# jameschapman19/cca_zoo

Hardware: NVIDIA H100
Metric: rcca_fit_per_s (higher is better)
Workload: dtype tf32x3b+f32

## Files before the change

cca_zoo_b200/_base.py:

```python
from __future__ import annotations

from abc import ABC, abstractmethod
from numbers import Integral
from typing import Any, ClassVar

import numpy as np
import torch
from sklearn.base import BaseEstimator
from sklearn.utils._param_validation import Interval, StrOptions
from sklearn.utils.validation import check_is_fitted

from . import ops, parallel
from ._validation import validate_views


_COPY_STREAMS: dict = {}


def _copy_stream(device):
    key = (device.type, device.index)
    if key not in _COPY_STREAMS:
        _COPY_STREAMS[key] = torch.cuda.Stream(device)
    return _COPY_STREAMS[key]

# ... 24 lines not shown
    _wants_second_moment: ClassVar[bool] = False
    _wants_column_means: ClassVar[bool] = False

    def __init__(self, latent_dimensions: int = 1, center: bool = True, precision: str = "tf32x3b",
                 device=None) -> None:
        self.latent_dimensions = latent_dimensions
        self.center = center
        self.precision = precision
        self.device = device

    _param_names_by_class: ClassVar[dict] = {}

    def _validate_params(self):
        cls = type(self)
        names = BaseModel._param_names_by_class.get(cls)
        if names is None:
            names = BaseModel._param_names_by_class[cls] = tuple(cls._get_param_names())
        snap = tuple(_freeze(getattr(self, n, None)) for n in names)
        if self.__dict__.get("_validated_params_") == snap:
            return
        super()._validate_params()
        self._validated_params_ = snap

    @abstractmethod
    def fit(self, views, y=None):
        """Fit the model to multiview data (list of ``(n_samples, n_features_i)`` arrays)."""

    @abstractmethod
    def _solve(self, C: torch.Tensor, dims: list[int], n_total: int) -> list[torch.Tensor]:
        """Weights from the block covariance (device tensors)."""

    def _device(self) -> torch.device:
        if not torch.cuda.is_available():
            raise RuntimeError(
                "cca_zoo_b200 needs a CUDA device (sm_90a); there is no CPU fallback.  "
                "Use the reference cca_zoo package on CPU-only machines."
            )
        if self.device is None:
            return torch.device("cuda", torch.cuda.current_device())
        return torch.device(self.device)

    def _to_device(self, v, device):
        if isinstance(v, torch.Tensor):
            t = v
        else:
            arr = np.asarray(v)
            if arr.dtype not in (np.float32, np.float64):
                arr = arr.astype(np.float64)
            t = torch.from_numpy(np.ascontiguousarray(arr))
        if t.dtype not in (torch.float32, torch.float64):
            t = t.to(torch.float64)
        return t.to(device, non_blocking=True)

    _stream_threshold_bytes: ClassVar[int] = 64 << 20
    _stream_chunk_rows: ClassVar[int] = 16384

    def _local_moments(self, validated, device):
        host = all(not (isinstance(v, torch.Tensor) and v.is_cuda) for v in validated)
        n_rows = int(validated[0].shape[0])
        nbytes = sum(int(np.prod(v.shape)) * (v.element_size() if isinstance(v, torch.Tensor) else v.dtype.itemsize)
                     for v in validated)
        if not (host and nbytes >= self._stream_threshold_bytes and n_rows >= 4 * self._stream_chunk_rows):
            dev_views = [self._to_device(v, device) for v in validated]
            if len({v.dtype for v in dev_views}) > 1:
                dev_views = [v.to(torch.float64) for v in dev_views]
            dims = [int(v.shape[1]) for v in dev_views]
            mom, _ = ops.moments_safe(dev_views, precision=self.precision)
            return mom, n_rows, dims, dev_views[0].dtype
        cpu_views = []
        for v in validated:
            t = v if isinstance(v, torch.Tensor) else torch.from_numpy(np.ascontiguousarray(v))
            if t.dtype not in (torch.float32, torch.float64):
                t = t.to(torch.float64)
            cpu_views.append(t)
        if len({t.dtype for t in cpu_views}) > 1:
            cpu_views = [t.to(torch.float64) for t in cpu_views]
        dims = [int(t.shape[1]) for t in cpu_views]
        main = torch.cuda.current_stream(device)
        copy = _copy_stream(device)
        mom = None
        step = self._stream_chunk_rows
        pending = None
        self._stream_x0 = "undecided"
        for lo in range(0, n_rows, step):
            hi = min(lo + step, n_rows)
            with torch.cuda.stream(copy):
                chunk = [t[lo:hi].to(device, non_blocking=True) for t in cpu_views]
                ready = torch.cuda.Event()
                ready.record(copy)
            if pending is not None:
                mom = self._accumulate(mom, pending, main)
            pending = (chunk, ready)
        mom = self._accumulate(mom, pending, main)
        return mom, n_rows, dims, cpu_views[0].dtype

    def _accumulate(self, mom, pending, main):
        chunk, ready = pending
        main.wait_event(ready)
        for c in chunk:
            c.record_stream(main)
        if isinstance(self._stream_x0, str):
            cand, ratio = ops.column_pilot(chunk)
            self._stream_x0 = cand if ratio > ops.SHIFT_RATIO[chunk[0].dtype] else None
        if self._stream_x0 is None:
            part = ops.moments(chunk, precision=self.precision)
        else:
            part, _ = ops.moments_safe(chunk, precision=self.precision, x0=self._stream_x0)
        if mom is None:
            return part
        mom.add_(part)
        return mom

    def _solve_dtype(self, in_dtype):
        return torch.float64 if (self._solve_in_float64 or in_dtype == torch.float64) else torch.float32

    def _covariance_stage(self, mom, n_local, dims, in_dtype, check_finite, reduced=False):
        if reduced:
            n_total = int(n_local)
        else:
            mom, n_total = parallel.allreduce_moments(mom, n_local, dims=dims)
        if check_finite and not bool(torch.isfinite(mom).all()):
            raise ValueError("Input contains NaN or infinity.")
        solve_dtype = self._solve_dtype(in_dtype)
        centred = bool(self.center) or self._covariance_always_centred
        C, mean = ops.covariance(mom, dims, n_total, center=centred, dtype=solve_dtype)
        self._second_moment = None
        if self._wants_second_moment and not self.center:
            self._second_moment, _ = ops.covariance(mom, dims, n_total, center=False, dtype=solve_dtype)
        self.n_views_ = len(dims)
        self.n_features_in_ = dims
        self.n_samples_ = n_total
        off = np.concatenate([[0], np.cumsum(dims)]).astype(int)
        mean_np = mean.to(torch.float64).cpu().numpy()
        if self._wants_column_means:
            self._column_means = mean_np if centred else ops.column_means(mom, dims, n_total)
        np_dtype = np.float32 if in_dtype == torch.float32 else np.float64
        if self.center:
            self.means_ = [mean_np[off[i]:off[i + 1]].astype(np_dtype) for i in range(len(dims))]
        else:
            self.means_ = [np.zeros(p) for p in dims]
        return C, dims, n_total

    def _fit_device(self, views, min_views: int = 2):
        self._validate_params()
        validated = validate_views(views, min_views)
        device = self._device()
        mom, n_local, dims, in_dtype = self._local_moments(validated, device)
        self._partial = None
        return self._covariance_stage(mom, n_local, dims, in_dtype, True)

    def _device_fit_plan(self, dims, n_local, in_dtype):
        return None

    def _fit_moments(self, mom, n_local, dims, in_dtype):
        plan = self._device_fit_plan(dims, n_local, in_dtype)
        if plan is None:
            C, dims, n_total = self._covariance_stage(mom, n_local, dims, in_dtype, True)
            return self._finish(self._solve(C, dims, n_total))
        mom, n_host, n_dev = parallel.allreduce_moments_lazy(mom, n_local, dims=dims)
        solve_dtype = self._solve_dtype(in_dtype)
        attempts = plan.pop("iters")
        hdr = None
        for iters in attempts:
            block, offsets = plan["call"](mom, dims, n_host, n_dev, solve_dtype, iters)
            host = block.cpu()
            hdr, mean, sig, ws = ops.decode_fit_block(host, offsets, dims, plan["k"], solve_dtype)
            status = int(hdr[0])
            if status & ops.FIT_NON_FINITE:
                raise ValueError("Input contains NaN or infinity.")
            if status == 0:
                n_total = int(round(float(hdr[1])))
                self.n_views_ = len(dims)
                self.n_features_in_ = dims
                self.n_samples_ = n_total
                np_dtype = np.float32 if in_dtype == torch.float32 else np.float64
                off = np.concatenate([[0], np.cumsum(dims)]).astype(int)
                if self.center:
                    self.means_ = [mean[off[i]:off[i + 1]].astype(np_dtype) for i in range(len(dims))]
                else:
                    self.means_ = [np.zeros(p) for p in dims]
                self._second_moment = None
                self.weights_ = [np.array(w) for w in ws]
                self._fit_info = {"route": "device", "iters": iters, "residual": float(hdr[2]), "sigma_1": float(hdr[3]),
                                  "ritz_sweeps": int(hdr[5])}
                return self
            if status != ops.FIT_NOT_CONVERGED:
                break
        n_total = int(round(float(hdr[1])))
        C, dims, n_total = self._covariance_stage(mom, n_total, dims, in_dtype, False, reduced=True)
        self._fit_info = {"route": "host", "device_status": int(hdr[0])}
        return self._finish(self._solve(C, dims, n_total))

    def partial_fit(self, views, y=None, solve: bool = True):
        self._validate_params()
        validated = validate_views(views)
        device = self._device()
        mom, n_local, dims, in_dtype = self._local_moments(validated, device)
        state = getattr(self, "_partial", None)
        if state is not None:
            if state["dims"] != dims or state["dtype"] != in_dtype:
                raise ValueError(f"partial_fit batches must keep the view widths/dtype: {state['dims']} vs {dims}")
            mom = state["mom"].to(device).add_(mom)
            n_local += state["n"]
        self._partial = {"mom": mom, "n": n_local, "dims": dims, "dtype": in_dtype}
        if solve:
            if type(self)._requires_two_views and len(dims) != 2:
                raise ValueError(f"rCCA requires exactly 2 views, got {len(dims)}. Use MCCA for more than 2 views.")
            self._fit_moments(mom.clone(), n_local, dims, in_dtype)
        return self

    _requires_two_views: ClassVar[bool] = False

    def __getstate__(self):
        state = super().__getstate__()
        part = state.get("_partial")
        if part is not None:
            state = dict(state)
            state["_partial"] = {**part, "mom": part["mom"].detach().cpu()}
        return state

    def _finish(self, weights: list[torch.Tensor]):
        self.weights_ = [w.cpu().numpy() for w in weights]
        return self

    @staticmethod
    def _as_numpy_views(views):
        out = []
        for v in views:
            out.append(v.detach().cpu().numpy() if isinstance(v, torch.Tensor) else v)
        return out

    def transform(self, views):
        check_is_fitted(self)
        on_gpu = any(isinstance(v, torch.Tensor) and v.is_cuda for v in views)
        big = sum(int(np.prod(getattr(v, "shape", (0,)))) for v in views) >= self._device_score_threshold
        if on_gpu or (big and torch.cuda.is_available()):
            return self._transform_device(validate_views(views))
        validated = validate_views(self._as_numpy_views(views))
        return [(v - m) @ w for v, m, w in zip(validated, self.means_, self.weights_)]

    def _transform_device(self, validated, weights=None):
        device = self._device()
        out = []
        for v, m, w in zip(validated, self.means_, self.weights_ if weights is None else weights):
            X = self._to_device(v, device)
            np_dt = np.result_type(X.cpu().numpy().dtype if False else (np.float32 if X.dtype == torch.float32
                                                                         else np.float64), w.dtype)
            dt = torch.float32 if np_dt == np.float32 else torch.float64
            X = X.to(dt)
            W = torch.from_numpy(np.ascontiguousarray(w, dtype=np_dt)).to(device)
            mw = -(np.asarray(m, dtype=np.float64) @ np.asarray(w, dtype=np.float64))
            Z = torch.from_numpy(mw.astype(np_dt)).to(device).expand(X.shape[0], -1).contiguous()
            ops.gemm(X, W, beta=1.0, out=Z)
            out.append(Z.cpu().numpy())
        return out

    def fit_transform(self, views, y=None):
        return self.fit(views, y).transform(views)

    def score(self, views, y=None):
        return self.average_pairwise_correlations(views)

    _device_score_threshold: ClassVar[int] = 1 << 24

    def _pairwise_correlations_device(self, validated):
        device = self._device()
        dev_views = [self._to_device(v, device) for v in validated]
        if len({v.dtype for v in dev_views}) > 1:
            dev_views = [v.to(torch.float64) for v in dev_views]
        dims = [int(v.shape[1]) for v in dev_views]
        if dims != list(self.n_features_in_):
            raise ValueError(f"views have {dims} features, the model was fitted on {self.n_features_in_}")
        mom, _ = ops.moments_safe(dev_views, precision=self.precision)
        mom, n_total = parallel.allreduce_moments(mom, int(dev_views[0].shape[0]), dims=dims)
        C, _ = ops.covariance(mom, dims, n_total, center=True, dtype=torch.float64)
        off = np.concatenate([[0], np.cumsum(dims)]).astype(int)
        sl = [slice(int(off[i]), int(off[i + 1])) for i in range(len(dims))]
        W = [torch.from_numpy(np.ascontiguousarray(w, dtype=np.float64)).to(device) for w in self.weights_]
        m, k = len(dims), W[0].shape[1]
        S = torch.empty((m, m, k), dtype=torch.float64, device=device)
        for i in range(m):
            Ti = ops.gemm(C[:, sl[i]], W[i])
            for j in range(m):
                S[j, i] = ops.gemm(W[j], Ti[sl[j]], transa=True).diagonal()
        S = S.cpu().numpy()
        norms = np.sqrt(np.stack([S[i, i] for i in range(m)]) * (n_total - 1))
        denom = np.where(norms > 1e-12, norms, 1.0) / np.sqrt(n_total - 1)
        return S / (denom[:, None, :] * denom[None, :, :])

    def pairwise_correlations(self, views):
        check_is_fitted(self)
        on_gpu = any(isinstance(v, torch.Tensor) and v.is_cuda for v in views)
        big = sum(int(np.prod(getattr(v, "shape", (0,)))) for v in views) >= self._device_score_threshold
        if on_gpu or (big and torch.cuda.is_available()):
            return self._pairwise_correlations_device(validate_views(views))
        transformed = self.transform(views)
        T = np.stack(transformed, axis=0)
        T = T - T.mean(axis=1, keepdims=True)
        norms = np.sqrt((T**2).sum(axis=1, keepdims=True))
        T_norm = T / np.where(norms > 1e-12, norms, 1.0)
        return np.einsum("isd,jsd->ijd", T_norm, T_norm)

    def average_pairwise_correlations(self, views):
        corrs = self.pairwise_correlations(views)
        n_views = corrs.shape[0]
        off_diag_sum = corrs.sum(axis=(0, 1)) - sum(corrs[i, i, :] for i in range(n_views))
        return off_diag_sum / (n_views * (n_views - 1))

    @property
    def weights(self):
        check_is_fitted(self)
        return self.weights_

    def get_factor_loadings(self, views):
        validated = validate_views(self._as_numpy_views(views))
        transformed = self.transform(views)
        loadings = []
# ... 16 lines not shown
```

cca_zoo_b200/_lib.py:

```python
from __future__ import annotations

import ctypes as C
import os

_HERE = os.path.dirname(os.path.abspath(__file__))
LIB_PATH = os.path.join(_HERE, "libccab200.so")

F32, F64 = 0, 1
PREC_TF32, PREC_TF32X3, PREC_EXACT, PREC_TF32X3B = 0, 1, 2, 3
MAX_VIEWS = 8

_i64p = C.POINTER(C.c_int64)
_vp = C.c_void_p

SIGNATURES = {
    "ccab_version": (C.c_int, []),
    "ccab_last_error": (C.c_char_p, []),
    "ccab_launch_count": (C.c_int64, []),
    "ccab_moments_size": (C.c_int64, [C.c_int, _i64p]),
    "ccab_moments_padded_dim": (C.c_int64, [C.c_int, _i64p]),
    "ccab_moments_workspace_bytes": (C.c_size_t, [C.c_int, C.c_int, C.c_int, _i64p, C.c_int64]),
    "ccab_moments": (C.c_int, [C.c_int, C.c_int, C.c_int, C.POINTER(_vp), _i64p, _i64p, C.c_int64, _vp, _vp,
                               C.c_size_t, _vp]),
    "ccab_moments_packed_size": (C.c_int64, [C.c_int, _i64p]),
    "ccab_moments_pack": (C.c_int, [C.c_int, _i64p, _vp, C.c_double, _vp, _vp]),
    "ccab_moments_unpack": (C.c_int, [C.c_int, _i64p, _vp, _vp, _vp]),
    "ccab_moments_exchange_nvls": (C.c_int, [C.c_int, _i64p, _vp, C.c_double, _vp, _vp, _vp, C.c_int, C.c_int, C.c_int,
                                             C.c_int64, C.c_uint, _vp, _vp]),
    "ccab_column_pilot": (C.c_int, [C.c_int, _vp, C.c_int64, C.c_int, C.c_int64, _vp, _vp, _vp]),
    "ccab_shift_rows": (C.c_int, [C.c_int, _vp, C.c_int64, C.c_int, C.c_int64, _vp, _vp, C.c_int64, _vp]),
    "ccab_moments_unshift": (C.c_int, [C.c_int, C.c_int, _i64p, _vp, C.POINTER(_vp), C.c_double, _vp]),
    "ccab_covariance": (C.c_int, [C.c_int, C.c_int, _i64p, _vp, C.c_double, C.c_int, _vp, C.c_int64, _vp, _vp]),
    "ccab_syevj_workspace_bytes": (C.c_size_t, [C.c_int, C.c_int, C.c_int]),
    "ccab_syevj": (C.c_int, [C.c_int, C.c_int, C.c_int, _vp, C.c_int64, C.c_int64, C.c_double, _vp, _vp, C.c_int64,
                             C.POINTER(C.c_int), C.POINTER(C.c_float), _vp, C.c_size_t, _vp]),
    "ccab_syevj_small": (C.c_int, [C.c_int, C.c_int, C.c_int, _vp, C.c_int64, C.c_int64, _vp, _vp, C.c_int64, _vp, _vp]),
    "ccab_gesvj_workspace_bytes": (C.c_size_t, [C.c_int, C.c_int, C.c_int]),
    "ccab_gesvj": (C.c_int, [C.c_int, C.c_int, C.c_int, _vp, C.c_int64, _vp, _vp, C.c_int64, _vp, C.c_int64,
                             C.POINTER(C.c_int), C.POINTER(C.c_float), _vp, C.c_size_t, _vp]),
    "ccab_gemm": (C.c_int, [C.c_int, C.c_int, C.c_int, C.c_int, C.c_int, C.c_int, C.c_double, _vp, C.c_int64, _vp,
                            C.c_int64, C.c_double, _vp, C.c_int64, _vp]),
    "ccab_gemm_tc": (C.c_int, [C.c_int, C.c_int, C.c_int, C.c_int, C.c_int, C.c_double, _vp, C.c_int64, C.c_int64, _vp,
                               C.c_int64, C.c_int64, C.c_double, _vp, C.c_int64, C.c_int64, _vp, C.c_int64, C.c_int64,
                               C.c_int, C.c_int, _vp]),
    "ccab_whiten_rows": (C.c_int, [C.c_int, C.c_int, _vp, _vp, C.c_int64, C.c_double, C.c_double, _vp, C.c_double,
                                   C.c_double, C.c_int, C.c_double, _vp, C.c_int64, _vp, _vp, _vp]),
    "ccab_ccaloss_small": (C.c_int, [C.c_int, C.c_int, C.c_int, _vp, C.c_int64, C.c_double, _vp, _vp, _vp, _vp, _vp,
                                     _vp]),
    "ccab_potrf_inv_workspace_bytes": (C.c_size_t, [C.c_int, C.c_int, C.c_int]),
    "ccab_potrf_inv": (C.c_int, [C.c_int, C.c_int, C.c_int, _vp, C.c_int64, C.c_int64, _vp, C.c_int64, C.c_int64,
                                 C.c_double, _vp, _vp, C.c_size_t, _vp]),
    "ccab_rcca_fit_workspace_bytes": (C.c_size_t, [C.c_int, _i64p, C.c_int, C.c_int]),
    "ccab_rcca_fit_result_layout": (C.c_int, [C.c_int, _i64p, C.c_int, C.c_int, _i64p]),
    "ccab_rcca_fit": (C.c_int, [C.c_int, _i64p, _vp, _vp, C.c_double, C.c_int, C.POINTER(C.c_double), C.c_int, C.c_int,
                                C.c_int, _vp, C.c_size_t, _vp, C.c_size_t, _vp]),
    "ccab_ccaloss_workspace_bytes": (C.c_size_t, [C.c_int, C.c_int, C.c_int, C.c_int, C.c_int64]),
    "ccab_ccaloss_fwd": (C.c_int, [C.c_int, C.c_int, _vp, C.c_int64, _vp, C.c_int64, C.c_int64, C.c_int, C.c_int,
                                   C.c_double, _vp, _vp, _vp, _vp, C.c_size_t, _vp]),
    "ccab_ccaloss_bwd": (C.c_int, [C.c_int, _vp, C.c_int64, _vp, C.c_int64, C.c_int64, C.c_int, C.c_int, _vp, _vp, _vp,
                                   C.c_int64, _vp, C.c_int64, _vp]),
    "ccab_mcca_fit_workspace_bytes": (C.c_size_t, [C.c_int, C.c_int, _i64p, C.c_int, C.c_int]),
    "ccab_mcca_fit_result_layout": (C.c_int, [C.c_int, C.c_int, _i64p, C.c_int, C.c_int, _i64p]),
    "ccab_mcca_fit": (C.c_int, [C.c_int, C.c_int, _i64p, _vp, _vp, C.c_double, C.c_int, C.POINTER(C.c_double),
                                C.c_double, C.c_int, C.c_int, C.c_int, _vp, C.c_size_t, _vp, C.c_size_t, _vp]),
    "ccab_als_fit_workspace_bytes": (C.c_size_t, [C.c_int, _i64p]),
    "ccab_als_regression_workspace_bytes": (C.c_size_t, [C.c_int, _i64p]),
    "ccab_als_fit": (C.c_int, [C.c_int, C.c_int, _i64p, _vp, C.c_double, C.c_double, C.POINTER(C.c_double), C.c_double,
                               _vp, C.c_int, C.c_int, C.c_double, _vp, _vp, _vp, C.c_size_t, _vp]),
    "ccab_ey_fit_workspace_bytes": (C.c_size_t, [C.c_int, _i64p, C.c_int, C.c_int]),
    "ccab_ey_fit": (C.c_int, [C.c_int, _i64p, C.c_int, C.c_double, C.c_double, C.c_double, C.c_double, C.c_int, _vp,
                              C.c_int, C.POINTER(_vp), _i64p, C.c_int, _vp, _vp, _vp, C.c_size_t, _vp]),
    "ccab_gfa_fit_workspace_bytes": (C.c_size_t, [C.c_int, _i64p, C.c_int]),
    "ccab_gfa_fit": (C.c_int, [C.c_int, _i64p, C.c_int, _vp, C.c_double, _vp, C.c_double, C.c_int, C.c_int, _vp, _vp,
                               C.c_size_t, _vp]),
    "ccab_scale": (C.c_int, [C.c_int, C.c_int, C.c_int, _vp, C.c_int64, _vp, C.c_int, _vp, C.c_int, _vp, C.c_int64,
                             _vp]),
    "ccab_center_columns": (C.c_int, [C.c_int, C.c_int, C.c_int, _vp, C.c_int64, _vp]),
    "ccab_frobenius_norm": (C.c_int, [C.c_int, C.c_int, C.c_int, _vp, C.c_int64, _vp, _vp]),
    "ccab_profile_moments": (C.c_int, [C.c_int]),
    "ccab_profile_moments_last_ms": (C.c_double, []),
}

_lib = None


def load():
    global _lib
    if _lib is None:
        if not os.path.exists(LIB_PATH):
            raise RuntimeError(
                f"{LIB_PATH} not found: build it with `python -c 'import __graft_entry__ as g; g.build()'` "
                "(or `make -C cca_zoo_b200/csrc`).  cca_zoo_b200 has no CPU fallback."
            )
        lib = C.CDLL(LIB_PATH)
        for name, (res, args) in SIGNATURES.items():
            fn = getattr(lib, name)
            fn.restype = res
            fn.argtypes = args
        _lib = lib
    return _lib


def last_error() -> str:
    return load().ccab_last_error().decode("utf-8", "replace")


def check(rc: int, what: str) -> None:
    if rc == 0:
        return
    msg = f"{what} failed (code {rc}): {last_error()}"
    if rc < 0:
        raise ValueError(msg)
    raise RuntimeError(msg)


def i64_array(values):
    return (C.c_int64 * len(values))(*[int(v) for v in values])
```

cca_zoo_b200/_solvers.py:

```python
from __future__ import annotations

import os

import numpy as np
import torch

from . import ops


def _slices(dims):
    off = np.concatenate([[0], np.cumsum(dims)]).astype(int)
    return [slice(int(off[i]), int(off[i + 1])) for i in range(len(dims))]


def _eps(dtype):
    return float(torch.finfo(dtype).eps)


class _two_streams:

    _pool = {}

    def __init__(self, device):
        self.device = device

    def __enter__(self):
        key = (self.device.index, torch.cuda.current_stream(self.device).cuda_stream)
        if key not in self._pool:
            self._pool[key] = [torch.cuda.Stream(self.device), torch.cuda.Stream(self.device)]
        self.streams = self._pool[key]
        self.main = torch.cuda.current_stream(self.device)
        ev = torch.cuda.Event()
        ev.record(self.main)
        for st in self.streams:
            st.wait_event(ev)
        return self.streams

    def __exit__(self, *exc):
        for st in self.streams:
            ev = torch.cuda.Event()
            ev.record(st)
            self.main.wait_event(ev)
        return False


def _rank_tol(d, dtype):
    return d * _eps(dtype)


def _regularised_rank_tol(lam, c, d):
    tol = _rank_tol(d, lam.dtype)
    if c == 0.0:
        return tol
    if c >= 1.0:
        return -1.0
    lam_max = max(float(lam[0].item()), 0.0)
    thr = (tol * ((1.0 - c) * lam_max + c) - c) / (1.0 - c)
    if thr < 0.0 or lam_max == 0.0:
        return -1.0
    return thr / lam_max


def _block_eigh(C, dims):
    sl = _slices(dims)
    lams, vts = [None] * len(dims), [None] * len(dims)
    by_size = {}
    for i, d in enumerate(dims):
        by_size.setdefault(d, []).append(i)
    for d, idx in by_size.items():
        A = torch.stack([C[sl[i], sl[i]] for i in idx]).contiguous()
        ev, evt = ops.syevj(A)
        for b, i in enumerate(idx):
            lams[i], vts[i] = ev[b], evt[b]
    return lams, vts


def _cholqr(Y, flags, passes=1):
    for _ in range(passes):
        Ginv, info = ops.potrf_inv_(ops.gemm(Y, Y, transa=True))
        flags.append(info)
        Y = ops.gemm(Y, Ginv, transb=True)
    return Y


def topk_svd(T, k, max_rounds=4, iters_per_round=5, oversample=None, seed=1234):
    d1, d2 = T.shape
    if oversample is None:
        oversample = int(os.environ.get("CCAB_TOPK_OVERSAMPLE", "0")) or max(32, k // 2)
    p = min(min(d1, d2), k + oversample)
    gen = torch.Generator(device=T.device).manual_seed(seed)
    Z = torch.randn((d2, p), generator=gen, device=T.device, dtype=T.dtype)
    flags = []
    tol = 200.0 * _eps(T.dtype)
    iters_per_round = int(os.environ.get("CCAB_TOPK_ITERS", "0")) or iters_per_round
    for _ in range(max_rounds):
        for it in range(iters_per_round):
            Y = ops.gemm(T, Z)
            Z = _cholqr(ops.gemm(T, Y, transa=True), flags,
                         passes=2 if it == iters_per_round - 1 else 1)
        Y = ops.gemm(T, Z)
        sig2, Vy_t = ops.syevj(ops.gemm(Y, Y, transa=True))
        sig = sig2.clamp_min(0).sqrt()
        Ut = ops.scale(ops.gemm(Vy_t[:k], Y, transb=True), rows=sig[:k], rows_pow=-1)
        Vt = ops.gemm(Vy_t[:k], Z, transb=True)
        E = ops.gemm(Ut, T)
        E -= ops.scale(Vt, rows=sig[:k])
        stats = torch.stack([ops.frobenius_norm(E)[0], sig[0], torch.stack(flags).max().to(T.dtype).reshape(())])
        resid, s1, bad = (float(x) for x in stats.cpu())
        if os.environ.get("CCAB_DEBUG_TOPK"):
            print(f"[topk_svd] p={p} iters={iters_per_round} resid={resid:.3e} limit={tol * s1 * (k ** 0.5):.3e}")
        if bad != 0.0 or not (s1 > 0.0):
            return None
        if resid <= tol * s1 * (k ** 0.5):
            return sig[:k], Ut, Vt
        flags = []
        Z = ops.gemm(Z, Vy_t, transb=True)
    return None


def topk_eigsh(K, k, shift, max_rounds=6, iters_per_round=8, seed=4321):
    D = K.shape[0]
    p = min(D, max(2 * k, k + 32))
    gen = torch.Generator(device=K.device).manual_seed(seed)
    Z = torch.randn((D, p), generator=gen, device=K.device, dtype=K.dtype)
    flags = []
    Z = _cholqr(Z, flags, passes=2)
    tol = 200.0 * _eps(K.dtype)
    for _ in range(max_rounds):
        for it in range(iters_per_round):
            Y = ops.gemm(K, Z)
            if shift != 0.0:
                Y.add_(Z, alpha=shift)
            Z = _cholqr(Y, flags, passes=2 if it == iters_per_round - 1 else 1)
        KZ = ops.gemm(K, Z)
        H = ops.gemm(Z, KZ, transa=True)
        H = 0.5 * (H + H.T)
        nrm = ops.frobenius_norm(H)
        theta, Qt = ops.syevj(H, shift=float(nrm.item()))
        Zr_t = ops.gemm(Qt[:k], Z, transb=True)
        E = ops.gemm(Qt[:k], KZ, transb=True)
        E -= ops.scale(Zr_t, rows=theta[:k])
        stats = torch.stack([ops.frobenius_norm(E)[0], theta[0].abs() + abs(shift),
                             torch.stack(flags).max().to(K.dtype).reshape(())])
        resid, scale, bad = (float(x) for x in stats.cpu())
        if bad != 0.0 or not (scale > 0.0):
            return None
        if resid <= tol * scale * (k ** 0.5):
            return theta[:k], Zr_t
        flags = []
        Z = ops.gemm(Z, Qt, transb=True)
    return None


def _cholesky_whiteners(C, dims, c, scales, eps_floor):
    sl = _slices(dims)
    out, flags, norms = [], [], []
    for i, s in enumerate(sl):
        R = (1.0 - c[i]) * C[s, s]
        R.diagonal().add_(c[i])
        dmax = R.diagonal().max()
        Linv, info = ops.potrf_inv_(R, pivot_tol=0.0)
        flags.append(info)
        norms.append(torch.stack([ops.frobenius_norm(Linv)[0], dmax]))
        out.append(Linv)
    stats = torch.cat([torch.stack(flags).max().to(C.dtype).reshape(1), torch.stack(norms).reshape(-1)]).cpu()
    if float(stats[0]) != 0.0:
        return None
    for i in range(len(dims)):
        fro, dmax = float(stats[1 + 2 * i]), float(stats[2 + 2 * i])
        if not (fro > 0.0) or not np.isfinite(fro):
            return None
        lam_min_lb = 1.0 / (fro * fro)
        if lam_min_lb < eps_floor or lam_min_lb < _rank_tol(dims[i], C.dtype) * dmax:
            return None
    return [Linv if scales[i] == 1.0 else Linv.mul_(scales[i] ** 0.5) for i, Linv in enumerate(out)]


def mcca_weights_cholesky(C, dims, latent_dimensions, c, eps):
    m = len(dims)
    sl = _slices(dims)
    D = C.shape[0]
    k = min(latent_dimensions, D)
    if 4 * k > D:
        return None
    Linv = _cholesky_whiteners(C, dims, c, [1.0] * m, eps)
    if Linv is None:
        return None
    K = torch.zeros((D, D), dtype=C.dtype, device=C.device)
    for i in range(m):
        for j in range(i + 1, m):
            tmp = ops.gemm(Linv[i], C[sl[i], sl[j]])
            ops.gemm(tmp, Linv[j], transb=True, out=K[sl[i], sl[j]])
            K[sl[j], sl[i]] = K[sl[i], sl[j]].T
    cmax = max(c)
    shift = 1.0 / (1.0 - cmax) if cmax <= 0.9 else float(ops.frobenius_norm(K).item())
    res = topk_eigsh(K, k, shift)
    if res is None:
        return None
    _, Yt = res
    return [ops.gemm(Linv[i], Yt[:, sl[i]], transa=True, transb=True, alpha=m ** 0.5) for i in range(m)]


def _pad_null_components(weights, k_out):
    k = weights[0].shape[1]
    if k_out <= k:
        return weights
    return [torch.cat([w, torch.zeros((w.shape[0], k_out - k), dtype=w.dtype, device=w.device)], dim=1)
            for w in weights]


def gcca_weights_cholesky(C, dims, n_samples, latent_dimensions, c, mu, eps, second_moment=None):
    Cd = C if second_moment is None else second_moment
    m = len(dims)
    sl = _slices(dims)
    D = C.shape[0]
    k = min(latent_dimensions, D, n_samples)
    if 4 * k > D:
        return None
    Wt = _cholesky_whiteners(C, dims, c, mu, eps)
    if Wt is None:
        return None
    Lc = _cholesky_whiteners(Cd, dims, [0.0] * m, [1.0] * m, 0.0) \
        if (Cd is not C or any(ci != 0.0 for ci in c) or any(x == 0.0 for x in mu)) \
        else [w / (mu[i] ** 0.5) for i, w in enumerate(Wt)]
# ... 159 lines not shown
```

cca_zoo_b200/csrc/api.cu:

```cuda
#include "../../include/ccab200.h"

#include <cstdarg>
#include <cmath>
#include <cstring>
#include <atomic>
#include <exception>

#include "als.cuh"
#include "ccaloss.cuh"
#include "cholinv.cuh"
#include "common.cuh"
#include "gfa.cuh"
#include "dense.cuh"
#include "ey.cuh"
#include "fit.cuh"
#include "moments.cuh"
#include "syevj.cuh"
#include "syevj_small.cuh"
#include "tgemm.cuh"

namespace ccab {
static thread_local char g_err[512] = "";
void set_error(const char* fmt, ...) {
  va_list ap;
// ... 321 lines not shown
              const void* B, int64_t ldb, double beta, void* C, int64_t ldc, void* stream) {
  CCAB_TRY
  CCAB_CHECK_ARG(dtype == CCAB_F32 || dtype == CCAB_F64, "bad dtype %d", dtype);
  CCAB_CHECK_ARG(A && B && C, "null pointer argument");
  int rc = require_device();
  if (rc) return rc;
  cudaStream_t s = static_cast<cudaStream_t>(stream);
  if (dtype == CCAB_F32) {
    GemmArgs<float> g;
    g.transa = transa; g.transb = transb; g.m = m; g.n = n; g.k = k; g.alpha = (float)alpha; g.beta = (float)beta;
    g.A = static_cast<const float*>(A); g.lda = lda; g.B = static_cast<const float*>(B); g.ldb = ldb;
    g.C = static_cast<float*>(C); g.ldc = ldc;
    return xgemm<float>(g, s);
  }
  GemmArgs<double> g;
  g.transa = transa; g.transb = transb; g.m = m; g.n = n; g.k = k; g.alpha = alpha; g.beta = beta;
  g.A = static_cast<const double*>(A); g.lda = lda; g.B = static_cast<const double*>(B); g.ldb = ldb;
  g.C = static_cast<double*>(C); g.ldc = ldc;
  return xgemm<double>(g, s);
  CCAB_CATCH
}

int ccab_gemm_tc(int transa, int transb, int m, int n, int k, double alpha, const void* A, int64_t lda,
                 int64_t stride_a, const void* B, int64_t ldb, int64_t stride_b, double beta, void* C, int64_t ldc,
                 int64_t stride_c, void* Ct, int64_t ldct, int64_t stride_ct, int batch, int lower_only,
                 void* stream) {
  CCAB_TRY
  CCAB_CHECK_ARG(A && B && (C || Ct), "null pointer argument");
  CCAB_CHECK_ARG(m >= 1 && n >= 1 && k >= 1 && batch >= 1, "bad shape m=%d n=%d k=%d batch=%d", m, n, k, batch);
  CCAB_CHECK_ARG((!C || ldc >= n) && (!Ct || ldct >= m), "output leading dimension too small");
  int rc = require_device();
  if (rc) return rc;
  TgemmArgs a;
  a.transa = transa;
  a.transb = transb;
  a.m = m;
  a.n = n;
  a.k = k;
  a.alpha = (float)alpha;
  a.beta = (float)beta;
  a.A = static_cast<const float*>(A);
  a.lda = lda;
  a.strideA = stride_a;
  a.B = static_cast<const float*>(B);
  a.ldb = ldb;
  a.strideB = stride_b;
  a.C = static_cast<float*>(C);
  a.ldc = ldc;
  a.strideC = stride_c;
  a.Ct = static_cast<float*>(Ct);
  a.ldct = ldct;
  a.strideCt = stride_ct;
  a.batch = batch;
  a.lower_only = lower_only;
  return tgemm(a, static_cast<cudaStream_t>(stream));
  CCAB_CATCH
}

int ccab_whiten_rows(int dtype, int d, const void* lam, const void* Vt, int64_t ldv, double c, double floor_add,
                     const void* floor_dev, double scale, double rank_tol, int max_rank, double lam_floor, void* Wt,
                     int64_t ldw, void* g_out, int* rank_out, void* stream) {
  CCAB_TRY
  CCAB_CHECK_ARG(dtype == CCAB_F32 || dtype == CCAB_F64, "bad dtype %d", dtype);
  CCAB_CHECK_ARG(lam && Vt && Wt, "null pointer argument");
  CCAB_CHECK_ARG(scale > 0.0, "scale must be positive");
  int rc = require_device();
  if (rc) return rc;
  cudaStream_t s = static_cast<cudaStream_t>(stream);
  if (dtype == CCAB_F32)
    return whiten_rows<float>(d, static_cast<const float*>(lam), static_cast<const float*>(Vt), ldv, c, floor_add,
                              static_cast<const float*>(floor_dev), scale, rank_tol, max_rank, lam_floor,
                              static_cast<float*>(Wt), ldw, static_cast<float*>(g_out), rank_out, s);
  return whiten_rows<double>(d, static_cast<const double*>(lam), static_cast<const double*>(Vt), ldv, c, floor_add,
                             static_cast<const double*>(floor_dev), scale, rank_tol, max_rank, lam_floor,
                             static_cast<double*>(Wt), ldw, static_cast<double*>(g_out), rank_out, s);
  CCAB_CATCH
}

int ccab_ccaloss_small(int dtype, int d1, int d2, const void* C, int64_t ldc, double eps, void* loss, void* G11,
                       void* P, void* G22, void* min_pivot, void* stream) {
  CCAB_TRY
  CCAB_CHECK_ARG(dtype == CCAB_F32 || dtype == CCAB_F64, "bad dtype %d", dtype);
  CCAB_CHECK_ARG(C && loss && G11 && P && G22 && min_pivot, "null pointer argument");
  int rc = require_device();
  if (rc) return rc;
  cudaStream_t s = static_cast<cudaStream_t>(stream);
  if (dtype == CCAB_F32)
    return ccaloss_small<float>(static_cast<const float*>(C), ldc, d1, d2, eps, static_cast<float*>(loss),
                                static_cast<float*>(G11), static_cast<float*>(P), static_cast<float*>(G22),
                                static_cast<float*>(min_pivot), s);
  return ccaloss_small<double>(static_cast<const double*>(C), ldc, d1, d2, eps, static_cast<double*>(loss),
                               static_cast<double*>(G11), static_cast<double*>(P), static_cast<double*>(G22),
                               static_cast<double*>(min_pivot), s);
  CCAB_CATCH
}

size_t ccab_potrf_inv_workspace_bytes(int dtype, int n, int batch) {
  if (n < 1 || batch < 1) return 0;
  return dtype == CCAB_F32 ? potrf_inv_workspace_bytes<float>(n, batch) : potrf_inv_workspace_bytes<double>(n, batch);
}

int ccab_potrf_inv(int dtype, int n, int batch, void* A, int64_t lda, int64_t stride_a, void* Linv, int64_t ldi,
                   int64_t stride_i, double pivot_tol, int* info_dev, void* workspace, size_t workspace_bytes,
                   void* stream) {
  CCAB_TRY
  CCAB_CHECK_ARG(dtype == CCAB_F32 || dtype == CCAB_F64, "bad dtype %d", dtype);
  CCAB_CHECK_ARG(A && Linv && info_dev && workspace, "null pointer argument");
  int rc = require_device();
  if (rc) return rc;
  cudaStream_t s = static_cast<cudaStream_t>(stream);
  if (dtype == CCAB_F32)
    return potrf_inv<float>(n, batch, static_cast<float*>(A), lda, stride_a, static_cast<float*>(Linv), ldi, stride_i,
                            pivot_tol, nullptr, info_dev, workspace, workspace_bytes, s);
  return potrf_inv<double>(n, batch, static_cast<double*>(A), lda, stride_a, static_cast<double*>(Linv), ldi, stride_i,
                           pivot_tol, nullptr, info_dev, workspace, workspace_bytes, s);
  CCAB_CATCH
}

size_t ccab_rcca_fit_workspace_bytes(int dtype, const int64_t* dims, int k, int p) {
  if (!dims || dims[0] < 1 || dims[1] < 1 || (dtype != CCAB_F32 && dtype != CCAB_F64)) return 0;
  return dtype == CCAB_F32 ? rcca_fit_workspace_bytes<float>((int)dims[0], (int)dims[1], k, p)
                           : rcca_fit_workspace_bytes<double>((int)dims[0], (int)dims[1], k, p);
}

int ccab_rcca_fit_result_layout(int dtype, const int64_t* dims, int k, int p, int64_t* offsets) {
  CCAB_TRY
  CCAB_CHECK_ARG(dims && offsets && dims[0] >= 1 && dims[1] >= 1 && k >= 1 && p >= k, "bad argument");
  if (dtype == CCAB_F32) rcca_fit_result_layout<float>((int)dims[0], (int)dims[1], k, p, offsets);
  else rcca_fit_result_layout<double>((int)dims[0], (int)dims[1], k, p, offsets);
  return 0;
  CCAB_CATCH
}

int ccab_rcca_fit(int dtype, const int64_t* dims, const double* moments, const double* n_total_dev, double n_total,
                  int center, const double* c, int k, int p, int iters, void* result, size_t result_bytes,
                  void* workspace, size_t workspace_bytes, void* stream) {
  CCAB_TRY
  CCAB_CHECK_ARG(dtype == CCAB_F32 || dtype == CCAB_F64, "bad dtype %d", dtype);
  CCAB_CHECK_ARG(dims && moments && c && result && workspace, "null pointer argument");
  ColumnLayout L;
  int rc = make_layout(2, dims, &L);
  if (rc) return rc;
  rc = require_device();
  if (rc) return rc;
  cudaStream_t s = static_cast<cudaStream_t>(stream);
  if (dtype == CCAB_F32)
    return rcca_fit<float>(L, moments, n_total_dev, n_total, center, c, k, p, iters, result, result_bytes, workspace,
                           workspace_bytes, s);
  return rcca_fit<double>(L, moments, n_total_dev, n_total, center, c, k, p, iters, result, result_bytes, workspace,
                          workspace_bytes, s);
  CCAB_CATCH
}

size_t ccab_ccaloss_workspace_bytes(int dtype, int precision, int d1, int d2, int64_t n) {
  int64_t dims[2] = {d1, d2};
  ColumnLayout L;
  if (make_layout(2, dims, &L)) return 0;
  if (dtype == CCAB_F64) precision = CCAB_PREC_EXACT;
  return dtype == CCAB_F32 ? ccaloss_workspace_bytes<float>(L, n, precision)
                           : ccaloss_workspace_bytes<double>(L, n, precision);
}

int ccab_ccaloss_fwd(int dtype, int precision, const void* z1, int64_t ld1, const void* z2, int64_t ld2, int64_t n,
                     int d1, int d2, double eps, void* loss, void* saved, int* flags_dev, void* workspace,
                     size_t workspace_bytes, void* stream) {
  CCAB_TRY
  CCAB_CHECK_ARG(dtype == CCAB_F32 || dtype == CCAB_F64, "bad dtype %d", dtype);
  CCAB_CHECK_ARG(precision >= 0 && precision <= 3, "bad precision %d", precision);
  CCAB_CHECK_ARG(z1 && z2 && loss && saved && flags_dev && workspace, "null pointer argument");
  CCAB_CHECK_ARG(ld1 >= d1 && ld2 >= d2, "leading dimension too small");
  int64_t dims[2] = {d1, d2};
  ColumnLayout L;
  int rc = make_layout(2, dims, &L);
  if (rc) return rc;
  rc = require_device();
  if (rc) return rc;
  cudaStream_t s = static_cast<cudaStream_t>(stream);
  if (dtype == CCAB_F32)
    return ccaloss_forward<float>(L, precision, z1, ld1, z2, ld2, n, eps, static_cast<float*>(loss),
                                  static_cast<float*>(saved), flags_dev, workspace, workspace_bytes, s);
  return ccaloss_forward<double>(L, CCAB_PREC_EXACT, z1, ld1, z2, ld2, n, eps, static_cast<double*>(loss),
                                 static_cast<double*>(saved), flags_dev, workspace, workspace_bytes, s);
  CCAB_CATCH
}

int ccab_ccaloss_bwd(int dtype, const void* z1, int64_t ld1, const void* z2, int64_t ld2, int64_t n, int d1, int d2,
                     const void* saved, const void* grad_out, void* g1, int64_t ldg1, void* g2, int64_t ldg2,
                     void* stream) {
  CCAB_TRY
  CCAB_CHECK_ARG(dtype == CCAB_F32 || dtype == CCAB_F64, "bad dtype %d", dtype);
  CCAB_CHECK_ARG(z1 && z2 && saved && g1 && g2, "null pointer argument");
  CCAB_CHECK_ARG(ld1 >= d1 && ld2 >= d2 && ldg1 >= d1 && ldg2 >= d2, "leading dimension too small");
  int rc = require_device();
  if (rc) return rc;
  cudaStream_t s = static_cast<cudaStream_t>(stream);
  if (dtype == CCAB_F32)
    return ccaloss_backward<float>(d1, d2, static_cast<const float*>(z1), ld1, static_cast<const float*>(z2), ld2, n,
                                   static_cast<const float*>(saved), static_cast<const float*>(grad_out),
                                   static_cast<float*>(g1), ldg1, static_cast<float*>(g2), ldg2, s);
  return ccaloss_backward<double>(d1, d2, static_cast<const double*>(z1), ld1, static_cast<const double*>(z2), ld2, n,
                                  static_cast<const double*>(saved), static_cast<const double*>(grad_out),
                                  static_cast<double*>(g1), ldg1, static_cast<double*>(g2), ldg2, s);
  CCAB_CATCH
}

size_t ccab_mcca_fit_workspace_bytes(int dtype, int n_views, const int64_t* dims, int k, int p) {
  ColumnLayout L;
  if (!dims || make_layout(n_views, dims, &L) || (dtype != CCAB_F32 && dtype != CCAB_F64)) return 0;
  return dtype == CCAB_F32 ? mcca_fit_workspace_bytes<float>(L, k, p) : mcca_fit_workspace_bytes<double>(L, k, p);
}

int ccab_mcca_fit_result_layout(int dtype, int n_views, const int64_t* dims, int k, int p, int64_t* offsets) {
  CCAB_TRY
  CCAB_CHECK_ARG(dims && offsets && k >= 1 && p >= k, "bad argument");
  ColumnLayout L;
  int rc = make_layout(n_views, dims, &L);
  if (rc) return rc;
  if (dtype == CCAB_F32) mcca_fit_result_layout<float>(L, k, p, offsets);
  else mcca_fit_result_layout<double>(L, k, p, offsets);
  return 0;
  CCAB_CATCH
}

int ccab_mcca_fit(int dtype, int n_views, const int64_t* dims, const double* moments, const double* n_total_dev,
                  double n_total, int center, const double* c, double eps, int k, int p, int iters, void* result,
                  size_t result_bytes, void* workspace, size_t workspace_bytes, void* stream) {
  CCAB_TRY
  CCAB_CHECK_ARG(dtype == CCAB_F32 || dtype == CCAB_F64, "bad dtype %d", dtype);
  CCAB_CHECK_ARG(dims && moments && c && result && workspace, "null pointer argument");
  ColumnLayout L;
  int rc = make_layout(n_views, dims, &L);
  if (rc) return rc;
  rc = require_device();
  if (rc) return rc;
  cudaStream_t s = static_cast<cudaStream_t>(stream);
  if (dtype == CCAB_F32)
    return mcca_fit<float>(L, moments, n_total_dev, n_total, center, c, eps, k, p, iters, result, result_bytes,
                           workspace, workspace_bytes, s);
  return mcca_fit<double>(L, moments, n_total_dev, n_total, center, c, eps, k, p, iters, result, result_bytes, workspace,
                          workspace_bytes, s);
  CCAB_CATCH
}

size_t ccab_als_fit_workspace_bytes(int n_views, const int64_t* dims) {
  ColumnLayout L;
  if (!dims || n_views < 2 || make_layout(n_views, dims, &L)) return 0;
  return als_fit_workspace_bytes(L, false);
}

size_t ccab_als_regression_workspace_bytes(int n_views, const int64_t* dims) {
  ColumnLayout L;
  if (!dims || n_views < 2 || make_layout(n_views, dims, &L)) return 0;
  return als_fit_workspace_bytes(L, true);
}

int ccab_als_fit(int kind, int n_views, const int64_t* dims, const double* G, double g_scale, double n_samples,
                 const double* params, double mu, const double* init, int k, int max_iter, double tol, double* W_out,
                 int* iters_out, void* workspace, size_t workspace_bytes, void* stream) {
  CCAB_TRY
  CCAB_CHECK_ARG(kind >= CCAB_ALS_PLS && kind <= CCAB_ALS_IPLS, "bad ALS kind %d", kind);
  CCAB_CHECK_ARG(n_views >= 2, "the ALS estimators need at least 2 views, got %d", n_views);
  CCAB_CHECK_ARG(dims && G && init && W_out && iters_out && workspace, "null pointer argument");
  CCAB_CHECK_ARG(kind == CCAB_ALS_PLS || params, "params is NULL");
  CCAB_CHECK_ARG(k >= 1 && max_iter >= 0, "bad k %d / max_iter %d", k, max_iter);
  CCAB_CHECK_ARG(kind != CCAB_ALS_ADMM || (mu > 0.0 && n_samples > 0.0), "ADMM needs mu > 0 and n_samples > 0");
  ColumnLayout L;
  int rc = make_layout(n_views, dims, &L);
  if (rc) return rc;
  const bool reg = kind == CCAB_ALS_ELASTIC || kind == CCAB_ALS_IPLS;
  for (int v = 0; reg && v < n_views; ++v) {
    const double alpha = params[2 * v], l1 = params[2 * v + 1];
    CCAB_CHECK_ARG(alpha >= 0.0 && alpha < INFINITY, "alpha[%d] = %g is not a finite non-negative number", v, alpha);
    CCAB_CHECK_ARG(l1 >= 0.0 && l1 <= 1.0, "l1_ratio[%d] = %g is not in [0, 1]", v, l1);
    CCAB_CHECK_ARG(dims[v] <= 2048, "view %d has %lld features; ElasticCCA / SCCA_IPLS take at most 2048 per view", v,
                   (long long)dims[v]);
  }
  CCAB_CHECK_ARG(!reg || n_samples > 0.0, "ElasticCCA / SCCA_IPLS need n_samples > 0");
  CCAB_CHECK_ARG(!reg || (mu >= 0.0 && mu < 1.0), "the eigenvalue cut mu = %g of ElasticCCA / SCCA_IPLS is not in [0, 1)",
                 mu);
  for (int v = 0; kind != CCAB_ALS_PLS && !reg && v < n_views; ++v) {
    CCAB_CHECK_ARG(params[v] >= 0.0, "params[%d] = %g is negative", v, params[v]);
    CCAB_CHECK_ARG(kind != CCAB_ALS_SPAN || (params[v] >= 1.0 && params[v] == (double)(int64_t)params[v]),
                   "span[%d] = %g is not a positive integer", v, params[v]);
  }
  rc = require_device();
  if (rc) return rc;
  return als_fit(kind, L, G, g_scale, n_samples, params, mu, init, k, max_iter, tol, W_out, iters_out, workspace,
                 workspace_bytes, static_cast<cudaStream_t>(stream));
  CCAB_CATCH
}

size_t ccab_ey_fit_workspace_bytes(int n_views, const int64_t* dims, int k, int batch) {
  ColumnLayout L;
  if (!dims || n_views < 2 || k < 1 || k > kEyMaxK || batch < 0 || batch == 1 || make_layout(n_views, dims, &L))
    return 0;
  return ey_fit_workspace_bytes(L, k, batch);
}

int ccab_ey_fit(int n_views, const int64_t* dims, int k, double c, double learning_rate, double momentum, double tol,
                int n_steps, const double* cov, int dtype, const void* const* views, const int64_t* ld, int batch,
                const int32_t* idx, double* state, void* workspace, size_t workspace_bytes, void* stream) {
  CCAB_TRY
  CCAB_CHECK_ARG(n_views >= 2, "the EY estimators need at least 2 views, got %d", n_views);
  CCAB_CHECK_ARG(dims && state && workspace, "null pointer argument");
  CCAB_CHECK_ARG(k >= 1 && k <= kEyMaxK, "k = %d: the EY fit supports 1 <= k <= %d", k, kEyMaxK);
  CCAB_CHECK_ARG(n_steps >= 0, "bad n_steps %d", n_steps);
// ... 104 lines not shown
```

cca_zoo_b200/csrc/fit.cu:

```cuda
#include "fit.cuh"

#include <cmath>
#include <type_traits>

#include "ccaloss.cuh"
#include "cholinv.cuh"
#include "dense.cuh"
#include "moments.cuh"
#include "syevj_small.cuh"

namespace ccab {

namespace {

inline size_t al256(size_t x) { return (x + 255) & ~size_t(255); }
inline int64_t r4(int64_t x) { return (x + 3) & ~int64_t(3); }

struct CovRidgeParams {
  int n_views, D, Dp;
  int dims[kMaxViews];
  int coff[kMaxViews + 1];
  int poff[kMaxViews + 1];
  double c[kMaxViews];
  double ridge_add[kMaxViews];
  void* R[kMaxViews];
  long long ldr[kMaxViews];
};
struct PivotTolParams {
  int n_views;
  double c[kMaxViews], rank_tol[kMaxViews];
  double floor;
};

__device__ __forceinline__ int view_of(const CovRidgeParams& p, int g) {
  int v = 0;
  while (v + 1 < p.n_views && p.coff[v + 1] <= g) ++v;
  return v;
}

template <typename T>
__global__ void cov_ridge_kernel(const CovRidgeParams p, const double* __restrict__ mom, const double* __restrict__ n_dev,
                                 double n_host, int center, T* __restrict__ C, int64_t ldc, double* __restrict__ mean,
                                 unsigned* __restrict__ dmax, int* __restrict__ flags) {
  const double n_total = n_dev ? n_dev[0] : n_host;
  const double* M = mom;
  const double* s = mom + (size_t)p.Dp * p.Dp;
  const int gi = blockIdx.y * blockDim.y + threadIdx.y;
  const int gj = blockIdx.x * blockDim.x + threadIdx.x;
  if (gi >= p.D || gj >= p.D) return;
  const int vi = view_of(p, gi), vj = view_of(p, gj);
  const int pi = p.poff[vi] + gi - p.coff[vi], pj = p.poff[vj] + gj - p.coff[vj];
  const int r = min(pi, pj), c = max(pi, pj);
  double v = M[(size_t)r * p.Dp + c];
  if (!isfinite(v)) atomicOr(flags, 1);
  if (center) v -= s[pi] * s[pj] / n_total;
  v /= (n_total - 1.0);
  C[(size_t)gi * ldc + gj] = (T)v;
  if (vi == vj && p.R[vi]) {
    const double cv = p.c[vi];
    const double rv = (1.0 - cv) * v + (gi == gj ? cv + p.ridge_add[vi] : 0.0);
    static_cast<T*>(p.R[vi])[(size_t)(gi - p.coff[vi]) * p.ldr[vi] + (gj - p.coff[vj])] = (T)rv;
    if (gi == gj && dmax) atomicMax(dmax + vi, __float_as_uint(fmaxf((float)v, 0.f)));
  }
  if (gi == 0 && mean) mean[gj] = center ? s[pj] / n_total : 0.0;
  if (gi == 0 && gj == 0 && !(n_total >= 2.0)) atomicOr(flags, 2);
}

__global__ void pivot_tol_kernel(const PivotTolParams q, const unsigned* __restrict__ dmax, double* __restrict__ tol) {
  const int v = threadIdx.x;
  if (v < q.n_views) tol[v] = fmax(q.floor, q.rank_tol[v] * ((1.0 - q.c[v]) * (double)__uint_as_float(dmax[v]) + q.c[v]));
}

template <typename T>
__global__ void randn_kernel(T* __restrict__ Z, int64_t ld, int rows, int cols, unsigned long long seed) {
  const size_t total = (size_t)rows * cols;
  for (size_t e = blockIdx.x * (size_t)blockDim.x + threadIdx.x; e < total; e += (size_t)gridDim.x * blockDim.x) {
    unsigned long long x = seed + 0x9E3779B97F4A7C15ull * (e + 1);
    x = (x ^ (x >> 30)) * 0xBF58476D1CE4E5B9ull;
    x = (x ^ (x >> 27)) * 0x94D049BB133111EBull;
    x ^= x >> 31;
    const double u1 = ((double)(unsigned)(x >> 32) + 1.0) * (1.0 / 4294967297.0);
    const double u2 = (double)(unsigned)(x & 0xffffffffu) * (1.0 / 4294967296.0);
    const double g = sqrt(-2.0 * log(u1)) * cospi(2.0 * u2);
    Z[(e / cols) * ld + (e % cols)] = (T)g;
  }
}

template <typename T>
__global__ void ritz_scale_kernel(T* __restrict__ U, int64_t ldu, int rows, int k, const T* __restrict__ lam,
                                  T* __restrict__ sig) {
  const int j = blockIdx.x * blockDim.x + threadIdx.x;
  const int i = blockIdx.y;
  if (j >= k) return;
  const T s = sqrt(fmax(lam[j], T(0)));
  if (i == 0 && sig) sig[j] = s;
  U[(size_t)i * ldu + j] *= s > T(0) ? T(1) / s : T(0);
}

constexpr int kResidBlocks = 64;
template <typename T>
__global__ void __launch_bounds__(256)
residual_kernel(const T* __restrict__ E, int64_t lde, const T* __restrict__ V, int64_t ldv, int rows, int k,
                const T* __restrict__ sig, double shift, int sym, double* __restrict__ stats,
                double* __restrict__ partial, unsigned* __restrict__ counter) {
  __shared__ double red[8];
  __shared__ bool last;
  const int per = (rows + gridDim.x - 1) / gridDim.x;
  const int r0 = blockIdx.x * per;
  const int nr = max(0, min(rows, r0 + per) - r0);
  double acc = 0.0;
  for (int e = threadIdx.x; e < nr * k; e += blockDim.x) {
    const int i = r0 + e / k, j = e % k;
    const double d = (double)E[(size_t)i * lde + j] - (double)V[(size_t)i * ldv + j] * (double)sig[j];
    acc += d * d;
  }
  for (int o = 16; o > 0; o >>= 1) acc += __shfl_xor_sync(0xffffffffu, acc, o);
  if ((threadIdx.x & 31) == 0) red[threadIdx.x >> 5] = acc;
  __syncthreads();
  if (threadIdx.x == 0) {
    double t = 0.0;
    for (int w = 0; w < (int)(blockDim.x >> 5); ++w) t += red[w];
    partial[blockIdx.x] = t;
    __threadfence();
    last = atomicAdd(counter, 1u) == gridDim.x - 1;
    if (last) {
      __threadfence();
      double tot = 0.0;
      for (unsigned b = 0; b < gridDim.x; ++b) tot += *reinterpret_cast<volatile double*>(partial + b);
      stats[0] = tot;
      stats[1] = sym ? fabs((double)sig[0]) + shift : (double)sig[0];
      *counter = 0u;
    }
  }
}

__global__ void fit_status_kernel(double* __restrict__ hdr, const int* __restrict__ flags, const int* __restrict__ infos,
                                  int n_infos, const int* __restrict__ rr_info, const double* __restrict__ stats,
                                  const double* __restrict__ n_dev, double n_host, double resid_tol, int k, int max_d) {
  if (threadIdx.x != 0) return;
  const double n_total = n_dev ? n_dev[0] : n_host;
  int status = 0;
  if (flags[0] & 1) status |= kFitNonFinite;
  if (flags[0] & 2) status |= kFitTooFewSamples;
  int first_bad = 0;
  for (int i = 0; i < n_infos; ++i)
    if (infos[i] != 0 && !first_bad) first_bad = i + 1;
  if (first_bad) status |= kFitNotPositiveDefinite;
  const double resid = sqrt(fmax(stats[0], 0.0)), s1 = stats[1];
  if (!(s1 > 0.0) || !(resid <= resid_tol * s1 * sqrt((double)k))) status |= kFitNotConverged;
  if (rr_info && rr_info[0] <= 0) status |= kFitNotConverged;
  if (!(n_total > (double)max_d)) status |= kFitTooFewSamples;
  hdr[0] = (double)status;
  hdr[1] = n_total;
  hdr[2] = resid;
  hdr[3] = s1;
  hdr[4] = (double)first_bad;
  hdr[5] = rr_info ? (double)rr_info[0] : 0.0;
}

template <typename T>
double eps_of() {
  return std::is_same<T, float>::value ? 1.1920928955078125e-7 : 2.220446049250313e-16;
}
template <typename T>
double resid_tol_of() {
  return std::max(200.0 * eps_of<T>(), 1e-10);
}

template <typename T>
struct CholQrWs {
  T* G;
  T* Ginv;
  void* pws;
  size_t pws_bytes;
  int64_t ldg;
  void* splitk_ws = nullptr;
  size_t splitk_ws_bytes = 0;
};

template <typename T>
int cholqr(const T* Zin, int64_t ldz, T* Zout, int64_t ldo, int rows, int p, const CholQrWs<T>& w, int* info,
           cudaStream_t s) {
  GemmArgs<T> g;
  g.transa = 1; g.m = p; g.n = p; g.k = rows;
  g.A = Zin; g.lda = ldz; g.B = Zin; g.ldb = ldz; g.C = w.G; g.ldc = w.ldg;
  g.splitk_ws = w.splitk_ws; g.splitk_ws_bytes = w.splitk_ws_bytes;
  int rc = xgemm<T>(g, s);
  if (rc) return rc;
  const int NB = potrf_inv_block_size<T>();
  int64_t ldi;
  if (p <= NB) {
    rc = potrf_inv_block<T>(w.G, w.ldg, 0, p, 0, w.Ginv, 0, 0.0, nullptr, info, 1, s);
    ldi = NB;
  } else {
    int* tmp_info = info;
    rc = potrf_inv<T>(p, 1, w.G, w.ldg, 0, w.Ginv, w.ldg, 0, 0.0, nullptr, tmp_info, w.pws, w.pws_bytes, s);
    ldi = w.ldg;
  }
  if (rc) return rc;
  GemmArgs<T> q;
  q.transb = 1; q.m = rows; q.n = p; q.k = p;
  q.A = Zin; q.lda = ldz; q.B = w.Ginv; q.ldb = ldi; q.C = Zout; q.ldc = ldo;
  return xgemm<T>(q, s);
}

struct RccaPlan {
  int d1, d2, D, k, p;
  int64_t ldC, ld1, ld2, ldT, ldp, ldk;
  size_t oC, oR, oLinv, oT1, oT, oZ, oZ2, oY, oG, oGinv, oH, oLam, oVy, oU, oV, oE, oPws, oSplit, oSmall, total;
  size_t pws_bytes, split_bytes;
  size_t r_mean, r_sig, r_w1, r_w2, r_total;
};

template <typename T>
RccaPlan make_rcca_plan(int d1, int d2, int k, int p) {
  RccaPlan P;
  P.d1 = d1; P.d2 = d2; P.D = d1 + d2; P.k = k; P.p = p;
  P.ldC = r4(P.D); P.ld1 = r4(d1); P.ld2 = r4(d2); P.ldT = r4(d2); P.ldp = r4(p); P.ldk = r4(k);
  const int NB = potrf_inv_block_size<T>();
  const int dm = std::max(d1, d2);
  size_t o = 0;
  auto take = [&](size_t elems) { size_t at = o; o += al256(elems * sizeof(T)); return at; };
  P.oC = take((size_t)P.D * P.ldC);
  P.oR = take(2 * (size_t)dm * r4(dm));
  P.oLinv = take(2 * (size_t)dm * r4(dm));
  P.oT1 = take((size_t)d1 * P.ldT);
  P.oT = take((size_t)d1 * P.ldT);
  P.oZ = take((size_t)d2 * P.ldp);
  P.oZ2 = take((size_t)d2 * P.ldp);
  P.oY = take((size_t)d1 * P.ldp);
  P.oG = take((size_t)p * P.ldp);
  P.oGinv = take((size_t)std::max(p, NB) * std::max<int64_t>(P.ldp, NB));
  P.oH = take((size_t)p * P.ldp);
  P.oLam = take((size_t)p);
  P.oVy = take((size_t)p * P.ldp);
  P.oU = take((size_t)d1 * P.ldk);
  P.oV = take((size_t)d2 * P.ldk);
  P.oE = take((size_t)d2 * P.ldk);
  P.pws_bytes = std::max(potrf_inv_workspace_bytes<T>(dm, 2), potrf_inv_workspace_bytes<T>(p, 1));
  P.oPws = o; o += al256(P.pws_bytes);
  P.split_bytes = 8 * (size_t)dm * r4(std::max(p, k)) * sizeof(T);
  P.oSplit = o; o += al256(P.split_bytes);
  P.oSmall = o; o += 4096;
  P.total = o + 256;
  size_t r = sizeof(double) * kFitHeaderDoubles;
  P.r_mean = r; r += al256(sizeof(double) * P.D);
  P.r_sig = r; r += al256(sizeof(T) * k);
  P.r_w1 = r; r += al256(sizeof(T) * (size_t)d1 * k);
  P.r_w2 = r; r += al256(sizeof(T) * (size_t)d2 * k);
  P.r_total = r;
  return P;
}

}

template <typename T>
size_t rcca_fit_workspace_bytes(int d1, int d2, int k, int p) {
  if (!(k >= 1 && p >= k && p <= std::min(d1, d2) && syevj_small_supported<T>(p))) return 0;
  return make_rcca_plan<T>(d1, d2, k, p).total;
}

template <typename T>
void rcca_fit_result_layout(int d1, int d2, int k, int p, int64_t* offsets) {
  RccaPlan P = make_rcca_plan<T>(d1, d2, k, p);
  offsets[0] = (int64_t)P.r_mean;
  offsets[1] = (int64_t)P.r_sig;
  offsets[2] = (int64_t)P.r_w1;
  offsets[3] = (int64_t)P.r_w2;
  offsets[4] = (int64_t)P.r_total;
}

template <typename T>
int rcca_fit(const ColumnLayout& L, const double* moments, const double* n_dev, double n_host, int center,
             const double* c, int k, int p, int iters, void* result, size_t result_bytes, void* ws, size_t ws_bytes,
             cudaStream_t s) {
  CCAB_CHECK_ARG(L.n_views == 2, "rcca_fit needs exactly 2 views");
  const int d1 = L.dims[0], d2 = L.dims[1], D = L.D;
  CCAB_CHECK_ARG(k >= 1 && p >= k && p <= std::min(d1, d2), "rcca_fit: need 1 <= k <= p <= min(d1, d2), got k=%d p=%d", k,
                 p);
  CCAB_CHECK_ARG(syevj_small_supported<T>(p), "rcca_fit: subspace width %d exceeds the single-CTA eigensolver", p);
  CCAB_CHECK_ARG(iters >= 1 && iters <= 64, "rcca_fit: bad iteration count %d", iters);
  RccaPlan P = make_rcca_plan<T>(d1, d2, k, p);
  CCAB_CHECK_ARG(ws_bytes >= P.total, "rcca_fit workspace too small: %zu < %zu", ws_bytes, P.total);
  CCAB_CHECK_ARG(result_bytes >= P.r_total, "rcca_fit result block too small: %zu < %zu", result_bytes, P.r_total);
  uint8_t* w = reinterpret_cast<uint8_t*>((reinterpret_cast<uintptr_t>(ws) + 255) & ~uintptr_t(255));
  uint8_t* res = static_cast<uint8_t*>(result);
  CCAB_CHECK_ARG((reinterpret_cast<uintptr_t>(res) & 255) == 0, "rcca_fit: result block must be 256-byte aligned");
  auto at = [&](size_t off) { return reinterpret_cast<T*>(w + off); };
  T* C = at(P.oC);
  const bool batched = d1 == d2;
  const int64_t ldR = r4(std::max(d1, d2));
  const int64_t strideR = (int64_t)std::max(d1, d2) * ldR;
  T* R1 = at(P.oR);
  T* R2 = R1 + strideR;
  T* Li1 = at(P.oLinv);
  T* Li2 = Li1 + strideR;
  const int64_t ldr1 = batched ? ldR : P.ld1, ldr2 = batched ? ldR : P.ld2;
  T *T1 = at(P.oT1), *Tm = at(P.oT), *Z = at(P.oZ), *Z2 = at(P.oZ2), *Y = at(P.oY), *H = at(P.oH), *lam = at(P.oLam),
    *Vy = at(P.oVy), *U = at(P.oU), *V = at(P.oV), *E = at(P.oE);
  CholQrWs<T> cq;
  cq.G = at(P.oG);
  cq.Ginv = at(P.oGinv);
  cq.pws = w + P.oPws;
  cq.pws_bytes = P.pws_bytes;
  cq.ldg = P.ldp;
  cq.splitk_ws = w + P.oSplit;
  cq.splitk_ws_bytes = P.split_bytes;
  auto thin = [&](GemmArgs<T>& g) { g.splitk_ws = cq.splitk_ws; g.splitk_ws_bytes = cq.splitk_ws_bytes; };
  uint8_t* sm = w + P.oSmall;
  int* flags = reinterpret_cast<int*>(sm);
  int* infos = flags + 4;
  const int n_infos = 2 + iters + 2;
  int* rr_info = infos + 80;
  unsigned* dmax = reinterpret_cast<unsigned*>(sm + 512);
  double* tol = reinterpret_cast<double*>(sm + 1024);
  double* stats = tol + 8;
  double* resid_part = reinterpret_cast<double*>(sm + 1280);
  unsigned* resid_cnt = reinterpret_cast<unsigned*>(sm + 1280 + 8 * kResidBlocks);

  CCAB_CUDA(cudaMemsetAsync(sm, 0, 2048, s));
  double* hdr = reinterpret_cast<double*>(res);
  double* mean = reinterpret_cast<double*>(res + P.r_mean);
  T* sig = reinterpret_cast<T*>(res + P.r_sig);
  T* W1 = reinterpret_cast<T*>(res + P.r_w1);
  T* W2 = reinterpret_cast<T*>(res + P.r_w2);

  {
    CovRidgeParams cp;
    memset(&cp, 0, sizeof(cp));
    cp.n_views = 2; cp.D = D; cp.Dp = L.Dp;
    for (int v = 0; v < 2; ++v) { cp.dims[v] = L.dims[v]; cp.c[v] = c[v]; }
    for (int v = 0; v <= 2; ++v) { cp.coff[v] = L.coff[v]; cp.poff[v] = L.poff[v]; }
    cp.R[0] = R1; cp.R[1] = R2; cp.ldr[0] = ldr1; cp.ldr[1] = ldr2;
    dim3 block(32, 8), grid((unsigned)ceil_div(D, 32), (unsigned)ceil_div(D, 8));
    cov_ridge_kernel<T><<<grid, block, 0, s>>>(cp, moments, n_dev, n_host, center, C, P.ldC, mean, dmax, flags);
    count_launches(1);
    PivotTolParams q;
    memset(&q, 0, sizeof(q));
    q.n_views = 2;
    q.c[0] = c[0]; q.c[1] = c[1];
    q.rank_tol[0] = d1 * eps_of<T>(); q.rank_tol[1] = d2 * eps_of<T>();
    pivot_tol_kernel<<<1, 32, 0, s>>>(q, dmax, tol);
    count_launches(1);
    CCAB_CUDA(cudaGetLastError());
  }
  int rc;
  if (batched) {
    rc = potrf_inv<T>(d1, 2, R1, ldR, strideR, Li1, ldR, strideR, 0.0, tol, infos, cq.pws, cq.pws_bytes, s);
    if (rc) return rc;
  } else {
    rc = potrf_inv<T>(d1, 1, R1, ldr1, 0, Li1, ldr1, 0, 0.0, tol, infos, cq.pws, cq.pws_bytes, s);
    if (rc) return rc;
    rc = potrf_inv<T>(d2, 1, R2, ldr2, 0, Li2, ldr2, 0, 0.0, tol + 1, infos + 1, cq.pws, cq.pws_bytes, s);
    if (rc) return rc;
  }
  {
    GemmArgs<T> g;
    g.m = d1; g.n = d2; g.k = d1;
    g.A = Li1; g.lda = ldr1; g.B = C + d1; g.ldb = P.ldC; g.C = T1; g.ldc = P.ldT;
    rc = xgemm<T>(g, s);
    if (rc) return rc;
    GemmArgs<T> h;
    h.transb = 1; h.m = d1; h.n = d2; h.k = d2;
    h.A = T1; h.lda = P.ldT; h.B = Li2; h.ldb = ldr2; h.C = Tm; h.ldc = P.ldT;
    rc = xgemm<T>(h, s);
    if (rc) return rc;
  }
  {
    const size_t total = (size_t)d2 * p;
    randn_kernel<T><<<(unsigned)std::min<size_t>((total + 255) / 256, 592), 256, 0, s>>>(Z, P.ldp, d2, p, 0x1234ull);
    count_launches(1);
    CCAB_CUDA(cudaGetLastError());
  }
  int info_slot = 2;
  const bool gram = d2 <= d1 && iters >= 2;
  if (gram) {
    GemmArgs<T> g;
    g.transa = 1; g.m = d2; g.n = d2; g.k = d1; g.A = Tm; g.lda = P.ldT; g.B = Tm; g.ldb = P.ldT; g.C = T1; g.ldc = P.ldT;
    rc = xgemm<T>(g, s);
    if (rc) return rc;
  }
  for (int it = 0; it < iters; ++it) {
    if (gram) {
      GemmArgs<T> a;
      a.transa = 1; a.m = d2; a.n = p; a.k = d2; a.A = T1; a.lda = P.ldT; a.B = Z; a.ldb = P.ldp; a.C = Z2; a.ldc = P.ldp;
      thin(a);
      rc = xgemm<T>(a, s);
      if (rc) return rc;
    } else {
      GemmArgs<T> a;
      a.m = d1; a.n = p; a.k = d2; a.A = Tm; a.lda = P.ldT; a.B = Z; a.ldb = P.ldp; a.C = Y; a.ldc = P.ldp;
      rc = xgemm<T>(a, s);
      if (rc) return rc;
      GemmArgs<T> b;
      b.transa = 1; b.m = d2; b.n = p; b.k = d1; b.A = Tm; b.lda = P.ldT; b.B = Y; b.ldb = P.ldp; b.C = Z2; b.ldc = P.ldp;
      rc = xgemm<T>(b, s);
      if (rc) return rc;
    }
    rc = cholqr<T>(Z2, P.ldp, Z, P.ldp, d2, p, cq, infos + info_slot++, s);
    if (rc) return rc;
    if (it == iters - 1) {
      rc = cholqr<T>(Z, P.ldp, Z2, P.ldp, d2, p, cq, infos + info_slot++, s);
      if (rc) return rc;
      std::swap(Z, Z2);
    }
  }
  {
    GemmArgs<T> a;
    a.m = d1; a.n = p; a.k = d2; a.A = Tm; a.lda = P.ldT; a.B = Z; a.ldb = P.ldp; a.C = Y; a.ldc = P.ldp;
    thin(a);
    rc = xgemm<T>(a, s);
    if (rc) return rc;
    GemmArgs<T> h;
    h.transa = 1; h.m = p; h.n = p; h.k = d1; h.A = Y; h.lda = P.ldp; h.B = Y; h.ldb = P.ldp; h.C = H; h.ldc = P.ldp;
    thin(h);
    rc = xgemm<T>(h, s);
    if (rc) return rc;
    rc = syevj_small<T>(p, 1, H, P.ldp, 0, lam, p, Vy, P.ldp, 0, rr_info, s);
    if (rc) return rc;
    GemmArgs<T> u;
    u.transb = 1; u.m = d1; u.n = k; u.k = p; u.A = Y; u.lda = P.ldp; u.B = Vy; u.ldb = P.ldp; u.C = U; u.ldc = P.ldk;
    rc = xgemm<T>(u, s);
    if (rc) return rc;
    ritz_scale_kernel<T><<<dim3((unsigned)ceil_div(k, 128), (unsigned)d1), 128, 0, s>>>(U, P.ldk, d1, k, lam, sig);
    count_launches(1);
    GemmArgs<T> v;
    v.transb = 1; v.m = d2; v.n = k; v.k = p; v.A = Z; v.lda = P.ldp; v.B = Vy; v.ldb = P.ldp; v.C = V; v.ldc = P.ldk;
    rc = xgemm<T>(v, s);
    if (rc) return rc;
    GemmArgs<T> e;
    e.transa = 1; e.m = d2; e.n = k; e.k = d1; e.A = Tm; e.lda = P.ldT; e.B = U; e.ldb = P.ldk; e.C = E; e.ldc = P.ldk;
    thin(e);
    rc = xgemm<T>(e, s);
    if (rc) return rc;
    residual_kernel<T><<<kResidBlocks, 256, 0, s>>>(E, P.ldk, V, P.ldk, d2, k, sig, 0.0, 0, stats, resid_part, resid_cnt);
    count_launches(1);
    CCAB_CUDA(cudaGetLastError());
  }
  {
    GemmArgs<T> a;
    a.transa = 1; a.m = d1; a.n = k; a.k = d1; a.A = Li1; a.lda = ldr1; a.B = U; a.ldb = P.ldk; a.C = W1; a.ldc = k;
    thin(a);
    rc = xgemm<T>(a, s);
    if (rc) return rc;
    GemmArgs<T> b;
    b.transa = 1; b.m = d2; b.n = k; b.k = d2; b.A = Li2; b.lda = ldr2; b.B = V; b.ldb = P.ldk; b.C = W2; b.ldc = k;
    thin(b);
    rc = xgemm<T>(b, s);
    if (rc) return rc;
  }
  fit_status_kernel<<<1, 32, 0, s>>>(hdr, flags, infos, n_infos, rr_info, stats, n_dev, n_host, resid_tol_of<T>(), k,
                                    std::max(d1, d2));
  count_launches(1);
  CCAB_CUDA(cudaGetLastError());
  return 0;
}


namespace {

struct MccaPlan {
  int m, D, k, p, dmax;
  bool equal;
  int64_t ldC, ldR, strideR, ldp, ldk;
  int off[kMaxViews + 1];
  size_t oC, oR, oLinv, oTmp, oK, oZ, oZ2, oY, oG, oGinv, oH, oLam, oVy, oZr, oE, oPws, oSplit, oSmall, total;
  size_t pws_bytes, split_bytes;
  size_t r_mean, r_val, r_w[kMaxViews], r_total;
};

template <typename T>
MccaPlan make_mcca_plan(const ColumnLayout& L, int k, int p) {
  MccaPlan P;
  P.m = L.n_views; P.D = L.D; P.k = k; P.p = p;
  P.dmax = 0;
  P.equal = true;
  for (int v = 0; v < P.m; ++v) {
    P.dmax = std::max(P.dmax, L.dims[v]);
    if (L.dims[v] != L.dims[0]) P.equal = false;
    P.off[v] = L.coff[v];
  }
  P.off[P.m] = L.D;
  P.ldC = r4(P.D); P.ldR = r4(P.dmax); P.strideR = (int64_t)P.dmax * P.ldR; P.ldp = r4(p); P.ldk = r4(k);
  const int NB = potrf_inv_block_size<T>();
  size_t o = 0;
  auto take = [&](size_t elems) { size_t at = o; o += al256(elems * sizeof(T)); return at; };
  P.oC = take((size_t)P.D * P.ldC);
  P.oR = take((size_t)P.m * P.strideR);
  P.oLinv = take((size_t)P.m * P.strideR);
  P.oTmp = take((size_t)P.dmax * P.ldR);
  P.oK = take((size_t)P.D * P.ldC);
  P.oZ = take((size_t)P.D * P.ldp);
  P.oZ2 = take((size_t)P.D * P.ldp);
  P.oY = take((size_t)P.D * P.ldp);
  P.oG = take((size_t)p * P.ldp);
  P.oGinv = take((size_t)std::max(p, NB) * std::max<int64_t>(P.ldp, NB));
  P.oH = take((size_t)p * P.ldp);
  P.oLam = take((size_t)p);
  P.oVy = take((size_t)p * P.ldp);
  P.oZr = take((size_t)P.D * P.ldk);
  P.oE = take((size_t)P.D * P.ldk);
  P.pws_bytes = std::max(potrf_inv_workspace_bytes<T>(P.dmax, P.m), potrf_inv_workspace_bytes<T>(p, 1));
  P.oPws = o; o += al256(P.pws_bytes);
  P.split_bytes = 8 * (size_t)P.D * p * sizeof(T);
  P.oSplit = o; o += al256(P.split_bytes);
  P.oSmall = o; o += 4096;
  P.total = o + 256;
  size_t r = sizeof(double) * kFitHeaderDoubles;
  P.r_mean = r; r += al256(sizeof(double) * P.D);
  P.r_val = r; r += al256(sizeof(T) * k);
  for (int v = 0; v < P.m; ++v) { P.r_w[v] = r; r += al256(sizeof(T) * (size_t)L.dims[v] * k); }
  P.r_total = r;
  return P;
}

template <typename T>
__global__ void copy_vals_kernel(const T* __restrict__ src, T* __restrict__ dst, int k) {
  const int j = blockIdx.x * blockDim.x + threadIdx.x;
  if (j < k) dst[j] = src[j];
}

}

template <typename T>
size_t mcca_fit_workspace_bytes(const ColumnLayout& L, int k, int p) {
  if (!(L.n_views >= 2 && k >= 1 && p >= k && p <= L.D && syevj_small_supported<T>(p))) return 0;
  return make_mcca_plan<T>(L, k, p).total;
}

template <typename T>
void mcca_fit_result_layout(const ColumnLayout& L, int k, int p, int64_t* offsets) {
  MccaPlan P = make_mcca_plan<T>(L, k, p);
  offsets[0] = (int64_t)P.r_mean;
  offsets[1] = (int64_t)P.r_val;
  for (int v = 0; v < P.m; ++v) offsets[2 + v] = (int64_t)P.r_w[v];
  offsets[2 + P.m] = (int64_t)P.r_total;
}

template <typename T>
int mcca_fit(const ColumnLayout& L, const double* moments, const double* n_dev, double n_host, int center,
             const double* c, double eps_floor, int k, int p, int iters, void* result, size_t result_bytes, void* ws,
             size_t ws_bytes, cudaStream_t s) {
  const int m = L.n_views, D = L.D;
  CCAB_CHECK_ARG(m >= 2, "mcca_fit needs at least 2 views");
  CCAB_CHECK_ARG(k >= 1 && p >= k && p <= D, "mcca_fit: need 1 <= k <= p <= D, got k=%d p=%d", k, p);
  CCAB_CHECK_ARG(syevj_small_supported<T>(p), "mcca_fit: subspace width %d exceeds the single-CTA eigensolver", p);
  CCAB_CHECK_ARG(iters >= 1 && iters <= 60, "mcca_fit: bad iteration count %d", iters);
  double cmax = 0.0;
  for (int v = 0; v < m; ++v) cmax = std::max(cmax, c[v]);
  CCAB_CHECK_ARG(cmax <= 0.9, "mcca_fit: max c = %g > 0.9 (no a-priori shift); use the host-assembled route", cmax);
  MccaPlan P = make_mcca_plan<T>(L, k, p);
  CCAB_CHECK_ARG(ws_bytes >= P.total, "mcca_fit workspace too small: %zu < %zu", ws_bytes, P.total);
  CCAB_CHECK_ARG(result_bytes >= P.r_total, "mcca_fit result block too small: %zu < %zu", result_bytes, P.r_total);
  uint8_t* w = reinterpret_cast<uint8_t*>((reinterpret_cast<uintptr_t>(ws) + 255) & ~uintptr_t(255));
  uint8_t* res = static_cast<uint8_t*>(result);
  CCAB_CHECK_ARG((reinterpret_cast<uintptr_t>(res) & 255) == 0, "mcca_fit: result block must be 256-byte aligned");
  auto at = [&](size_t off) { return reinterpret_cast<T*>(w + off); };
  T *C = at(P.oC), *R = at(P.oR), *Linv = at(P.oLinv), *Tmp = at(P.oTmp), *K = at(P.oK), *Z = at(P.oZ), *Z2 = at(P.oZ2),
    *Y = at(P.oY), *H = at(P.oH), *lam = at(P.oLam), *Vy = at(P.oVy), *Zr = at(P.oZr), *E = at(P.oE);
  CholQrWs<T> cq;
  cq.G = at(P.oG);
  cq.Ginv = at(P.oGinv);
  cq.pws = w + P.oPws;
  cq.pws_bytes = P.pws_bytes;
  cq.ldg = P.ldp;
  cq.splitk_ws = w + P.oSplit;
  cq.splitk_ws_bytes = P.split_bytes;
  uint8_t* sm = w + P.oSmall;
  int* flags = reinterpret_cast<int*>(sm);
  int* infos = flags + 4;
  const int n_infos = m + iters + 4;
  int* rr_info = infos + 100;
  unsigned* dmax = reinterpret_cast<unsigned*>(sm + 512);
  double* tol = reinterpret_cast<double*>(sm + 1024);
  double* stats = tol + kMaxViews;
  double* resid_part = reinterpret_cast<double*>(sm + 1280);
  unsigned* resid_cnt = reinterpret_cast<unsigned*>(sm + 1280 + 8 * kResidBlocks);
  CCAB_CUDA(cudaMemsetAsync(sm, 0, 2048, s));
  CCAB_CUDA(cudaMemsetAsync(K, 0, sizeof(T) * (size_t)D * P.ldC, s));
  double* hdr = reinterpret_cast<double*>(res);
  double* mean = reinterpret_cast<double*>(res + P.r_mean);
  T* vals = reinterpret_cast<T*>(res + P.r_val);

  {
    CovRidgeParams cp;
    memset(&cp, 0, sizeof(cp));
    cp.n_views = m; cp.D = D; cp.Dp = L.Dp;
    PivotTolParams q;
    memset(&q, 0, sizeof(q));
    q.n_views = m;
    for (int v = 0; v < m; ++v) {
      cp.dims[v] = L.dims[v]; cp.c[v] = c[v];
      cp.R[v] = R + (size_t)v * P.strideR; cp.ldr[v] = P.ldR;
      q.c[v] = c[v]; q.rank_tol[v] = L.dims[v] * eps_of<T>();
    }
    for (int v = 0; v <= m; ++v) { cp.coff[v] = L.coff[v]; cp.poff[v] = L.poff[v]; }
    q.floor = eps_floor;
    dim3 block(32, 8), grid((unsigned)ceil_div(D, 32), (unsigned)ceil_div(D, 8));
    cov_ridge_kernel<T><<<grid, block, 0, s>>>(cp, moments, n_dev, n_host, center, C, P.ldC, mean, dmax, flags);
    count_launches(1);
    pivot_tol_kernel<<<1, 32, 0, s>>>(q, dmax, tol);
    count_launches(1);
    CCAB_CUDA(cudaGetLastError());
  }
  int rc;
  if (P.equal) {
    rc = potrf_inv<T>(L.dims[0], m, R, P.ldR, P.strideR, Linv, P.ldR, P.strideR, 0.0, tol, infos, cq.pws, cq.pws_bytes, s);
    if (rc) return rc;
// ... 285 lines not shown
    rc = moments_tf32(L, views, lds, n, precision, mom, w + P.oMomWs, P.mom_ws_bytes, s);
  else
    rc = moments_simt<T>(L, views, lds, n, mom, w + P.oMomWs, P.mom_ws_bytes, s);
  if (rc) return rc;
  CCAB_CUDA(cudaMemsetAsync(sm, 0, 1024, s));
  {
    CovRidgeParams cp;
    memset(&cp, 0, sizeof(cp));
    cp.n_views = 2; cp.D = D; cp.Dp = L.Dp;
    for (int v = 0; v < 2; ++v) { cp.dims[v] = L.dims[v]; cp.c[v] = 0.0; cp.ridge_add[v] = eps; }
    for (int v = 0; v <= 2; ++v) { cp.coff[v] = L.coff[v]; cp.poff[v] = L.poff[v]; }
    cp.R[0] = R1; cp.R[1] = R2; cp.ldr[0] = ldr1; cp.ldr[1] = ldr2;
    dim3 block(32, 8), grid((unsigned)ceil_div(D, 32), (unsigned)ceil_div(D, 8));
    cov_ridge_kernel<T><<<grid, block, 0, s>>>(cp, mom, nullptr, (double)n, 1, C, P.ldC, nullptr, dmax, flags + 4);
    count_launches(1);
    CCAB_CUDA(cudaGetLastError());
  }
  const double piv_tol = 0.25 * eps;
  if (P.batched) {
    rc = potrf_inv<T>(d1, 2, R1, P.ldR, P.strideR, Li1, P.ldR, P.strideR, piv_tol, nullptr, flags, w + P.oPws, P.pws_bytes, s);
    if (rc) return rc;
  } else {
    rc = potrf_inv<T>(d1, 1, R1, ldr1, 0, Li1, ldr1, 0, piv_tol, nullptr, flags, w + P.oPws, P.pws_bytes, s);
    if (rc) return rc;
    rc = potrf_inv<T>(d2, 1, R2, ldr2, 0, Li2, ldr2, 0, piv_tol, nullptr, flags + 1, w + P.oPws, P.pws_bytes, s);
    if (rc) return rc;
  }
  if (P.batched) {
    GemmArgs<T> g;
    g.transa = 1; g.m = d1; g.n = d1; g.k = d1;
    g.A = Li1; g.lda = P.ldR; g.strideA = P.strideR; g.B = Li1; g.ldb = P.ldR; g.strideB = P.strideR;
    g.C = A1; g.ldc = P.ldR; g.strideC = P.strideR; g.batch = 2;
    rc = xgemm<T>(g, s);
    if (rc) return rc;
  } else {
    for (int v = 0; v < 2; ++v) {
      GemmArgs<T> g;
      const int d = v ? d2 : d1;
      const int64_t ld = v ? ldr2 : ldr1;
      g.transa = 1; g.m = d; g.n = d; g.k = d;
      g.A = v ? Li2 : Li1; g.lda = ld; g.B = g.A; g.ldb = ld; g.C = v ? A2 : A1; g.ldc = ld;
      rc = xgemm<T>(g, s);
      if (rc) return rc;
    }
  }
  const T* S12 = C + d1;
  {
    GemmArgs<T> g;
    g.m = d1; g.n = d2; g.k = d1; g.A = A1; g.lda = ldr1; g.B = S12; g.ldb = P.ldC; g.C = Q; g.ldc = ldq;
    rc = xgemm<T>(g, s);
    if (rc) return rc;
    GemmArgs<T> h;
    h.m = d1; h.n = d2; h.k = d2; h.A = S12; h.lda = P.ldC; h.B = A2; h.ldb = ldr2; h.C = Q2; h.ldc = ldq;
    rc = xgemm<T>(h, s);
    if (rc) return rc;
    GemmArgs<T> p;
    p.m = d1; p.n = d2; p.k = d2; p.A = Q; p.lda = ldq; p.B = A2; p.ldb = ldr2; p.C = Pm; p.ldc = d2;
    rc = xgemm<T>(p, s);
    if (rc) return rc;
    GemmArgs<T> a;
    a.transb = 1; a.m = d1; a.n = d1; a.k = d2; a.A = Pm; a.lda = d2; a.B = Q; a.ldb = ldq; a.C = G11; a.ldc = d1;
    rc = xgemm<T>(a, s);
    if (rc) return rc;
    GemmArgs<T> b;
    b.transa = 1; b.m = d2; b.n = d2; b.k = d1; b.A = Q2; b.lda = ldq; b.B = Pm; b.ldb = d2; b.C = G22; b.ldc = d2;
    rc = xgemm<T>(b, s);
    if (rc) return rc;
  }
  {
    double* partial = reinterpret_cast<double*>(sm + 2048);
    loss_dot_partial_kernel<T><<<64, 256, 0, s>>>(Pm, d2, S12, P.ldC, d1, d2, partial);
    loss_dot_final_kernel<T><<<1, 32, 0, s>>>(partial, 64, loss);
    count_launches(2);
  }
  CCAB_CUDA(cudaGetLastError());
  CCAB_CUDA(cudaMemcpyAsync(flags_out, flags, 2 * sizeof(int), cudaMemcpyDeviceToDevice, s));
  CCAB_CUDA(cudaMemcpyAsync(flags_out + 2, flags + 4, sizeof(int), cudaMemcpyDeviceToDevice, s));
  return 0;
}

template <typename T>
int ccaloss_backward(int d1, int d2, const T* z1, int64_t ld1, const T* z2, int64_t ld2, int64_t n, const T* saved,
                     const T* grad_out, T* g1, int64_t ldg1, T* g2, int64_t ldg2, cudaStream_t s) {
  CCAB_CHECK_ARG(n >= 2 && d1 >= 1 && d2 >= 1, "ccaloss_backward: bad shape");
  if (std::max(d1, d2) <= 64)
    return ccaloss_small_backward<T>(d1, d2, z1, ld1, z2, ld2, n, saved, grad_out, g1, ldg1, g2, ldg2, s);
  const T* G11 = saved;
  const T* Pm = saved + (size_t)d1 * d1;
  const T* G22 = Pm + (size_t)d1 * d2;
  const T a = (T)(2.0 / (double)(n - 1));
  GemmArgs<T> g;
  g.m = (int)n; g.n = d1; g.k = d1; g.alpha = a; g.A = z1; g.lda = ld1; g.B = G11; g.ldb = d1; g.C = g1; g.ldc = ldg1;
  int rc = xgemm<T>(g, s);
  if (rc) return rc;
  GemmArgs<T> h;
  h.transb = 1; h.m = (int)n; h.n = d1; h.k = d2; h.alpha = -a; h.beta = T(1);
  h.A = z2; h.lda = ld2; h.B = Pm; h.ldb = d2; h.C = g1; h.ldc = ldg1;
  rc = xgemm<T>(h, s);
  if (rc) return rc;
  GemmArgs<T> u;
  u.m = (int)n; u.n = d2; u.k = d2; u.alpha = a; u.A = z2; u.lda = ld2; u.B = G22; u.ldb = d2; u.C = g2; u.ldc = ldg2;
  rc = xgemm<T>(u, s);
  if (rc) return rc;
  GemmArgs<T> v;
  v.m = (int)n; v.n = d2; v.k = d1; v.alpha = -a; v.beta = T(1);
  v.A = z1; v.lda = ld1; v.B = Pm; v.ldb = d2; v.C = g2; v.ldc = ldg2;
  rc = xgemm<T>(v, s);
  if (rc) return rc;
  {
    const int nslabs = (int)std::min<int64_t>(32, ceil_div(n, 128));
    const int rows_per_slab = (int)ceil_div(n, nslabs);
    double* part = std::max(d1, d2) <= 4096 ? center_scratch(s) : nullptr;
    if (!part) {
      center_scale_kernel<T><<<(unsigned)ceil_div(d1, 32), 1024, 0, s>>>((int)n, d1, g1, ldg1, grad_out);
      center_scale_kernel<T><<<(unsigned)ceil_div(d2, 32), 1024, 0, s>>>((int)n, d2, g2, ldg2, grad_out);
      count_launches(2);
      CCAB_CUDA(cudaGetLastError());
      return 0;
    }
    for (int v = 0; v < 2; ++v) {
      T* g = v ? g2 : g1;
      const int d = v ? d2 : d1;
      const int64_t ldg = v ? ldg2 : ldg1;
      double* pv = part + (size_t)v * 32 * 4096;
      colsum_partial_kernel<T><<<dim3((unsigned)ceil_div(d, 32), (unsigned)nslabs), 256, 0, s>>>((int)n, d, g, ldg,
                                                                                                 rows_per_slab, pv);
      center_apply_kernel<T><<<dim3((unsigned)ceil_div(d, 32), 32), 256, 0, s>>>((int)n, d, g, ldg, pv, nslabs, grad_out);
    }
    count_launches(4);
  }
  CCAB_CUDA(cudaGetLastError());
  return 0;
}

template size_t ccaloss_workspace_bytes<float>(const ColumnLayout&, int64_t, int);
template size_t ccaloss_workspace_bytes<double>(const ColumnLayout&, int64_t, int);
template int ccaloss_forward<float>(const ColumnLayout&, int, const void*, int64_t, const void*, int64_t, int64_t, double,
                                    float*, float*, int*, void*, size_t, cudaStream_t);
template int ccaloss_forward<double>(const ColumnLayout&, int, const void*, int64_t, const void*, int64_t, int64_t, double,
                                     double*, double*, int*, void*, size_t, cudaStream_t);
template int ccaloss_backward<float>(int, int, const float*, int64_t, const float*, int64_t, int64_t, const float*,
                                     const float*, float*, int64_t, float*, int64_t, cudaStream_t);
template int ccaloss_backward<double>(int, int, const double*, int64_t, const double*, int64_t, int64_t, const double*,
                                      const double*, double*, int64_t, double*, int64_t, cudaStream_t);

template size_t rcca_fit_workspace_bytes<float>(int, int, int, int);
template size_t rcca_fit_workspace_bytes<double>(int, int, int, int);
template void rcca_fit_result_layout<float>(int, int, int, int, int64_t*);
template void rcca_fit_result_layout<double>(int, int, int, int, int64_t*);
template int rcca_fit<float>(const ColumnLayout&, const double*, const double*, double, int, const double*, int, int, int,
                             void*, size_t, void*, size_t, cudaStream_t);
template int rcca_fit<double>(const ColumnLayout&, const double*, const double*, double, int, const double*, int, int,
                              int, void*, size_t, void*, size_t, cudaStream_t);

}
```

cca_zoo_b200/csrc/fit.cuh:

```cuda
#pragma once
#include "common.cuh"
#include "moments.cuh"

namespace ccab {

constexpr int kFitHeaderDoubles = 32;
constexpr int kFitNotPositiveDefinite = 1;
constexpr int kFitNotConverged = 2;
constexpr int kFitNonFinite = 4;
constexpr int kFitTooFewSamples = 8;

template <typename T>
size_t rcca_fit_workspace_bytes(int d1, int d2, int k, int p);
template <typename T>
void rcca_fit_result_layout(int d1, int d2, int k, int p, int64_t* offsets );
template <typename T>
int rcca_fit(const ColumnLayout& L, const double* moments, const double* n_dev, double n_host, int center,
             const double* c, int k, int p, int iters, void* result, size_t result_bytes, void* ws, size_t ws_bytes,
             cudaStream_t stream);

template <typename T>
size_t mcca_fit_workspace_bytes(const ColumnLayout& L, int k, int p);
template <typename T>
void mcca_fit_result_layout(const ColumnLayout& L, int k, int p, int64_t* offsets);
template <typename T>
int mcca_fit(const ColumnLayout& L, const double* moments, const double* n_dev, double n_host, int center,
             const double* c, double eps_floor, int k, int p, int iters, void* result, size_t result_bytes, void* ws,
             size_t ws_bytes, cudaStream_t stream);

template <typename T>
size_t ccaloss_workspace_bytes(const ColumnLayout& L, int64_t n, int precision);
template <typename T>
int ccaloss_forward(const ColumnLayout& L, int precision, const void* z1, int64_t ld1, const void* z2, int64_t ld2,
                    int64_t n, double eps, T* loss, T* saved, int* flags_out, void* ws, size_t ws_bytes,
                    cudaStream_t stream);
template <typename T>
int ccaloss_backward(int d1, int d2, const T* z1, int64_t ld1, const T* z2, int64_t ld2, int64_t n, const T* saved,
                     const T* grad_out, T* g1, int64_t ldg1, T* g2, int64_t ldg2, cudaStream_t stream);

}
```

cca_zoo_b200/csrc/moments.cu:

```cuda
#include "moments.cuh"

#include <mutex>
#include <type_traits>

namespace ccab {

int make_layout(int n_views, const int64_t* dims, ColumnLayout* L) {
  CCAB_CHECK_ARG(n_views >= 1 && n_views <= kMaxViews, "n_views must be in [1,%d], got %d", kMaxViews,
                 n_views);
  L->n_views = n_views;
  L->coff[0] = 0;
  L->poff[0] = 0;
  int nb = 0;
  for (int v = 0; v < n_views; ++v) {
    CCAB_CHECK_ARG(dims[v] >= 1 && dims[v] <= kMaxBlocks * kBlk, "bad view width %lld", (long long)dims[v]);
    L->dims[v] = (int)dims[v];
    int b = (int)ceil_div(dims[v], kBlk);
    nb += b;
    L->coff[v + 1] = L->coff[v] + (int)dims[v];
    L->poff[v + 1] = L->poff[v] + b * kBlk;
  }
  CCAB_CHECK_ARG(nb <= kMaxBlocks, "total padded width %d exceeds %d", nb * kBlk, kMaxBlocks * kBlk);
  L->nblocks = nb;
  L->D = L->coff[n_views];
  L->Dp = nb * kBlk;
  return 0;
}

static bool g_prof_on = false;
static cudaEvent_t g_prof_e0 = nullptr, g_prof_e1 = nullptr;
static bool g_prof_valid = false;
void moments_profile_enable(int on) {
  g_prof_on = on != 0;
  g_prof_valid = false;
  if (g_prof_on && !g_prof_e0) {
    cudaEventCreate(&g_prof_e0);
    cudaEventCreate(&g_prof_e1);
  }
}
float moments_profile_last_ms() {
  if (!g_prof_valid) return -1.f;
  float ms = -1.f;
  if (cudaEventSynchronize(g_prof_e1) != cudaSuccess) return -1.f;
  if (cudaEventElapsedTime(&ms, g_prof_e0, g_prof_e1) != cudaSuccess) return -1.f;
  return ms;
}

struct WgParams {
  CUtensorMap map[kMaxViews];
  uint8_t blk_view[kMaxBlocks];
  int blk_col0[kMaxBlocks];
  float* partial;
  float* partial_sum;
  int64_t n_rows, rows_per_split;
  int64_t row_base;
  int nblocks, Dp;
};
static_assert(sizeof(WgParams) <= 4096, "kernel parameter space");

constexpr int kWgXpose = 256;
constexpr int kWgThreads = kWgXpose + 256;
constexpr int kWgKC = 32;
constexpr int kWgTile = kBlk * kWgKC * 4;
constexpr int kWgBox = 32 * kWgKC * 4;

__device__ __forceinline__ uint32_t raw_offset(int k, int m) {
  return (uint32_t)(m >> 5) * kWgBox + k128_offset(k, (m & 31) >> 2) + (uint32_t)(m & 3) * 4;
}

enum class K1Mode { TF32, X3 };

template <K1Mode M>
struct WgCfg {
  static constexpr int kOps = M == K1Mode::TF32 ? 1 : 2;
  static constexpr int kOpStage = kOps * kWgTile;
  static constexpr int kRawStage = 2 * kWgTile;
  static constexpr int kOpStages = M == K1Mode::TF32 ? 3 : 2;
  static constexpr int kRawStages = 5;
  static constexpr int kBarOff = kOpStages * kOpStage + kRawStages * kRawStage;
  static constexpr int kSumOff = kBarOff + 2 * (kOpStages + kRawStages) * 8;
  static constexpr int kSmem = kSumOff + kBlk * 4 + 1024;
};
static_assert(WgCfg<K1Mode::X3>::kSmem <= 227 * 1024 && WgCfg<K1Mode::TF32>::kSmem <= 227 * 1024,
              "shared memory per block");
static_assert(WgCfg<K1Mode::X3>::kRawStages > WgCfg<K1Mode::X3>::kOpStages &&
              WgCfg<K1Mode::TF32>::kRawStages > WgCfg<K1Mode::TF32>::kOpStages,
              "the refill of a raw stage must not wait on the MMA warps' current slice");

template <K1Mode M>
__global__ void __launch_bounds__(kWgThreads, 1) moments_wgmma_kernel(const __grid_constant__ WgParams p) {
  using Cfg = WgCfg<M>;
  constexpr bool X3 = M == K1Mode::X3;
  constexpr int NO = Cfg::kOpStages, NR = Cfg::kRawStages;
  extern __shared__ uint8_t smem_raw[];
  uint8_t* smem = smem_raw + ((1024u - (smem_u32(smem_raw) & 1023u)) & 1023u);
  uint8_t* ops = smem;
  uint8_t* raw = smem + NO * Cfg::kOpStage;
  uint64_t* raw_full = reinterpret_cast<uint64_t*>(smem + Cfg::kBarOff);
  uint64_t* raw_empty = raw_full + NR;
  uint64_t* op_full = raw_empty + NR;
  uint64_t* op_empty = op_full + NO;

  int t = blockIdx.x, bi = 0, rowlen = p.nblocks;
  while (t >= rowlen) { t -= rowlen; ++bi; --rowlen; }
  const int bj = bi + t;
  const bool diag = bi == bj;
  const int split = blockIdx.y;
  const int64_t r0 = (int64_t)split * p.rows_per_split;
  const int64_t r1 = min(r0 + p.rows_per_split, p.n_rows);
  const int nch = r1 > r0 ? (int)((r1 - r0 + kWgKC - 1) / kWgKC) : 0;

  if (threadIdx.x == 0) {
    for (int s = 0; s < NR; ++s) {
      mbar_init(&raw_full[s], 1);
      mbar_init(&raw_empty[s], kWgXpose + 8);
    }
    for (int s = 0; s < NO; ++s) {
      mbar_init(&op_full[s], kWgXpose);
      mbar_init(&op_empty[s], 8);
    }
    fence_mbar_init();
  }
  __syncthreads();

  if (threadIdx.x < kWgXpose) {
    setmaxnreg_dec<80>();
    const int m = threadIdx.x % kBlk, h = threadIdx.x / kBlk;
    const CUtensorMap* mapA = &p.map[p.blk_view[bi]];
    const CUtensorMap* mapB = &p.map[p.blk_view[bj]];
    const int colA = p.blk_col0[bi], colB = p.blk_col0[bj];
    auto issue = [&](int c) {
      const int s = c % NR;
      const int row = (int)(p.row_base + r0 + (int64_t)c * kWgKC);
      uint8_t* dst = raw + s * Cfg::kRawStage;
      mbar_arrive_expect_tx(&raw_full[s], diag ? kWgTile : 2 * kWgTile);
#pragma unroll
      for (int q = 0; q < kBlk / 32; ++q) {
        tma_load_2d(dst + q * kWgBox, mapA, &raw_full[s], colA + 32 * q, row);
        if (!diag) tma_load_2d(dst + kWgTile + q * kWgBox, mapB, &raw_full[s], colB + 32 * q, row);
      }
    };
    if (threadIdx.x == 0)
      for (int c = 0; c < min(NR, nch); ++c) issue(c);

    float csum = 0.f;
    auto transpose = [&](const uint8_t* src, uint8_t* hi, uint8_t* lo, bool sums) {
#pragma unroll
      for (int j = 0; j < kWgKC / 8; ++j) {
        const int kg = 2 * j + h;
        float v[4];
#pragma unroll
        for (int e = 0; e < 4; ++e)
          v[e] = *reinterpret_cast<const float*>(src + raw_offset(4 * kg + e, m));
        const uint32_t off = k128_offset(m, kg);
        *reinterpret_cast<float4*>(hi + off) = make_float4(tf32_hi(v[0]), tf32_hi(v[1]), tf32_hi(v[2]), tf32_hi(v[3]));
        if (X3)
          *reinterpret_cast<float4*>(lo + off) = make_float4(tf32_residual(v[0]), tf32_residual(v[1]),
                                                             tf32_residual(v[2]), tf32_residual(v[3]));
        if (sums) csum += (v[0] + v[1]) + (v[2] + v[3]);
      }
    };
    for (int c = 0; c < nch; ++c) {
      const int sr = c % NR, so = c % NO;
      mbar_wait(&raw_full[sr], (c / NR) & 1);
      mbar_wait(&op_empty[so], ((c / NO) & 1) ^ 1);
      uint8_t* dst = ops + so * Cfg::kOpStage;
      transpose(raw + sr * Cfg::kRawStage + (diag ? 0 : kWgTile), dst, dst + kWgTile, diag);
      fence_proxy_async_smem();
      mbar_arrive(&raw_empty[sr]);
      mbar_arrive(&op_full[so]);
      const int rf = c + NR - NO + 1;
      if (threadIdx.x == 0 && rf >= NR && rf < nch) {
        mbar_wait(&raw_empty[rf % NR], (rf / NR - 1) & 1);
        issue(rf);
      }
    }
    if (diag) {
      float* odd = reinterpret_cast<float*>(smem + Cfg::kSumOff);
      if (h) odd[m] = csum;
      asm volatile("bar.sync 1, %0;" ::"n"(kWgXpose) : "memory");
      if (!h) p.partial_sum[(size_t)split * p.Dp + bi * kBlk + m] = csum + odd[m];
    }
  } else {
    setmaxnreg_inc<168>();
    const int wg = (threadIdx.x - kWgXpose) >> 7, lane = threadIdx.x & 31, t = lane & 3;
    const int m = wg * 64 + ((threadIdx.x >> 5) & 3) * 16 + (lane >> 2);
    const int kx = t ^ ((t & 1) << 2);
    const bool swap = t & 1;
    const uint32_t o00 = raw_offset(kx, m), o01 = raw_offset(kx ^ 4, m);
    const uint32_t o10 = raw_offset(kx, m + 8), o11 = raw_offset(kx ^ 4, m + 8);
    float acc[64];
#pragma unroll
    for (int i = 0; i < 64; ++i) acc[i] = 0.f;
    wgmma_fence_regs<64>(acc);
    constexpr int KS = kWgKC / 8;
    constexpr int KR = Cfg::kOps * 4;
    uint32_t fa[KS][KR] = {};
    for (int c = 0; c < nch; ++c) {
      const int sr = c % NR, so = c % NO;
      mbar_wait(&raw_full[sr], (c / NR) & 1);
      const uint8_t* a_src = raw + sr * Cfg::kRawStage;
      const uint32_t b0 = smem_u32(ops + so * Cfg::kOpStage);
#pragma unroll
      for (int kk = 0; kk < KS; ++kk) {
        wgmma_wait<KS - 1>();
        wgmma_fence_regs<KR>(fa[kk]);
        if (kk == KS - 1 && c > 0 && lane == 0) mbar_arrive(&op_empty[(c - 1) % NO]);
        {
          const uint8_t* s = a_src + kk * 1024;
          const float v00 = *reinterpret_cast<const float*>(s + o00), v01 = *reinterpret_cast<const float*>(s + o01);
          const float v10 = *reinterpret_cast<const float*>(s + o10), v11 = *reinterpret_cast<const float*>(s + o11);
          const float a[4] = {swap ? v01 : v00, swap ? v11 : v10, swap ? v00 : v01, swap ? v10 : v11};
#pragma unroll
          for (int i = 0; i < 4; ++i) {
            fa[kk][i] = __float_as_uint(tf32_hi(a[i]));
            if constexpr (X3) fa[kk][4 + i] = __float_as_uint(tf32_residual(a[i]));
          }
        }
        wgmma_fence_regs<KR>(fa[kk]);
        if (kk == KS - 1) {
          __syncwarp();
          if (lane == 0) mbar_arrive(&raw_empty[sr]);
        }
        if (kk == 0) mbar_wait(&op_full[so], (c / NO) & 1);
        wgmma_fence();
        const uint64_t b_hi = wgmma_desc_k128(b0 + 32 * kk);
        if constexpr (X3) {
          const uint64_t b_lo = wgmma_desc_k128(b0 + kWgTile + 32 * kk);
          wgmma_tf32_ra<128>(acc, &fa[kk][4], b_hi);
          wgmma_tf32_ra<128>(acc, &fa[kk][0], b_lo);
        }
        wgmma_tf32_ra<128>(acc, &fa[kk][0], b_hi);
        wgmma_commit();
      }
    }
    wgmma_wait_all();
    wgmma_fence_regs<64>(acc);

    const int warp = (threadIdx.x >> 5) & 3;
    float* P = p.partial + (size_t)split * p.Dp * p.Dp;
    const int row0 = bi * kBlk + wg * 64 + warp * 16 + (lane >> 2);
    const int col0 = bj * kBlk + 2 * (lane & 3);
#pragma unroll
    for (int r = 0; r < 64; r += 2) {
      const int row = row0 + 8 * ((r >> 1) & 1), col = col0 + 8 * (r >> 2);
      *reinterpret_cast<float2*>(P + (size_t)row * p.Dp + col) = make_float2(acc[r], acc[r + 1]);
    }
  }
}

constexpr int kPrXpose = 128;
constexpr int kPrThreads = kPrXpose + 256;
struct PairCfg {
  static constexpr int kOpStage = 2 * kWgTile;
  static constexpr int kRawStage = 3 * kWgTile;
  static constexpr int kOpStages = 2;
  static constexpr int kRawStages = 3;
  static constexpr int kFrag = 4;
  static constexpr int kBarOff = kOpStages * kOpStage + kRawStages * kRawStage;
  static constexpr int kSmem = kBarOff + 2 * (kOpStages + kRawStages) * 8 + 1024;
  static constexpr int kXposeRegs = 56, kMmaRegs = 224;
};
static_assert(PairCfg::kSmem <= 227 * 1024, "shared memory per block");
static_assert(PairCfg::kRawStages > PairCfg::kOpStages,
              "the refill of a raw stage must not wait on the MMA warps' current slice");
static_assert(kPrXpose * PairCfg::kXposeRegs + 256 * PairCfg::kMmaRegs <= kPrThreads * (65536 / kPrThreads / 8 * 8),
              "the register budgets must fit in what the CTA is allocated at launch");
static_assert(4 % PairCfg::kFrag == 0, "a slice is four steps");

inline int pair_tiles(int nblocks) {
  int n = 0;
  for (int i = 0; 2 * i < nblocks; ++i) n += nblocks - 2 * i;
  return n;
}

__global__ void __launch_bounds__(kPrThreads, 1) moments_x3b_pair_kernel(const __grid_constant__ WgParams p) {
  constexpr int NO = PairCfg::kOpStages, NR = PairCfg::kRawStages, NF = PairCfg::kFrag;
  extern __shared__ uint8_t smem_raw[];
  uint8_t* smem = smem_raw + ((1024u - (smem_u32(smem_raw) & 1023u)) & 1023u);
  uint8_t* ops = smem;
  uint8_t* raw = smem + NO * PairCfg::kOpStage;
  uint64_t* raw_full = reinterpret_cast<uint64_t*>(smem + PairCfg::kBarOff);
  uint64_t* raw_empty = raw_full + NR;
  uint64_t* op_full = raw_empty + NR;
  uint64_t* op_empty = op_full + NO;

  int t = blockIdx.x, i = 0, rowlen = p.nblocks;
  while (t >= rowlen) { t -= rowlen; ++i; rowlen -= 2; }
  const int a0 = 2 * i, bj = a0 + t;
  const int nload = min(t, 2) + 1;
  const int na = min(nload, 2);
  const int bslot = nload - 1;
  const bool diag = t < 2;
  const int split = blockIdx.y;
  const int64_t r0 = (int64_t)split * p.rows_per_split;
  const int64_t r1 = min(r0 + p.rows_per_split, p.n_rows);
  const int nch = r1 > r0 ? (int)((r1 - r0 + kWgKC - 1) / kWgKC) : 0;

  if (threadIdx.x == 0) {
    for (int s = 0; s < NR; ++s) {
      mbar_init(&raw_full[s], 1);
      mbar_init(&raw_empty[s], kPrXpose + 4 * na);
    }
    for (int s = 0; s < NO; ++s) {
      mbar_init(&op_full[s], kPrXpose);
      mbar_init(&op_empty[s], 4 * na);
    }
    fence_mbar_init();
  }
  __syncthreads();

  if (threadIdx.x < kPrXpose) {
    setmaxnreg_dec<PairCfg::kXposeRegs>();
    const int m = threadIdx.x;
    auto issue = [&](int c) {
      const int s = c % NR;
      const int row = (int)(p.row_base + r0 + (int64_t)c * kWgKC);
      uint8_t* dst = raw + s * PairCfg::kRawStage;
      mbar_arrive_expect_tx(&raw_full[s], nload * kWgTile);
      for (int b = 0; b < nload; ++b) {
        const int blk = b < 2 ? a0 + b : bj;
        const CUtensorMap* map = &p.map[p.blk_view[blk]];
#pragma unroll
        for (int q = 0; q < kBlk / 32; ++q)
          tma_load_2d(dst + b * kWgTile + q * kWgBox, map, &raw_full[s], p.blk_col0[blk] + 32 * q, row);
      }
    };
    if (threadIdx.x == 0)
      for (int c = 0; c < min(NR, nch); ++c) issue(c);

    float csum[2] = {0.f, 0.f};
    for (int c = 0; c < nch; ++c) {
      const int sr = c % NR, so = c % NO;
      mbar_wait(&raw_full[sr], (c / NR) & 1);
      mbar_wait(&op_empty[so], ((c / NO) & 1) ^ 1);
      const uint8_t* src = raw + sr * PairCfg::kRawStage + bslot * kWgTile;
      uint8_t* hi = ops + so * PairCfg::kOpStage;
      uint8_t* lo = hi + kWgTile;
#pragma unroll
      for (int e = 0; e < 4; ++e) {
        float v[8], x[8];
#pragma unroll
        for (int k = 0; k < 8; ++k) {
          v[k] = *reinterpret_cast<const float*>(src + raw_offset(8 * e + k, m));
          x[k] = tf32_hi(v[k]);
        }
        *reinterpret_cast<float4*>(hi + k128_offset(m, 2 * e)) = make_float4(x[0], x[1], x[2], x[3]);
        *reinterpret_cast<float4*>(hi + k128_offset(m, 2 * e + 1)) = make_float4(x[4], x[5], x[6], x[7]);
        *reinterpret_cast<uint4*>(lo + k128_offset(m, e)) =
            make_uint4(pack_bf16x2(x[0], x[4]), pack_bf16x2(x[1], x[5]), pack_bf16x2(x[2], x[6]),
                       pack_bf16x2(x[3], x[7]));
        *reinterpret_cast<uint4*>(lo + k128_offset(m, 4 + e)) =
            make_uint4(pack_bf16x2(v[0] - x[0], v[4] - x[4]), pack_bf16x2(v[1] - x[1], v[5] - x[5]),
                       pack_bf16x2(v[2] - x[2], v[6] - x[6]), pack_bf16x2(v[3] - x[3], v[7] - x[7]));
        if (diag) csum[e >> 1] += ((v[0] + v[1]) + (v[2] + v[3])) + ((v[4] + v[5]) + (v[6] + v[7]));
      }
      fence_proxy_async_smem();
      mbar_arrive(&raw_empty[sr]);
      mbar_arrive(&op_full[so]);
      const int rf = c + NR - NO + 1;
      if (threadIdx.x == 0 && rf >= NR && rf < nch) {
        mbar_wait(&raw_empty[rf % NR], (rf / NR - 1) & 1);
        issue(rf);
      }
    }
    if (diag) p.partial_sum[(size_t)split * p.Dp + bj * kBlk + m] = csum[0] + csum[1];
  } else {
    setmaxnreg_inc<PairCfg::kMmaRegs>();
    const int g = (threadIdx.x - kPrXpose) >> 7;
    if (g >= na) return;
    const int lane = threadIdx.x & 31, t4 = lane & 3, warp = (threadIdx.x >> 5) & 3;
    const int m = warp * 16 + (lane >> 2);
    const int kx = t4 ^ ((t4 & 1) << 2);
    const bool swap = t4 & 1;
    const uint32_t o00 = raw_offset(kx, m), o01 = raw_offset(kx ^ 4, m);
    const uint32_t o10 = raw_offset(kx, m + 8), o11 = raw_offset(kx ^ 4, m + 8);
    float acc[2][64];
#pragma unroll
    for (int r = 0; r < 2; ++r) {
#pragma unroll
      for (int k = 0; k < 64; ++k) acc[r][k] = 0.f;
      wgmma_fence_regs<64>(acc[r]);
    }
    uint32_t fa[NF][16] = {};
    for (int c = 0; c < nch; ++c) {
      const int sr = c % NR, so = c % NO;
      mbar_wait(&raw_full[sr], (c / NR) & 1);
      const uint8_t* a_src = raw + sr * PairCfg::kRawStage + g * kWgTile;
      const uint32_t b0 = smem_u32(ops + so * PairCfg::kOpStage);
#pragma unroll
      for (int s = 0; s < 4; ++s) {
        const int kk = s >> 1, r = s & 1, f = s % NF;
        wgmma_wait<NF - 1>();
        wgmma_fence_regs<16>(fa[f]);
        if (s == NF - 1 && c > 0 && lane == 0) mbar_arrive(&op_empty[(c - 1) % NO]);
#pragma unroll
        for (int q = 0; q < 2; ++q) {
          const uint8_t* src = a_src + (2 * kk + q) * 1024 + r * 2 * kWgBox;
          const float v00 = *reinterpret_cast<const float*>(src + o00), v01 = *reinterpret_cast<const float*>(src + o01);
          const float v10 = *reinterpret_cast<const float*>(src + o10), v11 = *reinterpret_cast<const float*>(src + o11);
          const float a[4] = {swap ? v01 : v00, swap ? v11 : v10, swap ? v00 : v01, swap ? v10 : v11};
          float x[4];
#pragma unroll
          for (int k = 0; k < 4; ++k) {
            x[k] = tf32_hi(a[k]);
            fa[f][4 * q + k] = __float_as_uint(x[k]);
          }
#pragma unroll
          for (int h = 0; h < 2; ++h) {
            fa[f][8 + 2 * q + h] = pack_bf16x2(x[h], x[h + 2]);
            fa[f][12 + 2 * q + h] = pack_bf16x2(a[h] - x[h], a[h + 2] - x[h + 2]);
          }
        }
        wgmma_fence_regs<16>(fa[f]);
        if (s == 3) {
          __syncwarp();
          if (lane == 0) mbar_arrive(&raw_empty[sr]);
        }
        if (s == 0) mbar_wait(&op_full[so], (c / NO) & 1);
        wgmma_fence();
        wgmma_bf16_ra<128>(acc[r], &fa[f][12], wgmma_desc_k128(b0 + kWgTile + 32 * kk));
        wgmma_bf16_ra<128>(acc[r], &fa[f][8], wgmma_desc_k128(b0 + kWgTile + 64 + 32 * kk));
        wgmma_tf32_ra<128>(acc[r], &fa[f][0], wgmma_desc_k128(b0 + 64 * kk));
        wgmma_tf32_ra<128>(acc[r], &fa[f][4], wgmma_desc_k128(b0 + 64 * kk + 32));
        wgmma_commit();
      }
    }
    wgmma_wait_all();
    wgmma_fence_regs<64>(acc[0]);
    wgmma_fence_regs<64>(acc[1]);

    float* P = p.partial + (size_t)split * p.Dp * p.Dp;
    const int col0 = bj * kBlk + 2 * t4;
#pragma unroll
    for (int r = 0; r < 2; ++r) {
      const int row0 = (a0 + g) * kBlk + r * 64 + m;
#pragma unroll
      for (int k = 0; k < 64; k += 2) {
        const int row = row0 + 8 * ((k >> 1) & 1), col = col0 + 8 * (k >> 2);
        *reinterpret_cast<float2*>(P + (size_t)row * p.Dp + col) = make_float2(acc[r][k], acc[r][k + 1]);
      }
// ... 60 lines not shown
      fold_sum[i] += (double)csum[i];
      csum[i] = T(0);
#pragma unroll
      for (int j = 0; j < 4; ++j) {
        fold[i][j] += (double)acc[i][j];
        acc[i][j] = T(0);
      }
    }
  };

  const int lc = threadIdx.x & 63, lr = threadIdx.x >> 6;
  for (int64_t r = r0; r < r1; r += KC) {
    if (r > r0 && (r - r0) % kRun == 0) fold_run();
#pragma unroll
    for (int i = 0; i < KC / 4; ++i) {
      const int kr = lr + 4 * i;
      const int64_t row = r + kr;
      const bool rv = row < r1;
      As[kr][lc] = (rv && cA + lc < dA) ? XA[row * ldA + cA + lc] : T(0);
      Bs[kr][lc] = (rv && cB + lc < dB) ? XB[row * ldB + cB + lc] : T(0);
    }
    __syncthreads();
#pragma unroll
    for (int k = 0; k < KC; ++k) {
      T a[4], b[4];
#pragma unroll
      for (int i = 0; i < 4; ++i) { a[i] = As[k][ty * 4 + i]; b[i] = Bs[k][tx * 4 + i]; }
#pragma unroll
      for (int i = 0; i < 4; ++i)
#pragma unroll
        for (int j = 0; j < 4; ++j) acc[i][j] = fma(a[i], b[j], acc[i][j]);
      if (ty == 0) {
#pragma unroll
        for (int j = 0; j < 4; ++j) csum[j] += b[j];
      }
    }
    __syncthreads();
  }
  fold_run();
  T* P = static_cast<T*>(p.partial) + (size_t)split * p.Dp * p.Dp;
#pragma unroll
  for (int i = 0; i < 4; ++i)
#pragma unroll
    for (int j = 0; j < 4; ++j)
      P[(size_t)(bi * 64 + ty * 4 + i) * p.Dp + bj * 64 + tx * 4 + j] = (T)fold[i][j];
  if (bi == bj && ty == 0) {
    T* S = static_cast<T*>(p.partial_sum) + (size_t)split * p.Dp;
#pragma unroll
    for (int j = 0; j < 4; ++j) S[bi * 64 + tx * 4 + j] = (T)fold_sum[j];
  }
}

__device__ __forceinline__ void dmma_m8n8k4(double& c0, double& c1, double a, double b) {
  asm volatile("mma.sync.aligned.m8n8k4.row.col.f64.f64.f64.f64 {%0, %1}, {%2}, {%3}, {%0, %1};"
               : "+d"(c0), "+d"(c1)
               : "d"(a), "d"(b));
}

__global__ void __launch_bounds__(256) moments_dmma_kernel(const SimtParams p) {
  constexpr int KC = 16;
  constexpr int LDS = 64 + 4;
  __shared__ double As[2][KC][LDS];
  __shared__ double Bs[2][KC][LDS];
  int t = blockIdx.x, bi = 0, rowlen = p.nb64;
  while (t >= rowlen) { t -= rowlen; ++bi; --rowlen; }
  const int bj = bi + t;
  const int split = blockIdx.y;
  const int64_t r0 = split * p.rows_per_split;
  const int64_t r1 = min(r0 + p.rows_per_split, p.n_rows);

  auto locate = [&](int pcol0, int& v, int& c0) {
    v = 0;
    while (v + 1 < p.n_views && p.view_poff[v + 1] <= pcol0) ++v;
    c0 = pcol0 - p.view_poff[v];
  };
  int vA, cA, vB, cB;
  locate(bi * 64, vA, cA);
  locate(bj * 64, vB, cB);
  const double* XA = static_cast<const double*>(p.view_ptr[vA]);
  const double* XB = static_cast<const double*>(p.view_ptr[vB]);
  const int64_t ldA = p.view_ld[vA], ldB = p.view_ld[vB];
  const int dA = p.view_dim[vA], dB = p.view_dim[vB];

  const int warp = threadIdx.x >> 5, lane = threadIdx.x & 31;
  const int wm = (warp & 1) * 32, wn = (warp >> 1) * 16;
  const int gq = lane >> 2, tq = lane & 3;
  double acc[4][2][2];
#pragma unroll
  for (int i = 0; i < 4; ++i)
#pragma unroll
    for (int j = 0; j < 2; ++j) acc[i][j][0] = acc[i][j][1] = 0.0;
  double csum = 0.0;

  const int lc = threadIdx.x & 63, lr = threadIdx.x >> 6;
  double ra[KC / 4], rb[KC / 4];
  auto gload = [&](int64_t r) {
#pragma unroll
    for (int i = 0; i < KC / 4; ++i) {
      const int64_t row = r + lr + 4 * i;
      const bool rv = row < r1;
      ra[i] = (rv && cA + lc < dA) ? XA[row * ldA + cA + lc] : 0.0;
      rb[i] = (rv && cB + lc < dB) ? XB[row * ldB + cB + lc] : 0.0;
    }
  };
  auto sstore = [&](int buf) {
#pragma unroll
    for (int i = 0; i < KC / 4; ++i) {
      As[buf][lr + 4 * i][lc] = ra[i];
      Bs[buf][lr + 4 * i][lc] = rb[i];
    }
  };
  gload(r0);
  sstore(0);
  __syncthreads();
  int buf = 0;
  for (int64_t r = r0; r < r1; r += KC, buf ^= 1) {
    const bool more = r + KC < r1;
    if (more) gload(r + KC);
#pragma unroll
    for (int k0 = 0; k0 < KC; k0 += 4) {
      double a[4], b[2];
#pragma unroll
      for (int i = 0; i < 4; ++i) a[i] = As[buf][k0 + tq][wm + 8 * i + gq];
#pragma unroll
      for (int j = 0; j < 2; ++j) b[j] = Bs[buf][k0 + tq][wn + 8 * j + gq];
#pragma unroll
      for (int i = 0; i < 4; ++i)
#pragma unroll
        for (int j = 0; j < 2; ++j) dmma_m8n8k4(acc[i][j][0], acc[i][j][1], a[i], b[j]);
    }
    if (bi == bj && threadIdx.x < 64) {
#pragma unroll
      for (int k = 0; k < KC; ++k) csum += Bs[buf][k][threadIdx.x];
    }
    if (more) sstore(buf ^ 1);
    __syncthreads();
  }
  double* P = static_cast<double*>(p.partial) + (size_t)split * p.Dp * p.Dp;
#pragma unroll
  for (int i = 0; i < 4; ++i)
#pragma unroll
    for (int j = 0; j < 2; ++j) {
      const int row = bi * 64 + wm + 8 * i + gq;
      const int col = bj * 64 + wn + 8 * j + 2 * tq;
      *reinterpret_cast<double2*>(P + (size_t)row * p.Dp + col) = make_double2(acc[i][j][0], acc[i][j][1]);
    }
  if (bi == bj && threadIdx.x < 64)
    static_cast<double*>(p.partial_sum)[(size_t)split * p.Dp + bi * 64 + threadIdx.x] = csum;
}

template <typename T>
__global__ void reduce_partials_kernel(const T* __restrict__ partial, const T* __restrict__ partial_sum,
                                       int S, int Dp, int ldp, int blk, double* __restrict__ out,
                                       int accumulate = 0) {
  const size_t total = (size_t)Dp * Dp + (partial_sum ? Dp : 0);
  const size_t slab = (size_t)ldp * ldp;
  for (size_t i = blockIdx.x * (size_t)blockDim.x + threadIdx.x; i < total;
       i += (size_t)gridDim.x * blockDim.x) {
    double acc = 0.0;
    if (i < (size_t)Dp * Dp) {
      const int r = (int)(i / Dp), c = (int)(i % Dp);
      if (r / blk <= c / blk) {
        const T* src = partial + (size_t)r * ldp + c;
        int s = 0;
        for (; s + 8 <= S; s += 8) {
          T v[8];
#pragma unroll
          for (int u = 0; u < 8; ++u) v[u] = src[(size_t)(s + u) * slab];
#pragma unroll
          for (int u = 0; u < 8; ++u) acc += (double)v[u];
        }
        for (; s < S; ++s) acc += (double)src[(size_t)s * slab];
      }
    } else {
      const size_t j = i - (size_t)Dp * Dp;
      for (int s = 0; s < S; ++s) acc += (double)partial_sum[(size_t)s * ldp + j];
    }
    out[i] = accumulate ? out[i] + acc : acc;
  }
}

struct CovParams {
  int n_views, D, Dp;
  int dims[kMaxViews];
  int coff[kMaxViews + 1];
  int poff[kMaxViews + 1];
};

__device__ __forceinline__ int compact_to_padded(const CovParams& p, int g) {
  int v = 0;
  while (v + 1 < p.n_views && p.coff[v + 1] <= g) ++v;
  return p.poff[v] + (g - p.coff[v]);
}

template <typename Tout>
__global__ void covariance_kernel(const CovParams p, const double* __restrict__ mom, double n_total,
                                  int center, Tout* __restrict__ C, int64_t ldc, Tout* __restrict__ mean) {
  const double* M = mom;
  const double* s = mom + (size_t)p.Dp * p.Dp;
  const int gi = blockIdx.y * blockDim.y + threadIdx.y;
  const int gj = blockIdx.x * blockDim.x + threadIdx.x;
  if (gi >= p.D || gj >= p.D) return;
  const int pi = compact_to_padded(p, gi), pj = compact_to_padded(p, gj);
  const int r = min(pi, pj), c = max(pi, pj);
  double v = M[(size_t)r * p.Dp + c];
  if (center) v -= s[pi] * s[pj] / n_total;
  C[(size_t)gi * ldc + gj] = (Tout)(v / (n_total - 1.0));
  if (gi == 0 && mean) mean[gj] = (Tout)(center ? s[pj] / n_total : 0.0);
}

namespace {

int sm_count() {
  static int n[64] = {};
  int dev = 0;
  cudaGetDevice(&dev);
  if (dev < 0 || dev >= 64) return 132;
  if (!n[dev]) {
    cudaDeviceGetAttribute(&n[dev], cudaDevAttrMultiProcessorCount, dev);
    if (n[dev] <= 0) n[dev] = 132;
  }
  return n[dev];
}

struct TcPlan {
  int total_chunks, num_splits, chunks_per_split, ntiles;
  size_t partial_bytes, sum_bytes;
};

TcPlan plan_tc(const ColumnLayout& L, int64_t n_rows, int mode) {
  const bool x3 = mode != 0;
  TcPlan P;
  P.total_chunks = (int)ceil_div(n_rows, kWgKC);
  P.ntiles = L.nblocks * (L.nblocks + 1) / 2;
  int S = (int)ceil_div(4 * sm_count(), P.ntiles);
  int max_splits = 64;
  if (x3) {
    S = std::max<int64_t>(S, ceil_div(n_rows, 2048));
    max_splits = 256;
  }
  const int min_chunks = 8;
  S = (int)std::min<int64_t>(S, std::max<int64_t>(1, P.total_chunks / min_chunks));
  const int64_t slab = (int64_t)L.Dp * L.Dp * (int64_t)sizeof(float);
  max_splits = (int)std::max<int64_t>(1, std::min<int64_t>(max_splits, ((int64_t)2 << 30) / slab));
  S = std::min(S, max_splits);
  S = std::max(1, std::min(S, P.total_chunks));
  P.chunks_per_split = (int)ceil_div(P.total_chunks, S);
  P.num_splits = (int)ceil_div(P.total_chunks, P.chunks_per_split);
  P.partial_bytes = (size_t)P.num_splits * L.Dp * L.Dp * sizeof(float);
  P.sum_bytes = (size_t)P.num_splits * L.Dp * sizeof(float);
  return P;
}

int64_t tc_rows_cap(const ColumnLayout& L, int mode) {
  if (mode == 0) return (int64_t)1 << 31;
  const int64_t slab = (int64_t)L.Dp * L.Dp * (int64_t)sizeof(float);
  const int64_t max_splits = std::max<int64_t>(1, std::min<int64_t>(256, ((int64_t)2 << 30) / slab));
  return max_splits * 2048;
}

inline size_t align256(size_t x) { return (x + 255) & ~size_t(255); }

struct SimtPlan {
  int nb64, ntiles, num_splits;
  int64_t rows_per_split;
};

SimtPlan plan_simt(const ColumnLayout& L, int64_t n_rows) {
  SimtPlan P;
  P.nb64 = L.Dp / 64;
  P.ntiles = P.nb64 * (P.nb64 + 1) / 2;
  int S = 1;
  if (P.ntiles < 2 * sm_count()) S = (2 * sm_count()) / P.ntiles;
  S = (int)std::min<int64_t>(S, std::max<int64_t>(1, n_rows / 64));
  S = std::max(1, std::min(S, 64));
  P.rows_per_split = ceil_div(ceil_div(n_rows, S), 16) * 16;
  P.num_splits = (int)ceil_div(n_rows, P.rows_per_split);
  return P;
}

}

size_t moments_workspace_bytes(int dtype, int precision, const ColumnLayout& L, int64_t n_rows) {
  if (precision == 2 || dtype == 1) {
    SimtPlan P = plan_simt(L, n_rows);
    size_t el = dtype == 1 ? 8 : 4;
    return align256((size_t)P.num_splits * L.Dp * L.Dp * el) + align256((size_t)P.num_splits * L.Dp * el);
  }
  TcPlan P = plan_tc(L, std::min(n_rows, tc_rows_cap(L, precision)), precision);
  return align256(P.partial_bytes) + align256(P.sum_bytes) + 256;
}

namespace {

typedef CUresult (*EncodeTiledFn)(CUtensorMap*, CUtensorMapDataType, cuuint32_t, void*, const cuuint64_t*,
                                  const cuuint64_t*, const cuuint32_t*, const cuuint32_t*, CUtensorMapInterleave,
                                  CUtensorMapSwizzle, CUtensorMapL2promotion, CUtensorMapFloatOOBfill);

EncodeTiledFn encode_fn() {
  static EncodeTiledFn fn = nullptr;
  static std::once_flag once;
  std::call_once(once, [] {
    void* f = nullptr;
    cudaDriverEntryPointQueryResult q;
    if (cudaGetDriverEntryPoint("cuTensorMapEncodeTiled", &f, cudaEnableDefault, &q) == cudaSuccess &&
        q == cudaDriverEntryPointSuccess)
      fn = reinterpret_cast<EncodeTiledFn>(f);
  });
  return fn;
}

int encode_view_map(CUtensorMap* map, const void* ptr, int64_t n_rows, int64_t d, int64_t ld) {
  EncodeTiledFn enc = encode_fn();
  if (!enc) {
    set_error("cuTensorMapEncodeTiled entry point not available (driver too old?)");
    return -2;
  }
  cuuint64_t gdim[2] = {(cuuint64_t)d, (cuuint64_t)n_rows};
  cuuint64_t gstride[1] = {(cuuint64_t)ld * 4};
  cuuint32_t box[2] = {32, (cuuint32_t)kWgKC};
  cuuint32_t estr[2] = {1, 1};
  CUresult r = enc(map, CU_TENSOR_MAP_DATA_TYPE_FLOAT32, 2, const_cast<void*>(ptr), gdim, gstride, box, estr,
                   CU_TENSOR_MAP_INTERLEAVE_NONE, CU_TENSOR_MAP_SWIZZLE_128B, CU_TENSOR_MAP_L2_PROMOTION_L2_256B,
                   CU_TENSOR_MAP_FLOAT_OOB_FILL_NONE);
  if (r != CUDA_SUCCESS) {
    set_error("cuTensorMapEncodeTiled failed with CUresult %d (d=%lld n=%lld ld=%lld)", (int)r, (long long)d,
              (long long)n_rows, (long long)ld);
    return -3;
  }
  return 0;
}

int moments_tf32_pass(const ColumnLayout& L, WgParams& prm, int64_t row_base, int64_t n_rows, int mode,
                      double* moments_out, void* ws, size_t ws_bytes, cudaStream_t stream, int accumulate);

}

int moments_tf32(const ColumnLayout& L, const void* const* views, const int64_t* lds, int64_t n_rows, int mode,
                 double* moments_out, void* ws, size_t ws_bytes, cudaStream_t stream) {
  CCAB_CHECK_ARG(n_rows >= 1 && n_rows < (int64_t)1 << 31, "n_rows out of range");
  for (int v = 0; v < L.n_views; ++v)
    CCAB_CHECK_ARG((reinterpret_cast<uintptr_t>(views[v]) & 15) == 0 && lds[v] % 4 == 0,
                   "TF32 moments need 16-byte aligned views and lds %% 4 == 0 (view %d: ld %lld)", v,
                   (long long)lds[v]);
  {
    int dev = 0;
    CCAB_CUDA(cudaGetDevice(&dev));
    CCAB_CUDA(cudaSetDevice(dev));
  }
  WgParams prm;
  memset(&prm, 0, sizeof(prm));
  for (int v = 0; v < L.n_views; ++v) {
    int rc = encode_view_map(&prm.map[v], views[v], n_rows, L.dims[v], lds[v]);
    if (rc) return rc;
  }
  int b = 0;
  for (int v = 0; v < L.n_views; ++v)
    for (int c = 0; c < L.dims[v]; c += kBlk, ++b) {
      prm.blk_view[b] = (uint8_t)v;
      prm.blk_col0[b] = c;
    }
  const int64_t cap = tc_rows_cap(L, mode);
  if (n_rows <= cap) return moments_tf32_pass(L, prm, 0, n_rows, mode, moments_out, ws, ws_bytes, stream, 0);
  const int64_t npass = ceil_div(n_rows, cap);
  const int64_t per = std::min(cap, ceil_div(ceil_div(n_rows, npass), 2048) * 2048);
  int pass = 0;
  for (int64_t r0 = 0; r0 < n_rows; r0 += per, ++pass) {
    int rc = moments_tf32_pass(L, prm, r0, std::min(per, n_rows - r0), mode, moments_out, ws, ws_bytes, stream,
                               pass > 0);
    if (rc) return rc;
  }
  return 0;
}

namespace {
template <K1Mode M>
int launch_wgmma(dim3 grid, const WgParams& prm, cudaStream_t stream) {
  CCAB_CUDA(cudaFuncSetAttribute(moments_wgmma_kernel<M>, cudaFuncAttributeMaxDynamicSharedMemorySize,
                                 WgCfg<M>::kSmem));
  moments_wgmma_kernel<M><<<grid, kWgThreads, WgCfg<M>::kSmem, stream>>>(prm);
  return 0;
}

int launch_x3b_pair(int num_splits, const WgParams& prm, cudaStream_t stream) {
  CCAB_CUDA(cudaFuncSetAttribute(moments_x3b_pair_kernel, cudaFuncAttributeMaxDynamicSharedMemorySize,
                                 PairCfg::kSmem));
  moments_x3b_pair_kernel<<<dim3(pair_tiles(prm.nblocks), num_splits), kPrThreads, PairCfg::kSmem, stream>>>(prm);
  return 0;
}

int moments_tf32_pass(const ColumnLayout& L, WgParams& prm, int64_t row_base, int64_t n_rows, int mode,
                      double* moments_out, void* ws, size_t ws_bytes, cudaStream_t stream, int accumulate) {
  TcPlan P = plan_tc(L, n_rows, mode);
  const size_t need = align256(P.partial_bytes) + align256(P.sum_bytes) + 256;
  CCAB_CHECK_ARG(ws_bytes >= need, "workspace too small: %zu < %zu", ws_bytes, need);
  uint8_t* w = reinterpret_cast<uint8_t*>((reinterpret_cast<uintptr_t>(ws) + 255) & ~uintptr_t(255));
  float* d_partial = reinterpret_cast<float*>(w);
  float* d_partial_sum = reinterpret_cast<float*>(w + align256(P.partial_bytes));

  prm.partial = d_partial;
  prm.partial_sum = d_partial_sum;
  prm.n_rows = n_rows;
  prm.rows_per_split = (int64_t)P.chunks_per_split * kWgKC;
  prm.row_base = row_base;
  prm.nblocks = L.nblocks;
  prm.Dp = L.Dp;
  dim3 grid(P.ntiles, P.num_splits);
  if (g_prof_on) cudaEventRecord(g_prof_e0, stream);
  int rc = mode == 3   ? launch_x3b_pair(P.num_splits, prm, stream)
           : mode != 0 ? launch_wgmma<K1Mode::X3>(grid, prm, stream)
                       : launch_wgmma<K1Mode::TF32>(grid, prm, stream);
  if (rc) return rc;
  count_launches(1);
  CCAB_CUDA(cudaGetLastError());
  if (g_prof_on) {
    cudaEventRecord(g_prof_e1, stream);
    g_prof_valid = true;
  }

  const size_t total = (size_t)L.Dp * L.Dp + L.Dp;
  int rblocks = (int)std::min<size_t>((total + 255) / 256, (size_t)sm_count() * 8);
  reduce_partials_kernel<float><<<rblocks, 256, 0, stream>>>(d_partial, d_partial_sum, P.num_splits, L.Dp, L.Dp,
                                                            kBlk, moments_out, accumulate); count_launches(1);
  CCAB_CUDA(cudaGetLastError());
  return 0;
}
}

template <typename T>
int moments_simt(const ColumnLayout& L, const void* const* views, const int64_t* lds, int64_t n_rows,
                 double* moments_out, void* ws, size_t ws_bytes, cudaStream_t stream) {
  CCAB_CHECK_ARG(n_rows >= 1, "n_rows must be positive");
  SimtPlan P = plan_simt(L, n_rows);
  const size_t pb = align256((size_t)P.num_splits * L.Dp * L.Dp * sizeof(T));
  const size_t sb = align256((size_t)P.num_splits * L.Dp * sizeof(T));
  CCAB_CHECK_ARG(ws_bytes >= pb + sb, "workspace too small: %zu < %zu", ws_bytes, pb + sb);
  uint8_t* w = static_cast<uint8_t*>(ws);
  SimtParams prm;
  memset(&prm, 0, sizeof(prm));
  for (int v = 0; v < L.n_views; ++v) {
    prm.view_ptr[v] = views[v];
    prm.view_ld[v] = lds[v];
    prm.view_dim[v] = L.dims[v];
  }
  for (int v = 0; v <= L.n_views; ++v) prm.view_poff[v] = L.poff[v];
  prm.n_views = L.n_views;
  prm.n_rows = n_rows;
  prm.rows_per_split = P.rows_per_split;
  prm.nb64 = P.nb64;
  prm.Dp = L.Dp;
  prm.partial = w;
  prm.partial_sum = w + pb;
  dim3 grid(P.ntiles, P.num_splits);
  if constexpr (std::is_same<T, double>::value)
    moments_dmma_kernel<<<grid, 256, 0, stream>>>(prm);
  else
    moments_simt_kernel<T><<<grid, 256, 0, stream>>>(prm);
  count_launches(1);
  CCAB_CUDA(cudaGetLastError());
  const size_t total = (size_t)L.Dp * L.Dp + L.Dp;
  int rblocks = (int)std::min<size_t>((total + 255) / 256, (size_t)sm_count() * 8);
  reduce_partials_kernel<T><<<rblocks, 256, 0, stream>>>(static_cast<const T*>(prm.partial),
                                                        static_cast<const T*>(prm.partial_sum), P.num_splits,
                                                        L.Dp, L.Dp, 64, moments_out); count_launches(1);
  CCAB_CUDA(cudaGetLastError());
  return 0;
}

template int moments_simt<float>(const ColumnLayout&, const void* const*, const int64_t*, int64_t, double*, void*,
                                 size_t, cudaStream_t);
template int moments_simt<double>(const ColumnLayout&, const void* const*, const int64_t*, int64_t, double*, void*,
                                  size_t, cudaStream_t);

__global__ void pack_moments_kernel(const double* __restrict__ mom, int nblocks, int Dp, double n_local,
                                    double* __restrict__ packed) {
  const int nt = nblocks * (nblocks + 1) / 2;
  const int t = blockIdx.x;
  if (t < nt) {
    int bi = 0, rem = t, rowlen = nblocks;
    while (rem >= rowlen) { rem -= rowlen; ++bi; --rowlen; }
    const int bj = bi + rem;
    const double* src = mom + (size_t)bi * kBlk * Dp + (size_t)bj * kBlk;
    double* dst = packed + (size_t)t * kBlk * kBlk;
    for (int e = threadIdx.x; e < kBlk * kBlk; e += blockDim.x) dst[e] = src[(size_t)(e / kBlk) * Dp + (e % kBlk)];
  } else {
    double* dst = packed + (size_t)nt * kBlk * kBlk;
    const double* s = mom + (size_t)Dp * Dp;
    for (int e = threadIdx.x; e < Dp; e += blockDim.x) dst[e] = s[e];
    if (threadIdx.x == 0) { dst[Dp] = n_local; dst[Dp + 1] = 0.0; }
  }
}

__global__ void unpack_moments_kernel(const double* __restrict__ packed, int nblocks, int Dp, double* __restrict__ mom) {
  const int nt = nblocks * (nblocks + 1) / 2;
  const int bi = blockIdx.y, bj = blockIdx.x;
  if (bi < nblocks) {
    double* dst = mom + (size_t)bi * kBlk * Dp + (size_t)bj * kBlk;
    if (bj >= bi) {
      const int t = bi * nblocks - bi * (bi - 1) / 2 + (bj - bi);
      const double* src = packed + (size_t)t * kBlk * kBlk;
      for (int e = threadIdx.x; e < kBlk * kBlk; e += blockDim.x) dst[(size_t)(e / kBlk) * Dp + (e % kBlk)] = src[e];
    } else {
      for (int e = threadIdx.x; e < kBlk * kBlk; e += blockDim.x) dst[(size_t)(e / kBlk) * Dp + (e % kBlk)] = 0.0;
    }
  } else if (bj == 0) {
    const double* src = packed + (size_t)nt * kBlk * kBlk;
    double* s = mom + (size_t)Dp * Dp;
    for (int e = threadIdx.x; e < Dp; e += blockDim.x) s[e] = src[e];
  }
}

__device__ __forceinline__ double multimem_ld_reduce_add_f64(const double* mc_addr) {
  double v;
  asm volatile("multimem.ld_reduce.relaxed.sys.global.add.f64 %0, [%1];" : "=d"(v) : "l"(mc_addr) : "memory");
  return v;
}
__device__ __forceinline__ void multimem_st_f64(double* mc_addr, double v) {
  asm volatile("multimem.st.relaxed.sys.global.f64 [%0], %1;" ::"l"(mc_addr), "d"(v) : "memory");
}
__device__ __forceinline__ void st_release_sys_u32(uint32_t* p, uint32_t v) {
  asm volatile("st.release.sys.global.u32 [%0], %1;" ::"l"(p), "r"(v) : "memory");
}
__device__ __forceinline__ uint32_t ld_acquire_sys_u32(const uint32_t* p) {
  uint32_t v;
  asm volatile("ld.acquire.sys.global.u32 %0, [%1];" : "=r"(v) : "l"(p) : "memory");
  return v;
}

struct ExchangeParams {
  double* mom;
  double* sym;
  double* mc;
  uint32_t* const* pads;
  double* n_total_out;
  double n_local;
  long long packed;
  long long chunk;
  int rank, world, nblocks, Dp;
  unsigned epoch;
};

__device__ __forceinline__ const double* packed_src(const ExchangeParams& p, long long e, int nt) {
  const long long blk = e / (kBlk * kBlk);
  if (blk < nt) {
    int bi = 0, rem = (int)blk, rowlen = p.nblocks;
    while (rem >= rowlen) { rem -= rowlen; ++bi; --rowlen; }
    const int bj = bi + rem;
    const int off = (int)(e - blk * (kBlk * kBlk));
    return p.mom + ((size_t)bi * kBlk + off / kBlk) * p.Dp + (size_t)bj * kBlk + (off % kBlk);
  }
  const long long t = e - (long long)nt * kBlk * kBlk;
  return t < p.Dp ? p.mom + (size_t)p.Dp * p.Dp + t : nullptr;
}

__device__ __forceinline__ void exchange_barrier(const ExchangeParams& p, unsigned value) {
  __threadfence_system();
  __syncthreads();
  if ((int)threadIdx.x < p.world)
    st_release_sys_u32(p.pads[threadIdx.x] + (size_t)blockIdx.x * p.world + p.rank, value);
  if ((int)threadIdx.x < p.world) {
    const uint32_t* slot = p.pads[p.rank] + (size_t)blockIdx.x * p.world + threadIdx.x;
    unsigned spins = 0;
    while ((int)(ld_acquire_sys_u32(slot) - value) < 0) {
      if (++spins > (1u << 26)) {
        printf("ccab: exchange barrier timed out (rank %d cta %d peer %d)\n", p.rank, blockIdx.x, threadIdx.x);
        __trap();
      }
    }
  }
  __syncthreads();
}

__global__ void __launch_bounds__(512) exchange_nvls_kernel(const ExchangeParams p) {
  const int nt = p.nblocks * (p.nblocks + 1) / 2;
  const long long sub = (p.chunk + gridDim.x - 1) / gridDim.x;
  const long long r0 = (long long)blockIdx.x * sub;
// ... 217 lines not shown
```

cca_zoo_b200/csrc/moments.cuh:

```cuda
#pragma once
#include "common.cuh"

namespace ccab {

constexpr int kMaxViews = 8;
constexpr int kBlk = 128;
constexpr int kMaxBlocks = 128;

struct ColumnLayout {
  int n_views;
  int nblocks;
  int D;
  int Dp;
  int dims[kMaxViews];
  int coff[kMaxViews + 1];
  int poff[kMaxViews + 1];
};

int make_layout(int n_views, const int64_t* dims, ColumnLayout* out);

size_t moments_workspace_bytes(int dtype, int precision, const ColumnLayout& L, int64_t n_rows);

int moments_tf32(const ColumnLayout& L, const void* const* views, const int64_t* lds, int64_t n_rows,
                 int mode , double* moments_out, void* ws, size_t ws_bytes, cudaStream_t stream);

template <typename T>
int moments_simt(const ColumnLayout& L, const void* const* views, const int64_t* lds, int64_t n_rows,
                 double* moments_out, void* ws, size_t ws_bytes, cudaStream_t stream);

template <typename Tout>
int covariance_from_moments(const ColumnLayout& L, const double* moments, double n_total, int center,
                            Tout* C, int64_t ldc, Tout* mean, cudaStream_t stream);

int64_t moments_packed_size(const ColumnLayout& L);
int moments_pack(const ColumnLayout& L, const double* moments, double n_local, double* packed, cudaStream_t stream);
int moments_unpack(const ColumnLayout& L, const double* packed, double* moments, cudaStream_t stream);

template <typename T>
int column_pilot(const T* X, int64_t rows, int d, int64_t ld, T* x0, float* ratio_max, cudaStream_t stream);
template <typename T>
int shift_rows(const T* X, int64_t n, int d, int64_t ldx, const T* x0, T* Xs, int64_t lds, cudaStream_t stream);
int moments_unshift(const ColumnLayout& L, double* moments, const void* const* x0, int is_f64, double n,
                    cudaStream_t stream);

int moments_exchange_nvls(const ColumnLayout& L, double* moments, double n_local, double* sym_local,
                          double* sym_multicast, void* const* pads_dev, int rank, int world, int pad_slots,
                          int64_t sym_doubles, unsigned epoch, double* n_total_out, cudaStream_t stream);

void moments_profile_enable(int on);
float moments_profile_last_ms();

}
```

cca_zoo_b200/linear/_rcca.py:

```python
from __future__ import annotations

import os

from numbers import Real
from typing import Any, ClassVar

from sklearn.utils._param_validation import Interval, StrOptions

from .._base import BaseModel
from .. import ops
from ..ops import rcca_fit_workspace_bytes
from .._solvers import rcca_weights
from .._validation import perview_parameter, validate_views

RIDGE_PARAMETER: list[Any] = [Interval(Real, 0, 1, closed="both"), "array-like"]


class rCCA(BaseModel):

    _requires_two_views = True
    _parameter_constraints: ClassVar[dict[str, list[Any]]] = {
        **BaseModel._parameter_constraints,
        "c": RIDGE_PARAMETER,
        "solver": [StrOptions({"auto", "eigen", "cholesky"})],
    }

    def __init__(self, latent_dimensions: int = 1, center: bool = True, c=0.0, precision: str = "tf32x3b",
                 device=None, solver: str = "auto") -> None:
        super().__init__(latent_dimensions=latent_dimensions, center=center, precision=precision, device=device)
        self.c = c
        self.solver = solver

    def fit(self, views, y=None):
        self._validate_params()
        validated = validate_views(views)
        device = self._device()
        mom, n_local, dims, in_dtype = self._local_moments(validated, device)
        self._partial = None
        if len(dims) != 2:
            raise ValueError(
                f"rCCA requires exactly 2 views, got {len(dims)}. "
                "Use MCCA for more than 2 views."
            )
        return self._fit_moments(mom, n_local, dims, in_dtype)

    def _device_fit_plan(self, dims, n_local, in_dtype):
        if self.solver == "eigen":
            return None
        if self.solver == "auto" and not (min(dims) >= 256 and n_local > max(dims)):
            return None
        k = min(int(self.latent_dimensions), dims[0], dims[1])
        over = int(os.environ.get("CCAB_FIT_OVERSAMPLE", "0")) or max(16, k // 4)
        p = min(min(dims), k + over)
        if 4 * k > min(dims) or rcca_fit_workspace_bytes(dims, k, p, self._solve_dtype(in_dtype)) == 0:
            return None
        first = int(os.environ.get("CCAB_FIT_ITERS", "0")) or 6
        c_ = [float(x) for x in perview_parameter("c", self.c, 0.0, 2)]
        center = bool(self.center)

        def call(mom, dims_, n_host, n_dev, solve_dtype, iters):
            return ops.rcca_fit(mom, dims_, n_host, n_dev, center, c_, k, p, iters, solve_dtype)

        return {"call": call, "k": k, "iters": [first, 20]}

    def _solve(self, C, dims, n_total):
        c_ = perview_parameter("c", self.c, 0.0, 2)
        return rcca_weights(C, dims, n_total, self.latent_dimensions, [float(x) for x in c_], solver=self.solver)


class CCA(rCCA):

    def __init__(self, latent_dimensions: int = 1, center: bool = True, precision: str = "tf32x3b",
                 device=None) -> None:
        super().__init__(latent_dimensions=latent_dimensions, center=center, c=0.0, precision=precision,
                         device=device, solver="auto")


class PLS(rCCA):

    def __init__(self, latent_dimensions: int = 1, center: bool = True, precision: str = "tf32x3b",
                 device=None) -> None:
        super().__init__(latent_dimensions=latent_dimensions, center=center, c=1.0, precision=precision,
                         device=device, solver="auto")
```

cca_zoo_b200/ops.py:

```python
from __future__ import annotations

import ctypes as C

import torch

from . import _lib

_DT = {torch.float32: _lib.F32, torch.float64: _lib.F64}


def _require_cuda(t: torch.Tensor, name: str) -> None:
    if not t.is_cuda:
        raise RuntimeError(
            f"{name} must be a CUDA tensor: cca_zoo_b200 runs on sm_90a only and has no CPU fallback"
        )


def _stream(t: torch.Tensor):
    return C.c_void_p(torch.cuda.current_stream(t.device).cuda_stream)


def _ptr(t):
    return C.c_void_p(0 if t is None else t.data_ptr())

# ... 292 lines not shown
    if batched and B.shape[0] != batch:
        raise ValueError("gemm_tc: batch sizes differ")
    m, k = (A.shape[-1], A.shape[-2]) if transa else (A.shape[-2], A.shape[-1])
    k2, n = (B.shape[-1], B.shape[-2]) if transb else (B.shape[-2], B.shape[-1])
    if k != k2:
        raise ValueError(f"gemm inner dimensions differ: {k} vs {k2}")
    shape = (batch, m, n) if batched else (m, n)
    shape_t = (batch, n, m) if batched else (n, m)
    if out is None and want_c:
        out = torch.empty(shape, dtype=A.dtype, device=A.device)
        beta = 0.0
    for t, shp, nm in ((out, shape, "out"), (out_t, shape_t, "out_t")):
        if t is not None and (tuple(t.shape) != shp or t.stride(-1) != 1 or t.dtype != A.dtype or t.device != A.device):
            raise ValueError(f"gemm_tc `{nm}` must be a row-major {shp} float32 tensor on {A.device}")
    if out is None and out_t is None:
        raise ValueError("gemm_tc: no output requested")
    sa = A.stride(0) if batched else 0
    sb = B.stride(0) if batched else 0
    with torch.cuda.device(A.device):
        rc = lib.ccab_gemm_tc(int(transa), int(transb), m, n, k, float(alpha), _ptr(A), A.stride(-2), sa, _ptr(B),
                              B.stride(-2), sb, float(beta), _ptr(out), 0 if out is None else out.stride(-2),
                              (out.stride(0) if (batched and out is not None) else 0), _ptr(out_t),
                              0 if out_t is None else out_t.stride(-2),
                              (out_t.stride(0) if (batched and out_t is not None) else 0), batch, int(lower_only),
                              _stream(A))
    _lib.check(rc, "ccab_gemm_tc")
    return out if want_c else out_t


def gemm_batched(A, B, transa=False, transb=False, alpha=1.0):
    if _tc_ok(A) and _tc_ok(B):
        return gemm_tc(A, B, transa=transa, transb=transb, alpha=alpha)
    return torch.stack([gemm(A[i], B[i], transa=transa, transb=transb, alpha=alpha) for i in range(A.shape[0])])


def whiten_rows(lam, Vt, c, floor_add=0.0, floor_dev=None, scale=1.0, rank_tol=0.0, max_rank=None,
                lam_floor=-1e300):
    lib = _lib.load()
    _require_cuda(Vt, "Vt")
    d = Vt.shape[0]
    Wt = torch.empty_like(Vt)
    g = torch.empty(d, dtype=Vt.dtype, device=Vt.device)
    rank = torch.zeros(1, dtype=torch.int32, device=Vt.device)
    with torch.cuda.device(Vt.device):
        rc = lib.ccab_whiten_rows(_DT[Vt.dtype], d, _ptr(lam), _ptr(Vt), Vt.stride(0), float(c), float(floor_add),
                                  _ptr(floor_dev), float(scale), float(rank_tol),
                                  int(d if max_rank is None else max_rank), float(lam_floor), _ptr(Wt), Wt.stride(0),
                                  _ptr(g),
                                  _ptr(rank), _stream(Vt))
    _lib.check(rc, "ccab_whiten_rows")
    return Wt, g, rank


def ccaloss_small(Cm, d1, d2, eps):
    lib = _lib.load()
    _require_cuda(Cm, "C")
    dev, dt = Cm.device, Cm.dtype
    loss = torch.empty(1, dtype=dt, device=dev)
    minp = torch.empty(1, dtype=dt, device=dev)
    G11 = torch.empty((d1, d1), dtype=dt, device=dev)
    P = torch.empty((d1, d2), dtype=dt, device=dev)
    G22 = torch.empty((d2, d2), dtype=dt, device=dev)
    with torch.cuda.device(dev):
        rc = lib.ccab_ccaloss_small(_DT[dt], d1, d2, _ptr(Cm), Cm.stride(0), float(eps), _ptr(loss), _ptr(G11), _ptr(P),
                                    _ptr(G22), _ptr(minp), _stream(Cm))
    _lib.check(rc, "ccab_ccaloss_small")
    return loss, G11, P, G22, minp


def ccaloss_fwd(z1, z2, eps, precision="exact"):
    lib = _lib.load()
    _require_cuda(z1, "z1")
    _require_cuda(z2, "z2")
    n, d1, d2 = z1.shape[0], z1.shape[1], z2.shape[1]
    dt = _DT[z1.dtype]
    prec = {"tf32": _lib.PREC_TF32, "tf32x3": _lib.PREC_TF32X3, "exact": _lib.PREC_EXACT,
            "tf32x3b": _lib.PREC_TF32X3B}[precision]
    if z1.dtype == torch.float64:
        prec = _lib.PREC_EXACT
    loss = torch.empty(1, dtype=z1.dtype, device=z1.device)
    saved = torch.empty(d1 * d1 + d1 * d2 + d2 * d2 + d1 + d2, dtype=z1.dtype, device=z1.device)
    flags = torch.empty(3, dtype=torch.int32, device=z1.device)
    ws = _ws(lib.ccab_ccaloss_workspace_bytes(dt, prec, d1, d2, n), z1.device)
    with torch.cuda.device(z1.device):
        rc = lib.ccab_ccaloss_fwd(dt, prec, _ptr(z1), z1.stride(0), _ptr(z2), z2.stride(0), n, d1, d2, float(eps),
                                  _ptr(loss), _ptr(saved), _ptr(flags), _ptr(ws), ws.numel(), _stream(z1))
    _lib.check(rc, "ccab_ccaloss_fwd")
    return loss, saved, flags


def ccaloss_bwd(z1, z2, saved, grad_out):
    lib = _lib.load()
    n, d1, d2 = z1.shape[0], z1.shape[1], z2.shape[1]
    g1 = torch.empty((n, d1), dtype=z1.dtype, device=z1.device)
    g2 = torch.empty((n, d2), dtype=z1.dtype, device=z1.device)
    with torch.cuda.device(z1.device):
        rc = lib.ccab_ccaloss_bwd(_DT[z1.dtype], _ptr(z1), z1.stride(0), _ptr(z2), z2.stride(0), n, d1, d2, _ptr(saved),
                                  _ptr(grad_out), _ptr(g1), d1, _ptr(g2), d2, _stream(z1))
    _lib.check(rc, "ccab_ccaloss_bwd")
    return g1, g2


def potrf_inv_(A, pivot_tol=0.0):
    lib = _lib.load()
    _require_cuda(A, "A")
    squeeze = A.dim() == 2
    Ab = A.unsqueeze(0) if squeeze else A
    if Ab.dim() != 3 or Ab.shape[1] != Ab.shape[2] or Ab.stride(2) != 1 or Ab.dtype not in _DT:
        raise ValueError("square row-major float32/float64 matrices expected")
    batch, n, _ = Ab.shape
    Linv = torch.empty((batch, n, n), dtype=A.dtype, device=A.device)
    info = torch.empty(batch, dtype=torch.int32, device=A.device)
    dt = _DT[A.dtype]
    ws = _ws(lib.ccab_potrf_inv_workspace_bytes(dt, n, batch), A.device)
    with torch.cuda.device(A.device):
        rc = lib.ccab_potrf_inv(dt, n, batch, _ptr(Ab), Ab.stride(1), Ab.stride(0) if batch > 1 else 0, _ptr(Linv), n,
                                n * n, float(pivot_tol), _ptr(info), _ptr(ws), ws.numel(), _stream(A))
    _lib.check(rc, "ccab_potrf_inv")
    return (Linv[0] if squeeze else Linv), info


FIT_NOT_POSITIVE_DEFINITE, FIT_NOT_CONVERGED, FIT_NON_FINITE, FIT_TOO_FEW_SAMPLES = 1, 2, 4, 8
FIT_HEADER_DOUBLES = 32


def rcca_fit_workspace_bytes(dims, k: int, p: int, dtype) -> int:
    return int(_lib.load().ccab_rcca_fit_workspace_bytes(_DT[dtype], _lib.i64_array(dims), int(k), int(p)))


def mcca_fit_workspace_bytes(dims, k: int, p: int, dtype) -> int:
    return int(_lib.load().ccab_mcca_fit_workspace_bytes(_DT[dtype], len(dims), _lib.i64_array(dims), int(k), int(p)))


def rcca_fit(mom: torch.Tensor, dims, n_host, n_dev, center: bool, c, k: int, p: int, iters: int, dtype):
    lib = _lib.load()
    _require_cuda(mom, "moments")
    dt = _DT[dtype]
    d = _lib.i64_array(dims)
    offs = (C.c_int64 * 5)()
    _lib.check(lib.ccab_rcca_fit_result_layout(dt, d, int(k), int(p), offs), "ccab_rcca_fit_result_layout")
    offsets = [int(x) for x in offs]
    block = torch.empty(offsets[4] + 256, dtype=torch.uint8, device=mom.device)
    shift = (-block.data_ptr()) % 256
    block = block[shift:shift + offsets[4]]
    wsb = lib.ccab_rcca_fit_workspace_bytes(dt, d, int(k), int(p))
    ws = _ws(wsb, mom.device)
    cc = (C.c_double * 2)(float(c[0]), float(c[1]))
    with torch.cuda.device(mom.device):
        rc = lib.ccab_rcca_fit(dt, d, _ptr(mom), _ptr(n_dev), float(n_host if n_host is not None else 0.0),
                               1 if center else 0, cc, int(k), int(p), int(iters), _ptr(block), block.numel(), _ptr(ws),
                               ws.numel(), _stream(mom))
    _lib.check(rc, "ccab_rcca_fit")
    return block, offsets


def mcca_fit(mom: torch.Tensor, dims, n_host, n_dev, center: bool, c, eps: float, k: int, p: int, iters: int, dtype):
    lib = _lib.load()
    _require_cuda(mom, "moments")
    dt = _DT[dtype]
    m = len(dims)
    d = _lib.i64_array(dims)
    offs = (C.c_int64 * (m + 3))()
    _lib.check(lib.ccab_mcca_fit_result_layout(dt, m, d, int(k), int(p), offs), "ccab_mcca_fit_result_layout")
    offsets = [int(x) for x in offs]
    block = torch.empty(offsets[-1] + 256, dtype=torch.uint8, device=mom.device)
    shift = (-block.data_ptr()) % 256
    block = block[shift:shift + offsets[-1]]
    ws = _ws(lib.ccab_mcca_fit_workspace_bytes(dt, m, d, int(k), int(p)), mom.device)
    cc = (C.c_double * m)(*[float(x) for x in c])
    with torch.cuda.device(mom.device):
        rc = lib.ccab_mcca_fit(dt, m, d, _ptr(mom), _ptr(n_dev), float(n_host if n_host is not None else 0.0),
                               1 if center else 0, cc, float(eps), int(k), int(p), int(iters), _ptr(block),
                               block.numel(), _ptr(ws), ws.numel(), _stream(mom))
    _lib.check(rc, "ccab_mcca_fit")
    return block, offsets


def decode_fit_block(host: torch.Tensor, offsets, dims, k: int, dtype):
    import numpy as np

    buf = host.numpy()
    np_dt = np.float32 if dtype == torch.float32 else np.float64
    D = int(sum(dims))
    hdr = buf[:8 * FIT_HEADER_DOUBLES].view(np.float64)
    mean = buf[offsets[0]:offsets[0] + 8 * D].view(np.float64)
    sig = buf[offsets[1]:offsets[1] + np_dt().itemsize * k].view(np_dt)
    ws = []
    for i, d in enumerate(dims):
        o = offsets[2 + i]
        ws.append(buf[o:o + np_dt().itemsize * d * k].view(np_dt).reshape(d, k))
    return hdr, mean, sig, ws


def column_means(mom: torch.Tensor, dims, n_total: float):
    import numpy as np

    pads = [(int(p) + 127) // 128 * 128 for p in dims]
    Dp = sum(pads)
    sums = mom[Dp * Dp:Dp * Dp + Dp].to(torch.float64).cpu().numpy()
    off = np.concatenate([[0], np.cumsum(pads)]).astype(int)
    return np.concatenate([sums[off[i]:off[i] + int(p)] for i, p in enumerate(dims)]) / float(n_total)


ALS_KINDS = {"pls": 0, "pmd": 1, "parkhomenko": 2, "span": 3, "admm": 4, "elastic": 5, "ipls": 6}


ALS_RCOND_F64 = 1e-12


def als_fit(cov, dims, n_total, kind: str, params, init, max_iter: int, tol: float, mu: float | None = None):
    import numpy as np

    lib = _lib.load()
    _require_cuda(cov, "cov")
    if cov.dtype != torch.float64:
        raise ValueError("als_fit iterates in float64")
    cov = cov.contiguous()
    D, k = int(sum(dims)), int(init.shape[0])
    d = _lib.i64_array(dims)
    init = torch.as_tensor(init, dtype=torch.float64).to(cov.device).contiguous()
    out = torch.empty(D * k + (k + 1) // 2, dtype=torch.float64, device=cov.device)
    regression = kind in ("elastic", "ipls")
    if mu is None:
        mu = ALS_RCOND_F64 if regression else 1.0
    ws_bytes = (lib.ccab_als_regression_workspace_bytes if regression else lib.ccab_als_fit_workspace_bytes)(len(dims), d)
    ws = _ws(ws_bytes, cov.device)
    if regression:
        want = 2 * len(dims) + (D if kind == "ipls" else 0)
        if len(params) != want:
            raise ValueError(f"als_fit({kind!r}) takes {want} params, got {len(params)}")
    pp = (C.c_double * max(len(params), len(dims)))(*[float(x) for x in params])
    with torch.cuda.device(cov.device):
        rc = lib.ccab_als_fit(ALS_KINDS[kind], len(dims), d, _ptr(cov), float(n_total - 1), float(n_total), pp,
                              float(mu), _ptr(init), k, int(max_iter), float(tol), _ptr(out),
                              C.c_void_p(out.data_ptr() + 8 * D * k), _ptr(ws), ws.numel(), _stream(cov))
    _lib.check(rc, "ccab_als_fit")
    host = out.cpu().numpy()
    iters = host[D * k:].view(np.int32)[:k].astype(int).tolist()
    capped = [d for d, it in enumerate(iters) if it < 0]
    if capped:
        import warnings

        from sklearn.exceptions import ConvergenceWarning

        warnings.warn(f"als_fit({kind!r}): a coordinate descent of latent dimension(s) {capped} stopped at its sweep "
                      "limit above the KKT bound (1e-12 max(1, ||b||_inf)); consider a larger alpha",
                      ConvergenceWarning, stacklevel=2)
    return host[:D * k].reshape(D, k).copy(), [abs(it) for it in iters]


EY_HEADER = 8
EY_MAX_K = 32


class EyFit:

    def __init__(self, dims, init, c, learning_rate, momentum, tol, cov=None, views=None, batch=0):
        import numpy as np

        self.lib = _lib.load()
        self.dims = [int(d) for d in dims]
        self.D, self.k = int(sum(self.dims)), int(init.shape[1])
        self.hyper = (float(c), float(learning_rate), float(momentum), float(tol))
        self.cov, self.batch = cov, int(batch) if cov is None else 0
        ref = cov if cov is not None else views[0]
        _require_cuda(ref, "cov" if cov is not None else "view")
        self.device = ref.device
        self._d = _lib.i64_array(self.dims)
        if cov is not None:
            if cov.dtype != torch.float64 or tuple(cov.shape) != (self.D, self.D):
                raise ValueError("the covariance route takes the float64 D x D covariance")
            self.cov = cov.contiguous()
            self._views, self._ld, self.dtype = None, None, _lib.F64
        else:
            for v in views:
                _require_cuda(v, "view")
                if v.dtype != views[0].dtype or v.dtype not in _DT or v.stride(1) != 1 or v.device != self.device:
                    raise ValueError("the mini-batch route takes CUDA views of one dtype with unit column stride")
            self.views = views
            self._views = (C.c_void_p * len(views))(*[v.data_ptr() for v in views])
            self._ld = _lib.i64_array([v.stride(0) for v in views])
            self.dtype = _DT[views[0].dtype]
        nbytes = self.lib.ccab_ey_fit_workspace_bytes(len(self.dims), self._d, self.k, self.batch)
        if nbytes == 0:
            raise ValueError(f"ccab_ey_fit does not support widths {self.dims} with k = {self.k} (1 <= k <= "
                             f"{EY_MAX_K}, 2 to {_lib.MAX_VIEWS} views) and batch = {self.batch}")
        self.ws = _ws(nbytes, self.device)
        host = np.zeros(EY_HEADER + 2 * self.D * self.k)
        host[0] = np.inf
        host[EY_HEADER:EY_HEADER + self.D * self.k] = np.asarray(init, dtype=np.float64).T.reshape(-1)
        self.state = torch.from_numpy(host).to(self.device)
        self._flag = torch.empty(1, dtype=torch.float64, pin_memory=True)

    def run(self, n_steps: int, idx=None):
        c, lr, mom, tol = self.hyper
        with torch.cuda.device(self.device):
            rc = self.lib.ccab_ey_fit(len(self.dims), self._d, self.k, c, lr, mom, tol, int(n_steps),
                                      _ptr(self.cov), self.dtype, self._views, self._ld, self.batch, _ptr(idx),
                                      _ptr(self.state), _ptr(self.ws), self.ws.numel(),
                                      C.c_void_p(torch.cuda.current_stream(self.device).cuda_stream))
        _lib.check(rc, "ccab_ey_fit")

    def stopped(self) -> bool:
        self._flag.copy_(self.state[2:3])
        return bool(self._flag[0] != 0.0)

# ... 159 lines not shown
```

include/ccab200.h:

```cpp
#ifndef CCAB200_H
#define CCAB200_H

#include <stddef.h>
#include <stdint.h>

#ifdef __cplusplus
extern "C" {
#endif

#define CCAB_F32 0
#define CCAB_F64 1

#define CCAB_PREC_TF32 0
#define CCAB_PREC_TF32X3 1
#define CCAB_PREC_EXACT 2
#define CCAB_PREC_TF32X3B 3

#define CCAB_MAX_VIEWS 8

int ccab_version(void);
const char* ccab_last_error(void);
int64_t ccab_launch_count(void);

int64_t ccab_moments_size(int n_views, const int64_t* dims);
int64_t ccab_moments_padded_dim(int n_views, const int64_t* dims);
size_t ccab_moments_workspace_bytes(int dtype, int precision, int n_views, const int64_t* dims, int64_t n_rows);
int ccab_moments(int dtype, int precision, int n_views, const void* const* views, const int64_t* dims,
                 const int64_t* lds, int64_t n_rows, double* moments, void* workspace, size_t workspace_bytes,
                 void* stream);

int ccab_column_pilot(int dtype, const void* X, int64_t rows, int d, int64_t ld, void* x0, float* ratio_max_dev,
                      void* stream);
int ccab_shift_rows(int dtype, const void* X, int64_t n, int d, int64_t ldx, const void* x0, void* Xs, int64_t lds,
                    void* stream);
int ccab_moments_unshift(int dtype, int n_views, const int64_t* dims, double* moments, const void* const* x0,
                         double n_rows, void* stream);

int64_t ccab_moments_packed_size(int n_views, const int64_t* dims);
int ccab_moments_pack(int n_views, const int64_t* dims, const double* moments, double n_local, double* packed,
                      void* stream);
int ccab_moments_unpack(int n_views, const int64_t* dims, const double* packed, double* moments, void* stream);

int ccab_moments_exchange_nvls(int n_views, const int64_t* dims, double* moments, double n_local, double* sym_local,
                               double* sym_multicast, void* const* signal_pads_dev, int rank, int world,
                               int pad_slots, int64_t sym_doubles, unsigned epoch, double* n_total_out, void* stream);

int ccab_covariance(int out_dtype, int n_views, const int64_t* dims, const double* moments, double n_total,
                    int center, void* C, int64_t ldc, void* mean, void* stream);

size_t ccab_syevj_workspace_bytes(int dtype, int n, int batch);
int ccab_syevj(int dtype, int n, int batch, const void* A, int64_t lda, int64_t batch_stride, double shift,
               void* evals, void* evecs_t, int64_t ldv, int* info, float* info_offdiag, void* workspace,
               size_t workspace_bytes, void* stream);

int ccab_syevj_small(int dtype, int n, int batch, const void* A, int64_t lda, int64_t stride_a, void* evals,
                     void* evecs_t, int64_t ldv, int* info_dev, void* stream);

size_t ccab_gesvj_workspace_bytes(int dtype, int m, int n);
int ccab_gesvj(int dtype, int m, int n, const void* A, int64_t lda, void* sigma, void* right_t, int64_t ldr,
               void* left_t, int64_t ldl, int* info, float* info_offdiag, void* workspace, size_t workspace_bytes,
               void* stream);

int ccab_gemm(int dtype, int transa, int transb, int m, int n, int k, double alpha, const void* A, int64_t lda,
              const void* B, int64_t ldb, double beta, void* C, int64_t ldc, void* stream);

int ccab_gemm_tc(int transa, int transb, int m, int n, int k, double alpha, const void* A, int64_t lda,
                 int64_t stride_a, const void* B, int64_t ldb, int64_t stride_b, double beta, void* C, int64_t ldc,
                 int64_t stride_c, void* Ct, int64_t ldct, int64_t stride_ct, int batch, int lower_only,
                 void* stream);

int ccab_whiten_rows(int dtype, int d, const void* lam, const void* Vt, int64_t ldv, double c, double floor_add,
                     const void* floor_dev, double scale, double rank_tol, int max_rank, double lam_floor, void* Wt,
                     int64_t ldw, void* g_out, int* rank_out, void* stream);

int ccab_ccaloss_small(int dtype, int d1, int d2, const void* C, int64_t ldc, double eps, void* loss, void* G11,
                       void* P, void* G22, void* min_pivot, void* stream);

size_t ccab_potrf_inv_workspace_bytes(int dtype, int n, int batch);
int ccab_potrf_inv(int dtype, int n, int batch, void* A, int64_t lda, int64_t stride_a, void* Linv, int64_t ldi,
                   int64_t stride_i, double pivot_tol, int* info_dev, void* workspace, size_t workspace_bytes,
                   void* stream);

size_t ccab_rcca_fit_workspace_bytes(int dtype, const int64_t* dims, int k, int p);
int ccab_rcca_fit_result_layout(int dtype, const int64_t* dims, int k, int p, int64_t* offsets );
int ccab_rcca_fit(int dtype, const int64_t* dims, const double* moments, const double* n_total_dev, double n_total,
                  int center, const double* c, int k, int p, int iters, void* result, size_t result_bytes,
                  void* workspace, size_t workspace_bytes, void* stream);

size_t ccab_mcca_fit_workspace_bytes(int dtype, int n_views, const int64_t* dims, int k, int p);
int ccab_mcca_fit_result_layout(int dtype, int n_views, const int64_t* dims, int k, int p, int64_t* offsets);
int ccab_mcca_fit(int dtype, int n_views, const int64_t* dims, const double* moments, const double* n_total_dev,
                  double n_total, int center, const double* c, double eps, int k, int p, int iters, void* result,
                  size_t result_bytes, void* workspace, size_t workspace_bytes, void* stream);

#define CCAB_ALS_PLS 0
#define CCAB_ALS_PMD 1
#define CCAB_ALS_PARKHOMENKO 2
#define CCAB_ALS_SPAN 3
#define CCAB_ALS_ADMM 4
#define CCAB_ALS_ELASTIC 5
#define CCAB_ALS_IPLS 6
size_t ccab_als_fit_workspace_bytes(int n_views, const int64_t* dims);
size_t ccab_als_regression_workspace_bytes(int n_views, const int64_t* dims);
int ccab_als_fit(int kind, int n_views, const int64_t* dims, const double* G, double g_scale, double n_samples,
                 const double* params, double mu, const double* init, int k, int max_iter, double tol, double* W_out,
                 int* iters_out, void* workspace, size_t workspace_bytes, void* stream);

size_t ccab_ey_fit_workspace_bytes(int n_views, const int64_t* dims, int k, int batch);
int ccab_ey_fit(int n_views, const int64_t* dims, int k, double c, double learning_rate, double momentum, double tol,
                int n_steps, const double* cov, int dtype, const void* const* views, const int64_t* ld, int batch,
                const int32_t* idx, double* state, void* workspace, size_t workspace_bytes, void* stream);

size_t ccab_gfa_fit_workspace_bytes(int n_views, const int64_t* dims, int k);
int ccab_gfa_fit(int n_views, const int64_t* dims, int k, const double* G, double n_samples, const double* XtZ0,
                 double tol, int drop_k, int n_steps, double* state, void* workspace, size_t workspace_bytes,
                 void* stream);

size_t ccab_ccaloss_workspace_bytes(int dtype, int precision, int d1, int d2, int64_t n);
int ccab_ccaloss_fwd(int dtype, int precision, const void* z1, int64_t ld1, const void* z2, int64_t ld2, int64_t n,
                     int d1, int d2, double eps, void* loss, void* saved, int* flags_dev, void* workspace,
                     size_t workspace_bytes, void* stream);
int ccab_ccaloss_bwd(int dtype, const void* z1, int64_t ld1, const void* z2, int64_t ld2, int64_t n, int d1, int d2,
                     const void* saved, const void* grad_out, void* g1, int64_t ldg1, void* g2, int64_t ldg2,
                     void* stream);

int ccab_scale(int dtype, int m, int n, const void* A, int64_t lda, const void* r, int r_pow, const void* c,
               int c_pow, void* B, int64_t ldb, void* stream);

int ccab_center_columns(int dtype, int m, int n, void* A, int64_t lda, void* stream);

int ccab_frobenius_norm(int dtype, int m, int n, const void* A, int64_t lda, void* out, void* stream);

int ccab_profile_moments(int enable);
double ccab_profile_moments_last_ms(void);

#ifdef __cplusplus
}
#endif
#endif
```

Baseline: 166.4.

## Overlap diagonal-block moments and whitening with cross-view moments on a side stream

Adds an overlapped rCCA fit path for two float32 CUDA views under tf32x3b. The moment computation is split into two tile sets: the within-view blocks go first on a high-priority side stream, which then runs the ridge covariance, pivot tolerance and Cholesky inverse. Meanwhile the cross-view block is computed on the main stream, and the cross-covariance is filled once both streams join. The intent is to hide whitening latency behind the cross-moment GEMM, at the cost of an extra stream, events, a mutex and more complex moment kernels. It also adds a shifted retry when syevj does not converge.

```diff
diff --git a/cca_zoo_b200/_base.py b/cca_zoo_b200/_base.py
--- a/cca_zoo_b200/_base.py
+++ b/cca_zoo_b200/_base.py
@@ -200,7 +200,7 @@
     def _device_fit_plan(self, dims, n_local, in_dtype):
         return None
 
-    def _fit_moments(self, mom, n_local, dims, in_dtype):
+    def _fit_moments(self, mom, n_local, dims, in_dtype, first=None):
         plan = self._device_fit_plan(dims, n_local, in_dtype)
         if plan is None:
             C, dims, n_total = self._covariance_stage(mom, n_local, dims, in_dtype, True)
@@ -209,8 +209,11 @@
         solve_dtype = self._solve_dtype(in_dtype)
         attempts = plan.pop("iters")
         hdr = None
-        for iters in attempts:
-            block, offsets = plan["call"](mom, dims, n_host, n_dev, solve_dtype, iters)
+        for attempt, iters in enumerate(attempts):
+            if attempt == 0 and first is not None:
+                block, offsets = first
+            else:
+                block, offsets = plan["call"](mom, dims, n_host, n_dev, solve_dtype, iters)
             host = block.cpu()
             hdr, mean, sig, ws = ops.decode_fit_block(host, offsets, dims, plan["k"], solve_dtype)
             status = int(hdr[0])
diff --git a/cca_zoo_b200/_lib.py b/cca_zoo_b200/_lib.py
--- a/cca_zoo_b200/_lib.py
+++ b/cca_zoo_b200/_lib.py
@@ -54,6 +54,10 @@
     "ccab_rcca_fit_result_layout": (C.c_int, [C.c_int, _i64p, C.c_int, C.c_int, _i64p]),
     "ccab_rcca_fit": (C.c_int, [C.c_int, _i64p, _vp, _vp, C.c_double, C.c_int, C.POINTER(C.c_double), C.c_int, C.c_int,
                                 C.c_int, _vp, C.c_size_t, _vp, C.c_size_t, _vp]),
+    "ccab_rcca_fit_overlapped_workspace_bytes": (C.c_size_t, [C.c_int, _i64p, C.c_int64, C.c_int, C.c_int]),
+    "ccab_rcca_fit_overlapped": (C.c_int, [C.c_int, _i64p, C.POINTER(_vp), _i64p, C.c_int64, _vp, C.c_int,
+                                           C.POINTER(C.c_double), C.c_int, C.c_int, C.c_int, _vp, C.c_size_t, _vp,
+                                           C.c_size_t, _vp]),
     "ccab_ccaloss_workspace_bytes": (C.c_size_t, [C.c_int, C.c_int, C.c_int, C.c_int, C.c_int64]),
     "ccab_ccaloss_fwd": (C.c_int, [C.c_int, C.c_int, _vp, C.c_int64, _vp, C.c_int64, C.c_int64, C.c_int, C.c_int,
                                    C.c_double, _vp, _vp, _vp, _vp, C.c_size_t, _vp]),
diff --git a/cca_zoo_b200/_solvers.py b/cca_zoo_b200/_solvers.py
--- a/cca_zoo_b200/_solvers.py
+++ b/cca_zoo_b200/_solvers.py
@@ -69,7 +69,10 @@
         by_size.setdefault(d, []).append(i)
     for d, idx in by_size.items():
         A = torch.stack([C[sl[i], sl[i]] for i in idx]).contiguous()
-        ev, evt = ops.syevj(A)
+        ev, evt, info = ops.syevj(A, return_info=True)
+        if not info.get("converged", True):
+            shift = float((torch.diagonal(A, dim1=-2, dim2=-1).sum(-1) / d).max())
+            ev, evt = ops.syevj(A, shift=shift)
         for b, i in enumerate(idx):
             lams[i], vts[i] = ev[b], evt[b]
     return lams, vts
diff --git a/cca_zoo_b200/csrc/api.cu b/cca_zoo_b200/csrc/api.cu
--- a/cca_zoo_b200/csrc/api.cu
+++ b/cca_zoo_b200/csrc/api.cu
@@ -497,6 +497,37 @@
   CCAB_CATCH
 }
 
+size_t ccab_rcca_fit_overlapped_workspace_bytes(int dtype, const int64_t* dims, int64_t n_rows, int k, int p) {
+  ColumnLayout L;
+  if (!dims || (dtype != CCAB_F32 && dtype != CCAB_F64) || make_layout(2, dims, &L)) return 0;
+  return dtype == CCAB_F32 ? rcca_fit_overlapped_workspace_bytes<float>(L, n_rows, k, p)
+                           : rcca_fit_overlapped_workspace_bytes<double>(L, n_rows, k, p);
+}
+
+int ccab_rcca_fit_overlapped(int dtype, const int64_t* dims, const void* const* views, const int64_t* lds,
+                             int64_t n_rows, double* moments, int center, const double* c, int k, int p, int iters,
+                             void* result, size_t result_bytes, void* workspace, size_t workspace_bytes, void* stream) {
+  CCAB_TRY
+  CCAB_CHECK_ARG(dtype == CCAB_F32 || dtype == CCAB_F64, "bad dtype %d", dtype);
+  CCAB_CHECK_ARG(dims && views && lds && moments && c && result && workspace, "null pointer argument");
+  ColumnLayout L;
+  int rc = make_layout(2, dims, &L);
+  if (rc) return rc;
+  for (int v = 0; v < 2; ++v) {
+    CCAB_CHECK_ARG(views[v] != nullptr, "view %d is NULL", v);
+    CCAB_CHECK_ARG(lds[v] >= dims[v], "lds[%d] < dims[%d]", v, v);
+  }
+  rc = require_device();
+  if (rc) return rc;
+  cudaStream_t s = static_cast<cudaStream_t>(stream);
+  if (dtype == CCAB_F32)
+    return rcca_fit_overlapped<float>(L, views, lds, n_rows, moments, center, c, k, p, iters, result, result_bytes,
+                                      workspace, workspace_bytes, s);
+  return rcca_fit_overlapped<double>(L, views, lds, n_rows, moments, center, c, k, p, iters, result, result_bytes,
+                                     workspace, workspace_bytes, s);
+  CCAB_CATCH
+}
+
 size_t ccab_ccaloss_workspace_bytes(int dtype, int precision, int d1, int d2, int64_t n) {
   int64_t dims[2] = {d1, d2};
   ColumnLayout L;
diff --git a/cca_zoo_b200/csrc/fit.cu b/cca_zoo_b200/csrc/fit.cu
--- a/cca_zoo_b200/csrc/fit.cu
+++ b/cca_zoo_b200/csrc/fit.cu
@@ -1,6 +1,7 @@
 #include "fit.cuh"
 
 #include <cmath>
+#include <mutex>
 #include <type_traits>
 
 #include "ccaloss.cuh"
@@ -41,7 +42,7 @@
 template <typename T>
 __global__ void cov_ridge_kernel(const CovRidgeParams p, const double* __restrict__ mom, const double* __restrict__ n_dev,
                                  double n_host, int center, T* __restrict__ C, int64_t ldc, double* __restrict__ mean,
-                                 unsigned* __restrict__ dmax, int* __restrict__ flags) {
+                                 unsigned* __restrict__ dmax, int* __restrict__ flags, int part = 0) {
   const double n_total = n_dev ? n_dev[0] : n_host;
   const double* M = mom;
   const double* s = mom + (size_t)p.Dp * p.Dp;
@@ -50,6 +51,8 @@
   if (gi >= p.D || gj >= p.D) return;
   const int vi = view_of(p, gi), vj = view_of(p, gj);
   const int pi = p.poff[vi] + gi - p.coff[vi], pj = p.poff[vj] + gj - p.coff[vj];
+  if (gi == 0 && mean && part != 2) mean[gj] = center ? s[pj] / n_total : 0.0;
+  if ((part == 1 && vi != vj) || (part == 2 && vi == vj)) return;
   const int r = min(pi, pj), c = max(pi, pj);
   double v = M[(size_t)r * p.Dp + c];
   if (!isfinite(v)) atomicOr(flags, 1);
@@ -62,7 +65,6 @@
     static_cast<T*>(p.R[vi])[(size_t)(gi - p.coff[vi]) * p.ldr[vi] + (gj - p.coff[vj])] = (T)rv;
     if (gi == gj && dmax) atomicMax(dmax + vi, __float_as_uint(fmaxf((float)v, 0.f)));
   }
-  if (gi == 0 && mean) mean[gj] = center ? s[pj] / n_total : 0.0;
   if (gi == 0 && gj == 0 && !(n_total >= 2.0)) atomicOr(flags, 2);
 }
 
@@ -270,10 +272,51 @@
   offsets[4] = (int64_t)P.r_total;
 }
 
-template <typename T>
-int rcca_fit(const ColumnLayout& L, const double* moments, const double* n_dev, double n_host, int center,
-             const double* c, int k, int p, int iters, void* result, size_t result_bytes, void* ws, size_t ws_bytes,
-             cudaStream_t s) {
+namespace {
+
+struct RccaViews {
+  const void* const* views;
+  const int64_t* lds;
+  int64_t n_rows;
+  void* ws;
+  size_t ws_bytes;
+};
+
+struct SideStream {
+  cudaStream_t stream = nullptr;
+  cudaEvent_t fork = nullptr, join = nullptr;
+  std::mutex lock;
+};
+
+SideStream* side_stream() {
+  static SideStream side[64];
+  static std::mutex init;
+  int dev = 0;
+  if (cudaGetDevice(&dev) != cudaSuccess || dev < 0 || dev >= 64) {
+    set_error("no current CUDA device for the whitening stream");
+    return nullptr;
+  }
+  std::lock_guard<std::mutex> g(init);
+  SideStream& st = side[dev];
+  if (!st.stream) {
+    int least = 0, greatest = 0;
+    cudaStream_t stream = nullptr;
+    if (cudaDeviceGetStreamPriorityRange(&least, &greatest) != cudaSuccess ||
+        cudaStreamCreateWithPriority(&stream, cudaStreamNonBlocking, greatest) != cudaSuccess ||
+        cudaEventCreateWithFlags(&st.fork, cudaEventDisableTiming) != cudaSuccess ||
+        cudaEventCreateWithFlags(&st.join, cudaEventDisableTiming) != cudaSuccess) {
+      set_error("could not create the whitening stream and its events");
+      return nullptr;
+    }
+    st.stream = stream;
+  }
+  return &st;
+}
+
+template <typename T>
+int rcca_fit_impl(const ColumnLayout& L, const double* moments, const double* n_dev, double n_host, int center,
+                  const double* c, int k, int p, int iters, void* result, size_t result_bytes, void* ws,
+                  size_t ws_bytes, cudaStream_t s, const RccaViews* src) {
   CCAB_CHECK_ARG(L.n_views == 2, "rcca_fit needs exactly 2 views");
   const int d1 = L.dims[0], d2 = L.dims[1], D = L.D;
   CCAB_CHECK_ARG(k >= 1 && p >= k && p <= std::min(d1, d2), "rcca_fit: need 1 <= k <= p <= min(d1, d2), got k=%d p=%d", k,
@@ -319,6 +362,18 @@
   unsigned* resid_cnt = reinterpret_cast<unsigned*>(sm + 1280 + 8 * kResidBlocks);
 
   CCAB_CUDA(cudaMemsetAsync(sm, 0, 2048, s));
+  SideStream* side = nullptr;
+  std::unique_lock<std::mutex> side_lock;
+  cudaStream_t ws_stream = s;
+  if (src) {
+    side = side_stream();
+    if (!side) return -2;
+    side_lock = std::unique_lock<std::mutex>(side->lock);
+    ws_stream = side->stream;
+    int rc = moments_x3b_split(L, src->views, src->lds, src->n_rows, const_cast<double*>(moments), src->ws,
+                               src->ws_bytes, s, ws_stream, side->fork);
+    if (rc) return rc;
+  }
   double* hdr = reinterpret_cast<double*>(res);
   double* mean = reinterpret_cast<double*>(res + P.r_mean);
   T* sig = reinterpret_cast<T*>(res + P.r_sig);
@@ -333,26 +388,41 @@
     for (int v = 0; v <= 2; ++v) { cp.coff[v] = L.coff[v]; cp.poff[v] = L.poff[v]; }
     cp.R[0] = R1; cp.R[1] = R2; cp.ldr[0] = ldr1; cp.ldr[1] = ldr2;
     dim3 block(32, 8), grid((unsigned)ceil_div(D, 32), (unsigned)ceil_div(D, 8));
-    cov_ridge_kernel<T><<<grid, block, 0, s>>>(cp, moments, n_dev, n_host, center, C, P.ldC, mean, dmax, flags);
+    cov_ridge_kernel<T><<<grid, block, 0, ws_stream>>>(cp, moments, n_dev, n_host, center, C, P.ldC, mean, dmax, flags,
+                                                       src ? 1 : 0);
     count_launches(1);
     PivotTolParams q;
     memset(&q, 0, sizeof(q));
     q.n_views = 2;
     q.c[0] = c[0]; q.c[1] = c[1];
     q.rank_tol[0] = d1 * eps_of<T>(); q.rank_tol[1] = d2 * eps_of<T>();
-    pivot_tol_kernel<<<1, 32, 0, s>>>(q, dmax, tol);
+    pivot_tol_kernel<<<1, 32, 0, ws_stream>>>(q, dmax, tol);
     count_launches(1);
     CCAB_CUDA(cudaGetLastError());
   }
   int rc;
   if (batched) {
-    rc = potrf_inv<T>(d1, 2, R1, ldR, strideR, Li1, ldR, strideR, 0.0, tol, infos, cq.pws, cq.pws_bytes, s);
+    rc = potrf_inv<T>(d1, 2, R1, ldR, strideR, Li1, ldR, strideR, 0.0, tol, infos, cq.pws, cq.pws_bytes, ws_stream);
     if (rc) return rc;
   } else {
-    rc = potrf_inv<T>(d1, 1, R1, ldr1, 0, Li1, ldr1, 0, 0.0, tol, infos, cq.pws, cq.pws_bytes, s);
-    if (rc) return rc;
-    rc = potrf_inv<T>(d2, 1, R2, ldr2, 0, Li2, ldr2, 0, 0.0, tol + 1, infos + 1, cq.pws, cq.pws_bytes, s);
-    if (rc) return rc;
+    rc = potrf_inv<T>(d1, 1, R1, ldr1, 0, Li1, ldr1, 0, 0.0, tol, infos, cq.pws, cq.pws_bytes, ws_stream);
+    if (rc) return rc;
+    rc = potrf_inv<T>(d2, 1, R2, ldr2, 0, Li2, ldr2, 0, 0.0, tol + 1, infos + 1, cq.pws, cq.pws_bytes, ws_stream);
+    if (rc) return rc;
+  }
+  if (src) {
+    CCAB_CUDA(cudaEventRecord(side->join, ws_stream));
+    CCAB_CUDA(cudaStreamWaitEvent(s, side->join, 0));
+    side_lock.unlock();
+    CovRidgeParams cp;
+    memset(&cp, 0, sizeof(cp));
+    cp.n_views = 2; cp.D = D; cp.Dp = L.Dp;
+    for (int v = 0; v < 2; ++v) cp.dims[v] = L.dims[v];
+    for (int v = 0; v <= 2; ++v) { cp.coff[v] = L.coff[v]; cp.poff[v] = L.poff[v]; }
+    dim3 block(32, 8), grid((unsigned)ceil_div(D, 32), (unsigned)ceil_div(D, 8));
+    cov_ridge_kernel<T><<<grid, block, 0, s>>>(cp, moments, n_dev, n_host, center, C, P.ldC, nullptr, nullptr, flags, 2);
+    count_launches(1);
+    CCAB_CUDA(cudaGetLastError());
   }
   {
     GemmArgs<T> g;
@@ -454,6 +524,39 @@
   count_launches(1);
   CCAB_CUDA(cudaGetLastError());
   return 0;
+}
+
+}
+
+template <typename T>
+int rcca_fit(const ColumnLayout& L, const double* moments, const double* n_dev, double n_host, int center,
+             const double* c, int k, int p, int iters, void* result, size_t result_bytes, void* ws, size_t ws_bytes,
+             cudaStream_t s) {
+  return rcca_fit_impl<T>(L, moments, n_dev, n_host, center, c, k, p, iters, result, result_bytes, ws, ws_bytes, s,
+                          nullptr);
+}
+
+template <typename T>
+size_t rcca_fit_overlapped_workspace_bytes(const ColumnLayout& L, int64_t n_rows, int k, int p) {
+  if (L.n_views != 2 || !moments_x3b_splits(L, n_rows)) return 0;
+  const size_t fit = rcca_fit_workspace_bytes<T>(L.dims[0], L.dims[1], k, p);
+  if (!fit) return 0;
+  return al256(fit) + moments_workspace_bytes(0, 3, L, n_rows) + 256;
+}
+
+template <typename T>
+int rcca_fit_overlapped(const ColumnLayout& L, const void* const* views, const int64_t* lds, int64_t n_rows,
+                        double* moments, int center, const double* c, int k, int p, int iters, void* result,
+                        size_t result_bytes, void* ws, size_t ws_bytes, cudaStream_t s) {
+  const size_t need = rcca_fit_overlapped_workspace_bytes<T>(L, n_rows, k, p);
+  CCAB_CHECK_ARG(need, "rcca_fit_overlapped takes two views whose tf32x3b moments fit one pass, and a shape rcca_fit "
+                       "takes");
+  CCAB_CHECK_ARG(ws_bytes >= need, "rcca_fit_overlapped workspace too small: %zu < %zu", ws_bytes, need);
+  const size_t fit = al256(rcca_fit_workspace_bytes<T>(L.dims[0], L.dims[1], k, p));
+  uint8_t* w = reinterpret_cast<uint8_t*>((reinterpret_cast<uintptr_t>(ws) + 255) & ~uintptr_t(255));
+  RccaViews src{views, lds, n_rows, w + fit, ws_bytes - (size_t)(w - static_cast<uint8_t*>(ws)) - fit};
+  return rcca_fit_impl<T>(L, moments, nullptr, (double)n_rows, center, c, k, p, iters, result, result_bytes, w, fit, s,
+                          &src);
 }
 
 
@@ -1045,5 +1148,11 @@
                              void*, size_t, void*, size_t, cudaStream_t);
 template int rcca_fit<double>(const ColumnLayout&, const double*, const double*, double, int, const double*, int, int,
                               int, void*, size_t, void*, size_t, cudaStream_t);
-
-}
+template size_t rcca_fit_overlapped_workspace_bytes<float>(const ColumnLayout&, int64_t, int, int);
+template size_t rcca_fit_overlapped_workspace_bytes<double>(const ColumnLayout&, int64_t, int, int);
+template int rcca_fit_overlapped<float>(const ColumnLayout&, const void* const*, const int64_t*, int64_t, double*, int,
+                                        const double*, int, int, int, void*, size_t, void*, size_t, cudaStream_t);
+template int rcca_fit_overlapped<double>(const ColumnLayout&, const void* const*, const int64_t*, int64_t, double*, int,
+                                         const double*, int, int, int, void*, size_t, void*, size_t, cudaStream_t);
+
+}
diff --git a/cca_zoo_b200/csrc/fit.cuh b/cca_zoo_b200/csrc/fit.cuh
--- a/cca_zoo_b200/csrc/fit.cuh
+++ b/cca_zoo_b200/csrc/fit.cuh
@@ -20,6 +20,13 @@
              cudaStream_t stream);
 
 template <typename T>
+size_t rcca_fit_overlapped_workspace_bytes(const ColumnLayout& L, int64_t n_rows, int k, int p);
+template <typename T>
+int rcca_fit_overlapped(const ColumnLayout& L, const void* const* views, const int64_t* lds, int64_t n_rows,
+                        double* moments, int center, const double* c, int k, int p, int iters, void* result,
+                        size_t result_bytes, void* ws, size_t ws_bytes, cudaStream_t stream);
+
+template <typename T>
 size_t mcca_fit_workspace_bytes(const ColumnLayout& L, int k, int p);
 template <typename T>
 void mcca_fit_result_layout(const ColumnLayout& L, int k, int p, int64_t* offsets);
diff --git a/cca_zoo_b200/csrc/moments.cu b/cca_zoo_b200/csrc/moments.cu
--- a/cca_zoo_b200/csrc/moments.cu
+++ b/cca_zoo_b200/csrc/moments.cu
@@ -28,22 +28,27 @@
 }
 
 static bool g_prof_on = false;
-static cudaEvent_t g_prof_e0 = nullptr, g_prof_e1 = nullptr;
-static bool g_prof_valid = false;
+static cudaEvent_t g_prof_e0 = nullptr, g_prof_e1 = nullptr, g_prof_e2 = nullptr;
+static bool g_prof_valid = false, g_prof_split = false;
 void moments_profile_enable(int on) {
   g_prof_on = on != 0;
   g_prof_valid = false;
   if (g_prof_on && !g_prof_e0) {
     cudaEventCreate(&g_prof_e0);
     cudaEventCreate(&g_prof_e1);
+    cudaEventCreate(&g_prof_e2);
   }
 }
 float moments_profile_last_ms() {
   if (!g_prof_valid) return -1.f;
-  float ms = -1.f;
+  float ms = -1.f, ms2 = -1.f;
   if (cudaEventSynchronize(g_prof_e1) != cudaSuccess) return -1.f;
   if (cudaEventElapsedTime(&ms, g_prof_e0, g_prof_e1) != cudaSuccess) return -1.f;
-  return ms;
+  if (g_prof_split) {
+    if (cudaEventSynchronize(g_prof_e2) != cudaSuccess) return -1.f;
+    if (cudaEventElapsedTime(&ms2, g_prof_e0, g_prof_e2) != cudaSuccess) return -1.f;
+  }
+  return std::max(ms, ms2);
 }
 
 struct WgParams {
@@ -55,6 +60,7 @@
   int64_t n_rows, rows_per_split;
   int64_t row_base;
   int nblocks, Dp;
+  int tile_set, xv_rows, xv_col;
 };
 static_assert(sizeof(WgParams) <= 4096, "kernel parameter space");
 
@@ -268,9 +274,15 @@
               "the register budgets must fit in what the CTA is allocated at launch");
 static_assert(4 % PairCfg::kFrag == 0, "a slice is four steps");
 
-inline int pair_tiles(int nblocks) {
+__host__ __device__ __forceinline__ int pair_row_lo(int set, int i, int xv_col) { return set == 2 ? xv_col : 2 * i; }
+__host__ __device__ __forceinline__ int pair_row_hi(int set, int i, int nblocks, int xv_rows, int xv_col) {
+  return set == 1 && i < xv_rows ? xv_col : nblocks;
+}
+
+inline int pair_tile_count(int nblocks, int set, int xv_rows, int xv_col) {
   int n = 0;
-  for (int i = 0; 2 * i < nblocks; ++i) n += nblocks - 2 * i;
+  for (int i = 0; 2 * i < nblocks && (set != 2 || i < xv_rows); ++i)
+    n += pair_row_hi(set, i, nblocks, xv_rows, xv_col) - pair_row_lo(set, i, xv_col);
   return n;
 }
 
@@ -285,8 +297,13 @@
   uint64_t* op_full = raw_empty + NR;
   uint64_t* op_empty = op_full + NO;
 
-  int t = blockIdx.x, i = 0, rowlen = p.nblocks;
-  while (t >= rowlen) { t -= rowlen; ++i; rowlen -= 2; }
+  int t = blockIdx.x, i = 0;
+  for (;;) {
+    const int lo = pair_row_lo(p.tile_set, i, p.xv_col), hi = pair_row_hi(p.tile_set, i, p.nblocks, p.xv_rows, p.xv_col);
+    if (t < hi - lo) { t += lo - 2 * i; break; }
+    t -= hi - lo;
+    ++i;
+  }
   const int a0 = 2 * i, bj = a0 + t;
   const int nload = min(t, 2) + 1;
   const int na = min(nload, 2);
@@ -653,11 +670,15 @@
 template <typename T>
 __global__ void reduce_partials_kernel(const T* __restrict__ partial, const T* __restrict__ partial_sum,
                                        int S, int Dp, int ldp, int blk, double* __restrict__ out,
-                                       int accumulate = 0) {
+                                       int accumulate = 0, int tile_set = 0, int xv_rows = 0, int xv_col = 0) {
   const size_t total = (size_t)Dp * Dp + (partial_sum ? Dp : 0);
   const size_t slab = (size_t)ldp * ldp;
   for (size_t i = blockIdx.x * (size_t)blockDim.x + threadIdx.x; i < total;
        i += (size_t)gridDim.x * blockDim.x) {
+    if (tile_set) {
+      const bool xv = i < (size_t)Dp * Dp && (int)(i / Dp) / blk < 2 * xv_rows && (int)(i % Dp) / blk >= xv_col;
+      if (xv != (tile_set == 2)) continue;
+    }
     double acc = 0.0;
     if (i < (size_t)Dp * Dp) {
       const int r = (int)(i / Dp), c = (int)(i % Dp);
@@ -837,8 +858,9 @@
 
 }
 
-int moments_tf32(const ColumnLayout& L, const void* const* views, const int64_t* lds, int64_t n_rows, int mode,
-                 double* moments_out, void* ws, size_t ws_bytes, cudaStream_t stream) {
+namespace {
+int init_wg_params(const ColumnLayout& L, const void* const* views, const int64_t* lds, int64_t n_rows,
+                   WgParams& prm) {
   CCAB_CHECK_ARG(n_rows >= 1 && n_rows < (int64_t)1 << 31, "n_rows out of range");
   for (int v = 0; v < L.n_views; ++v)
     CCAB_CHECK_ARG((reinterpret_cast<uintptr_t>(views[v]) & 15) == 0 && lds[v] % 4 == 0,
@@ -849,7 +871,6 @@
     CCAB_CUDA(cudaGetDevice(&dev));
     CCAB_CUDA(cudaSetDevice(dev));
   }
-  WgParams prm;
   memset(&prm, 0, sizeof(prm));
   for (int v = 0; v < L.n_views; ++v) {
     int rc = encode_view_map(&prm.map[v], views[v], n_rows, L.dims[v], lds[v]);
@@ -861,17 +882,51 @@
       prm.blk_view[b] = (uint8_t)v;
       prm.blk_col0[b] = c;
     }
+  return 0;
+}
+}
+
+int moments_tf32(const ColumnLayout& L, const void* const* views, const int64_t* lds, int64_t n_rows, int mode,
+                 double* moments_out, void* ws, size_t ws_bytes, cudaStream_t stream) {
+  WgParams prm;
+  int rc = init_wg_params(L, views, lds, n_rows, prm);
+  if (rc) return rc;
   const int64_t cap = tc_rows_cap(L, mode);
   if (n_rows <= cap) return moments_tf32_pass(L, prm, 0, n_rows, mode, moments_out, ws, ws_bytes, stream, 0);
   const int64_t npass = ceil_div(n_rows, cap);
   const int64_t per = std::min(cap, ceil_div(ceil_div(n_rows, npass), 2048) * 2048);
   int pass = 0;
   for (int64_t r0 = 0; r0 < n_rows; r0 += per, ++pass) {
-    int rc = moments_tf32_pass(L, prm, r0, std::min(per, n_rows - r0), mode, moments_out, ws, ws_bytes, stream,
-                               pass > 0);
+    rc = moments_tf32_pass(L, prm, r0, std::min(per, n_rows - r0), mode, moments_out, ws, ws_bytes, stream,
+                           pass > 0);
     if (rc) return rc;
   }
   return 0;
+}
+
+bool moments_x3b_splits(const ColumnLayout& L, int64_t n_rows) {
+  return L.n_views == 2 && n_rows >= 1 && n_rows <= tc_rows_cap(L, 3);
+}
+
+int moments_x3b_split(const ColumnLayout& L, const void* const* views, const int64_t* lds, int64_t n_rows,
+                      double* moments_out, void* ws, size_t ws_bytes, cudaStream_t main, cudaStream_t side,
+                      cudaEvent_t fork) {
+  CCAB_CHECK_ARG(moments_x3b_splits(L, n_rows), "the split moment pass takes two views in one pass");
+  WgParams prm;
+  int rc = init_wg_params(L, views, lds, n_rows, prm);
+  if (rc) return rc;
+  const int b1 = L.poff[1] / kBlk;
+  prm.xv_rows = b1 / 2;
+  prm.xv_col = b1;
+  const bool cross = pair_tile_count(L.nblocks, 2, prm.xv_rows, prm.xv_col) > 0;
+  if (g_prof_on && cross) cudaEventRecord(g_prof_e0, main);
+  CCAB_CUDA(cudaEventRecord(fork, main));
+  CCAB_CUDA(cudaStreamWaitEvent(side, fork, 0));
+  prm.tile_set = cross ? 1 : 0;
+  rc = moments_tf32_pass(L, prm, 0, n_rows, 3, moments_out, ws, ws_bytes, side, 0);
+  if (rc || !cross) return rc;
+  prm.tile_set = 2;
+  return moments_tf32_pass(L, prm, 0, n_rows, 3, moments_out, ws, ws_bytes, main, 0);
 }
 
 namespace {
@@ -886,7 +941,8 @@
 int launch_x3b_pair(int num_splits, const WgParams& prm, cudaStream_t stream) {
   CCAB_CUDA(cudaFuncSetAttribute(moments_x3b_pair_kernel, cudaFuncAttributeMaxDynamicSharedMemorySize,
                                  PairCfg::kSmem));
-  moments_x3b_pair_kernel<<<dim3(pair_tiles(prm.nblocks), num_splits), kPrThreads, PairCfg::kSmem, stream>>>(prm);
+  const int tiles = pair_tile_count(prm.nblocks, prm.tile_set, prm.xv_rows, prm.xv_col);
+  moments_x3b_pair_kernel<<<dim3(tiles, num_splits), kPrThreads, PairCfg::kSmem, stream>>>(prm);
   return 0;
 }
 
@@ -907,7 +963,8 @@
   prm.nblocks = L.nblocks;
   prm.Dp = L.Dp;
   dim3 grid(P.ntiles, P.num_splits);
-  if (g_prof_on) cudaEventRecord(g_prof_e0, stream);
+  const bool set1 = prm.tile_set == 1;
+  if (g_prof_on && !prm.tile_set) cudaEventRecord(g_prof_e0, stream);
   int rc = mode == 3   ? launch_x3b_pair(P.num_splits, prm, stream)
            : mode != 0 ? launch_wgmma<K1Mode::X3>(grid, prm, stream)
                        : launch_wgmma<K1Mode::TF32>(grid, prm, stream);
@@ -915,14 +972,17 @@
   count_launches(1);
   CCAB_CUDA(cudaGetLastError());
   if (g_prof_on) {
-    cudaEventRecord(g_prof_e1, stream);
-    g_prof_valid = true;
+    cudaEventRecord(set1 ? g_prof_e2 : g_prof_e1, stream);
+    g_prof_split = prm.tile_set != 0;
+    g_prof_valid = !set1;
   }
 
   const size_t total = (size_t)L.Dp * L.Dp + L.Dp;
-  int rblocks = (int)std::min<size_t>((total + 255) / 256, (size_t)sm_count() * 8);
+  const int rcap = set1 ? 2 : 8;
+  int rblocks = (int)std::min<size_t>((total + 255) / 256, (size_t)sm_count() * rcap);
   reduce_partials_kernel<float><<<rblocks, 256, 0, stream>>>(d_partial, d_partial_sum, P.num_splits, L.Dp, L.Dp,
-                                                            kBlk, moments_out, accumulate); count_launches(1);
+                                                            kBlk, moments_out, accumulate, prm.tile_set, prm.xv_rows,
+                                                            prm.xv_col); count_launches(1);
   CCAB_CUDA(cudaGetLastError());
   return 0;
 }
diff --git a/cca_zoo_b200/csrc/moments.cuh b/cca_zoo_b200/csrc/moments.cuh
--- a/cca_zoo_b200/csrc/moments.cuh
+++ b/cca_zoo_b200/csrc/moments.cuh
@@ -23,6 +23,11 @@
 
 int moments_tf32(const ColumnLayout& L, const void* const* views, const int64_t* lds, int64_t n_rows,
                  int mode , double* moments_out, void* ws, size_t ws_bytes, cudaStream_t stream);
+
+bool moments_x3b_splits(const ColumnLayout& L, int64_t n_rows);
+int moments_x3b_split(const ColumnLayout& L, const void* const* views, const int64_t* lds, int64_t n_rows,
+                      double* moments_out, void* ws, size_t ws_bytes, cudaStream_t main, cudaStream_t side,
+                      cudaEvent_t fork);
 
 template <typename T>
 int moments_simt(const ColumnLayout& L, const void* const* views, const int64_t* lds, int64_t n_rows,
diff --git a/cca_zoo_b200/linear/_rcca.py b/cca_zoo_b200/linear/_rcca.py
--- a/cca_zoo_b200/linear/_rcca.py
+++ b/cca_zoo_b200/linear/_rcca.py
@@ -5,10 +5,11 @@
 from numbers import Real
 from typing import Any, ClassVar
 
+import torch
 from sklearn.utils._param_validation import Interval, StrOptions
 
 from .._base import BaseModel
-from .. import ops
+from .. import ops, parallel
 from ..ops import rcca_fit_workspace_bytes
 from .._solvers import rcca_weights
 from .._validation import perview_parameter, validate_views
@@ -35,14 +36,38 @@
         self._validate_params()
         validated = validate_views(views)
         device = self._device()
-        mom, n_local, dims, in_dtype = self._local_moments(validated, device)
+        overlapped = self._overlapped_moments(validated, device)
+        if overlapped is None:
+            mom, n_local, dims, in_dtype = self._local_moments(validated, device)
+            first = None
+        else:
+            mom, n_local, dims, in_dtype, first = overlapped
         self._partial = None
         if len(dims) != 2:
             raise ValueError(
                 f"rCCA requires exactly 2 views, got {len(dims)}. "
                 "Use MCCA for more than 2 views."
             )
-        return self._fit_moments(mom, n_local, dims, in_dtype)
+        return self._fit_moments(mom, n_local, dims, in_dtype, first=first)
+
+    def _overlapped_moments(self, validated, device):
+        if self.precision != "tf32x3b" or len(validated) != 2 or parallel.is_distributed():
+            return None
+        if not all(isinstance(v, torch.Tensor) and v.is_cuda and v.dtype == torch.float32 for v in validated):
+            return None
+        views = [self._to_device(v, device) for v in validated]
+        n = int(views[0].shape[0])
+        dims = [int(v.shape[1]) for v in views]
+        plan = self._device_fit_plan(dims, n, torch.float32)
+        solve_dtype = self._solve_dtype(torch.float32)
+        if plan is None or ops.rcca_fit_overlapped_workspace_bytes(dims, n, plan["k"], plan["p"], solve_dtype) == 0:
+            return None
+        x0, ratio = ops.column_pilot(views)
+        if ratio > ops.SHIFT_RATIO[torch.float32]:
+            mom, _ = ops.moments_safe(views, precision=self.precision, x0=x0)
+            return mom, n, dims, torch.float32, None
+        mom, block, offsets = plan["overlapped"](views, solve_dtype, plan["iters"][0])
+        return mom, n, dims, torch.float32, (block, offsets)
 
     def _device_fit_plan(self, dims, n_local, in_dtype):
         if self.solver == "eigen":
@@ -61,7 +86,10 @@
         def call(mom, dims_, n_host, n_dev, solve_dtype, iters):
             return ops.rcca_fit(mom, dims_, n_host, n_dev, center, c_, k, p, iters, solve_dtype)
 
-        return {"call": call, "k": k, "iters": [first, 20]}
+        def overlapped(views, solve_dtype, iters):
+            return ops.rcca_fit_overlapped(views, center, c_, k, p, iters, solve_dtype)
+
+        return {"call": call, "overlapped": overlapped, "k": k, "p": p, "iters": [first, 20]}
 
     def _solve(self, C, dims, n_total):
         c_ = perview_parameter("c", self.c, 0.0, 2)
diff --git a/cca_zoo_b200/ops.py b/cca_zoo_b200/ops.py
--- a/cca_zoo_b200/ops.py
+++ b/cca_zoo_b200/ops.py
@@ -468,6 +468,48 @@
                                ws.numel(), _stream(mom))
     _lib.check(rc, "ccab_rcca_fit")
     return block, offsets
+
+
+def rcca_fit_overlapped_workspace_bytes(dims, n_rows: int, k: int, p: int, dtype) -> int:
+    return int(_lib.load().ccab_rcca_fit_overlapped_workspace_bytes(_DT[dtype], _lib.i64_array(dims), int(n_rows),
+                                                                     int(k), int(p)))
+
+
+def rcca_fit_overlapped(views, center: bool, c, k: int, p: int, iters: int, dtype):
+    lib = _lib.load()
+    if len(views) != 2:
+        raise ValueError(f"rcca_fit_overlapped takes 2 views, got {len(views)}")
+    for v in views:
+        _require_cuda(v, "view")
+        if v.dtype != torch.float32:
+            raise ValueError("rcca_fit_overlapped takes float32 views")
+    if views[0].shape[0] != views[1].shape[0] or views[0].device != views[1].device:
+        raise ValueError("the views must have the same number of samples and live on one device")
+    vs = [_row_major(v, tma=True) for v in views]
+    n = int(vs[0].shape[0])
+    dims = [int(v.shape[1]) for v in vs]
+    d = _lib.i64_array(dims)
+    lds = _lib.i64_array([v.stride(0) for v in vs])
+    ptrs = (C.c_void_p * 2)(*[v.data_ptr() for v in vs])
+    dev = vs[0].device
+    dt = _DT[dtype]
+    wsb = lib.ccab_rcca_fit_overlapped_workspace_bytes(dt, d, n, int(k), int(p))
+    if wsb == 0:
+        raise ValueError(f"rcca_fit_overlapped does not take dims={dims}, n={n}, k={k}, p={p}")
+    offs = (C.c_int64 * 5)()
+    _lib.check(lib.ccab_rcca_fit_result_layout(dt, d, int(k), int(p), offs), "ccab_rcca_fit_result_layout")
+    offsets = [int(x) for x in offs]
+    mom = torch.empty(lib.ccab_moments_size(2, d), dtype=torch.float64, device=dev)
+    block = torch.empty(offsets[4] + 256, dtype=torch.uint8, device=dev)
+    shift = (-block.data_ptr()) % 256
+    block = block[shift:shift + offsets[4]]
+    ws = _ws(wsb, dev)
+    cc = (C.c_double * 2)(float(c[0]), float(c[1]))
+    with torch.cuda.device(dev):
+        rc = lib.ccab_rcca_fit_overlapped(dt, d, ptrs, lds, n, _ptr(mom), 1 if center else 0, cc, int(k), int(p),
+                                          int(iters), _ptr(block), block.numel(), _ptr(ws), ws.numel(), _stream(mom))
+    _lib.check(rc, "ccab_rcca_fit_overlapped")
+    return mom, block, offsets
 
 
 def mcca_fit(mom: torch.Tensor, dims, n_host, n_dev, center: bool, c, eps: float, k: int, p: int, iters: int, dtype):
diff --git a/include/ccab200.h b/include/ccab200.h
--- a/include/ccab200.h
+++ b/include/ccab200.h
@@ -87,6 +87,11 @@
                   int center, const double* c, int k, int p, int iters, void* result, size_t result_bytes,
                   void* workspace, size_t workspace_bytes, void* stream);
 
+size_t ccab_rcca_fit_overlapped_workspace_bytes(int dtype, const int64_t* dims, int64_t n_rows, int k, int p);
+int ccab_rcca_fit_overlapped(int dtype, const int64_t* dims, const void* const* views, const int64_t* lds,
+                             int64_t n_rows, double* moments, int center, const double* c, int k, int p, int iters,
+                             void* result, size_t result_bytes, void* workspace, size_t workspace_bytes, void* stream);
+
 size_t ccab_mcca_fit_workspace_bytes(int dtype, int n_views, const int64_t* dims, int k, int p);
 int ccab_mcca_fit_result_layout(int dtype, int n_views, const int64_t* dims, int k, int p, int64_t* offsets);
 int ccab_mcca_fit(int dtype, int n_views, const int64_t* dims, const double* moments, const double* n_total_dev,
```

Result: faster. 182.8, median of 6 (+9.8%).
